# DoHoonKim8/halo2-lasso

Hardware: AMD Instinct MI355X
Metric: lasso_prove_time_ms (lower is better)
Workload: dtype u256 (BN254 Fr/Fq, 8x u32 Montgomery); 1 GPU; 2^24 AND Lasso lookup (32-bit operands, 4 chunks of 8+8 bits); lookups_per_proof=16777216, pcs=multilinear KZG (BN254), proof_bytes=64256, parallelism=1 GPU

## Files before the change

bindings/rust/src/sys.rs:

```rust
#![allow(non_camel_case_types, dead_code)]
use halo2_curves::bn256::{Fr, G1Affine, G2Affine};
use std::os::raw::{c_char, c_int, c_void};

pub type lh_status = c_int;
pub const LH_OK: lh_status = 0;
pub const LH_ERR_INVALID_SUMCHECK: lh_status = -1;
pub const LH_ERR_INVALID_PCS_PARAM: lh_status = -2;
pub const LH_ERR_INVALID_PCS_OPEN: lh_status = -3;
pub const LH_ERR_INVALID_SNARK: lh_status = -4;
pub const LH_ERR_SERIALIZATION: lh_status = -5;
pub const LH_ERR_TRANSCRIPT: lh_status = -6;
pub const LH_ERR_DEVICE: lh_status = -7;
pub const LH_ERR_ARG: lh_status = -8;

pub const LH_SC_MAX_TERMS: usize = 48;
pub const LH_SC_MAX_FACTORS: usize = 4;
pub const LH_SC_EVALUATIONS: c_int = 0;
pub const LH_SC_COEFFICIENTS: c_int = 1;
pub const LH_LASSO_MAX_CHUNKS: usize = 8;
pub const LH_LASSO_MAX_MEMORIES: usize = 16;
pub const LH_LASSO_MAX_TERMS: usize = 16;
pub const LH_RCCL_UNIQUE_ID_BYTES: usize = 128;

#[repr(C)] pub struct lh_ctx { _p: [u8; 0] }
// ... 95 lines not shown
    pub g_factor: [[u8; LH_SC_MAX_FACTORS]; LH_LASSO_MAX_TERMS],
}

#[repr(C)]
pub struct lh_comm {
    pub rank: c_int,
    pub size: c_int,
    pub user: *mut c_void,
    pub all_gather: Option<unsafe extern "C" fn(*mut c_void, *const c_void, *mut c_void, usize) -> c_int>,
    pub all_gather_device: Option<unsafe extern "C" fn(*mut c_void, *const c_void, *mut c_void, usize, *mut c_void) -> c_int>,
}

#[repr(C)]
pub struct lh_hp_lookup { pub inputs: *const lh_expr, pub tables: *const lh_expr, pub width: usize }
#[repr(C)] #[derive(Clone, Copy)]
pub struct lh_hp_lasso_lookup {
    pub table: lh_lasso_table,
    pub output_poly: usize,
    pub chunk_polys: [usize; LH_LASSO_MAX_CHUNKS],
}
#[repr(C)]
pub struct lh_hp_param {
    pub num_vars: usize,
    pub num_instance_polys: usize,
    pub num_instances: *const usize,
    pub num_preprocess_polys: usize,
    pub d_preprocess_polys: *const *const c_void,
    pub num_witness_polys: usize,
    pub num_challenges: usize,
    pub num_lookups: usize,
    pub lookups: *const lh_hp_lookup,
    pub num_permutation_polys: usize,
    pub permutation_poly_index: *const usize,
    pub d_permutation_polys: *const *const c_void,
    pub num_permutation_z_polys: usize,
    pub expression: lh_expr,
    pub num_lasso_lookups: usize,
    pub lasso_lookups: *const lh_hp_lasso_lookup,
}
#[repr(C)]
pub struct lh_hp_vparam {
    pub num_vars: usize,
    pub num_instance_polys: usize,
    pub num_instances: *const usize,
    pub num_witness_polys: usize,
    pub num_challenges: usize,
    pub num_lookups: usize,
    pub num_permutation_z_polys: usize,
    pub expression: lh_expr,
    pub num_preprocess_polys: usize,
    pub preprocess_comms: *const G1Affine,
    pub num_permutation_polys: usize,
    pub permutation_comms: *const G1Affine,
    pub num_lasso_lookups: usize,
    pub lasso_lookups: *const lh_hp_lasso_lookup,
}
#[repr(C)]
pub struct lh_hp_circuit {
    pub user: *mut c_void,
    pub synthesize: Option<unsafe extern "C" fn(*mut c_void, usize, *const Fr, usize, *mut *const c_void, usize) -> c_int>,
}

#[repr(C)]
#[derive(Clone, Copy, Debug, Default)]
pub struct lh_lasso_route {
    pub open_small_depth: u32,
    pub open_small_passes: u32,
    pub eq_factored_rounds: u32,
    pub standard_rounds: u32,
    pub rw_leaf_rounds: u32,
    pub resident_tails: u32,
    pub resident_rounds: u32,
    pub packed_ts_pairs: u32,
    pub derived_commitments: u32,
    pub sorted_dim_reuse: u32,
    pub sharded_rounds: u32,
    pub shard_exchanges: u32,
    pub window_table_jobs: u32,
    pub open_precommit: u32,
    pub resident_layers: u32,
    pub pp_folds: u32,
    pub msm_half_batches: u32,
    pub open_shared_sums: u32,
    pub reserved: [u32; 6],
}

extern "C" {
    pub fn lh_last_error() -> *const c_char;
    pub fn lh_version() -> *const c_char;
    pub fn lh_ctx_create(device_id: c_int, out: *mut *mut lh_ctx) -> lh_status;
    pub fn lh_ctx_destroy(ctx: *mut lh_ctx);
    pub fn lh_ctx_sync(ctx: *mut lh_ctx) -> lh_status;
    pub fn lh_ctx_stream(ctx: *mut lh_ctx) -> *mut c_void;
    pub fn lh_alloc(ctx: *mut lh_ctx, bytes: usize, d_out: *mut *mut c_void) -> lh_status;
    pub fn lh_free(ctx: *mut lh_ctx, d_ptr: *mut c_void) -> lh_status;
    pub fn lh_upload(ctx: *mut lh_ctx, d_dst: *mut c_void, src: *const c_void, bytes: usize) -> lh_status;
    pub fn lh_download(ctx: *mut lh_ctx, dst: *mut c_void, d_src: *const c_void, bytes: usize) -> lh_status;
    pub fn lh_fr_from_u64(ctx: *mut lh_ctx, d_in: *const u64, n: usize, d_out: *mut Fr) -> lh_status;
    pub fn lh_fr_from_u32(ctx: *mut lh_ctx, d_in: *const u32, n: usize, d_out: *mut Fr) -> lh_status;
    pub fn lh_fr_batch_invert(ctx: *mut lh_ctx, d_in: *const Fr, n: usize, d_out: *mut Fr) -> lh_status;
    pub fn lh_fix_var(ctx: *mut lh_ctx, d_in: *const Fr, n_in: usize, x: *const Fr, d_out: *mut Fr) -> lh_status;
    pub fn lh_eq_xy(ctx: *mut lh_ctx, y: *const Fr, num_vars: usize, d_out: *mut Fr) -> lh_status;
    pub fn lh_evaluate(ctx: *mut lh_ctx, d_polys: *const *const Fr, num_polys: usize, num_vars: usize,
                       point: *const Fr, out_evals: *mut Fr) -> lh_status;
    pub fn lh_lincomb(ctx: *mut lh_ctx, d_polys: *const *const Fr, w: *const Fr, num_polys: usize, n: usize,
                      d_out: *mut Fr) -> lh_status;
    pub fn lh_sumcheck_prove(ctx: *mut lh_ctx, prover_kind: c_int, num_vars: usize, expr: *const lh_sop,
                             d_polys: *const *const Fr, num_polys: usize, ys: *const Fr, num_ys: usize,
                             sum: *const Fr, t: *mut lh_transcript, out_challenges: *mut Fr, out_evals: *mut Fr) -> lh_status;
    pub fn lh_sumcheck_prove_expr(ctx: *mut lh_ctx, num_vars: usize, expr: *const lh_expr, d_polys: *const *const Fr,
                                  num_polys: usize, challenges: *const Fr, num_challenges: usize, ys: *const Fr,
                                  num_ys: usize, sum: *const Fr, t: *mut lh_transcript, out_challenges: *mut Fr,
                                  out_evals: *mut Fr) -> lh_status;
    pub fn lh_sumcheck_verify(prover_kind: c_int, num_vars: usize, degree: usize, sum: *const Fr,
                              t: *mut lh_transcript, out_eval: *mut Fr, out_x: *mut Fr) -> lh_status;
    pub fn lh_gkr_fractional_prove(ctx: *mut lh_ctx, num_batching: usize, num_vars: usize,
                                   claimed_p_0s: *const *const Fr, claimed_q_0s: *const *const Fr,
                                   d_ps: *const *const Fr, d_qs: *const *const Fr, t: *mut lh_transcript,
                                   out_p_xs: *mut Fr, out_q_xs: *mut Fr, out_x: *mut Fr) -> lh_status;
    pub fn lh_msm(ctx: *mut lh_ctx, d_scalars: *const Fr, d_bases: *const G1Affine, n: usize, out: *mut G1Affine) -> lh_status;
    pub fn lh_msm_u32(ctx: *mut lh_ctx, d_scalars: *const u32, d_bases: *const G1Affine, n: usize, out: *mut G1Affine) -> lh_status;
    pub fn lh_srs_upload(ctx: *mut lh_ctx, eqs_flat: *const G1Affine, num_vars: usize, out: *mut *mut lh_srs) -> lh_status;
    pub fn lh_srs_num_vars(srs: *const lh_srs) -> usize;
    pub fn lh_srs_free(ctx: *mut lh_ctx, srs: *mut lh_srs);
    pub fn lh_mkzg_batch_commit(ctx: *mut lh_ctx, srs: *const lh_srs, d_polys: *const *const Fr, num_polys: usize,
                                num_vars: usize, out_comms: *mut G1Affine) -> lh_status;
    pub fn lh_mkzg_open(ctx: *mut lh_ctx, srs: *const lh_srs, d_poly: *const Fr, num_vars: usize, point: *const Fr,
                        t: *mut lh_transcript, out_eval: *mut Fr) -> lh_status;
    pub fn lh_mkzg_batch_open(ctx: *mut lh_ctx, srs: *const lh_srs, num_vars: usize, d_polys: *const *const Fr,
                              num_polys: usize, points: *const Fr, num_points: usize, evals: *const lh_evaluation,
                              num_evals: usize, t: *mut lh_transcript) -> lh_status;
    pub fn lh_mkzg_vp_new(g1: *const G1Affine, g2: *const G2Affine, ss: *const G2Affine, num_vars: usize,
                          out: *mut *mut lh_mkzg_vp) -> lh_status;
    pub fn lh_mkzg_vp_free(vp: *mut lh_mkzg_vp);
    pub fn lh_mkzg_verify(vp: *const lh_mkzg_vp, comm: *const G1Affine, point: *const Fr, num_vars: usize,
                          eval: *const Fr, t: *mut lh_transcript) -> lh_status;
    pub fn lh_mkzg_batch_verify(vp: *const lh_mkzg_vp, num_vars: usize, comms: *const G1Affine, num_comms: usize,
                                points: *const Fr, num_points: usize, evals: *const lh_evaluation, num_evals: usize,
                                t: *mut lh_transcript) -> lh_status;
    pub fn lh_lasso_prove(ctx: *mut lh_ctx, srs: *const lh_srs, table: *const lh_lasso_table, num_vars: usize,
                          d_dims: *const *const u32, t: *mut lh_transcript) -> lh_status;
    pub fn lh_lasso_verify(vp: *const lh_mkzg_vp, table: *const lh_lasso_table, num_vars: usize,
                           t: *mut lh_transcript) -> lh_status;
    pub fn lh_ctx_set_comm(ctx: *mut lh_ctx, comm: *const lh_comm, shard_bit: usize) -> lh_status;
    pub fn lh_rccl_unique_id(out: *mut u8) -> lh_status;
    pub fn lh_ctx_set_comm_rccl(ctx: *mut lh_ctx, rank: c_int, size: c_int, unique_id: *const u8, shard_bit: usize) -> lh_status;
    pub fn lh_ctx_set_comm_loopback(ctx: *mut lh_ctx, rank: c_int, size: c_int, shard_bit: usize) -> lh_status;
    pub fn lh_ctx_comm_stats(ctx: *mut lh_ctx, out: *mut u64) -> lh_status;
    pub fn lh_ctx_comm_phase_stats(ctx: *mut lh_ctx, out: *mut u64, reset: c_int) -> lh_status;
    pub fn lh_ctx_memory_stats(ctx: *mut lh_ctx, out: *mut u64) -> lh_status;
    pub fn lh_ctx_compute_units(ctx: *mut lh_ctx, out: *mut usize) -> lh_status;
    pub fn lh_ctx_host_cpus(ctx: *mut lh_ctx, bus_id: *mut c_char, bus_id_cap: usize, cpulist: *mut c_char, cpulist_cap: usize) -> lh_status;
    pub fn lh_shard_extract(ctx: *mut lh_ctx, d_global: *const c_void, n_local: usize, shard_bit: usize, rho: usize,
                            rank: usize, elem_bytes: usize, d_local: *mut c_void) -> lh_status;
    pub fn lh_ctx_set_option(ctx: *mut lh_ctx, name: *const c_char, value: i64) -> lh_status;
    pub fn lh_ctx_get_option(ctx: *mut lh_ctx, name: *const c_char, out: *mut i64) -> lh_status;
    pub fn lh_lasso_last_route(ctx: *mut lh_ctx, out: *mut lh_lasso_route) -> lh_status;
    pub fn lh_lasso_prove_sharded(ctx: *mut lh_ctx, srs: *const lh_srs, table: *const lh_lasso_table, num_vars: usize,
                                  d_dims_local: *const *const u32, t: *mut lh_transcript) -> lh_status;
    pub fn lh_hyperplonk_prove(ctx: *mut lh_ctx, srs: *const lh_srs, pp: *const lh_hp_param,
                               instances: *const *const Fr, d_witness_polys: *const *const Fr,
                               t: *mut lh_transcript) -> lh_status;
    pub fn lh_hyperplonk_prove_sharded(ctx: *mut lh_ctx, srs: *const lh_srs, pp: *const lh_hp_param,
                                       instances: *const *const Fr, d_witness_polys_local: *const *const Fr,
                                       t: *mut lh_transcript) -> lh_status;
    pub fn lh_hyperplonk_prove_phases(ctx: *mut lh_ctx, srs: *const lh_srs, pp: *const lh_hp_param, num_phases: usize,
                                      num_witness_polys: *const usize, num_challenges: *const usize,
// ... 183 lines not shown
```

halo2-lasso_amd/__init__.py:

```python
import ctypes as C

from . import _ffi
from ._ffi import (lh_fr, lh_g1, lh_sop, lh_evaluation, lh_lasso_table, lh_transcript,
                   LH_SC_EVALUATIONS, LH_SC_COEFFICIENTS)

R_MOD = 0x30644E72E131A029B85045B68181585D2833E84879B9709143E1F593F0000001
Q_MOD = 0x30644E72E131A029B85045B68181585D97816A916871CA8D3C208C16D87CFD47
_MONT = 1 << 256
_MONT_INV_R = pow(_MONT, -1, R_MOD)
_MONT_INV_Q = pow(_MONT, -1, Q_MOD)

SUBTABLE_IDENTITY, SUBTABLE_AND, SUBTABLE_XOR = 0, 1, 2


class Error(Exception):
    code = None


class InvalidSumcheck(Error):
    code = _ffi.LH_ERR_INVALID_SUMCHECK


class InvalidPcsParam(Error):
    code = _ffi.LH_ERR_INVALID_PCS_PARAM
# ... 1395 lines not shown
            C.memmove(recv, out, len(out))
            return 0
        except Exception:
            return _ffi.LH_ERR_DEVICE
    comm = _ffi.lh_comm()
    comm.rank, comm.size, comm.user = rank, size, None
    comm.all_gather = _ffi._AG_CB(cb)
    ctx._comm_keepalive = (comm, cb)
    _check(ctx.lib.lh_ctx_set_comm(ctx.h, C.byref(comm), shard_bit))


def rccl_unique_id():
    buf = C.create_string_buffer(_ffi.LH_RCCL_UNIQUE_ID_BYTES)
    _check(_ffi.load().lh_rccl_unique_id(buf))
    return buf.raw


def attach_comm_rccl(ctx, rank, size, unique_id, shard_bit):
    if len(unique_id) != _ffi.LH_RCCL_UNIQUE_ID_BYTES:
        raise ArgumentError("unique id must be %d bytes" % _ffi.LH_RCCL_UNIQUE_ID_BYTES)
    _check(ctx.lib.lh_ctx_set_comm_rccl(ctx.h, rank, size, unique_id, shard_bit))


def comm_stats(ctx):
    out = (C.c_uint64 * 2)()
    _check(ctx.lib.lh_ctx_comm_stats(ctx.h, out))
    return {"device": int(out[0]), "host": int(out[1])}


def comm_phase_stats(ctx, reset=False):
    out = (C.c_uint64 * 16)()
    _check(ctx.lib.lh_ctx_comm_phase_stats(ctx.h, out, 1 if reset else 0))
    names = ["witness", "commit", "surge", "leaves", "gkr", "evals", "open", "outside"]
    return {nm: {"collectives": int(out[2 * i]), "bytes": int(out[2 * i + 1])} for i, nm in enumerate(names) if out[2 * i]}


def memory_stats(ctx):
    out = (C.c_uint64 * 4)()
    _check(ctx.lib.lh_ctx_memory_stats(ctx.h, out))
    return {"arena_high_water_bytes": int(out[0]), "arena_reserved_bytes": int(out[1]), "device_free_bytes": int(out[2]),
            "device_total_bytes": int(out[3])}


def attach_comm_loopback(ctx, rank, size, shard_bit):
    _check(ctx.lib.lh_ctx_set_comm_loopback(ctx.h, rank, size, shard_bit))


def detach_comm(ctx):
    _check(ctx.lib.lh_ctx_set_comm(ctx.h, None, 0))
    ctx._comm_keepalive = None


def shard_of(column, rank, size, shard_bit):
    rho = size.bit_length() - 1
    n = len(column)
    return column.reshape(n >> (shard_bit + rho), size, 1 << shard_bit)[:, rank, :].reshape(-1).copy()


def shard_poly(poly, rank, size, shard_bit):
    rho = size.bit_length() - 1
    n_local = (1 << poly.num_vars) >> rho
    out = poly.ctx.alloc(32 * n_local)
    _check(poly.ctx.lib.lh_shard_extract(poly.ctx.h, poly.ptr, n_local, shard_bit, rho, rank, 32, out.ptr))
    return MultilinearPolynomial(poly.ctx, out, poly.num_vars - rho)


def lasso_prove_sharded(pp, table, num_vars, dims_local, transcript):
    if len(dims_local) != table.c:
        raise ArgumentError("expected %d dim columns" % table.c)
    t = table.to_c()
    _check(pp.ctx.lib.lh_lasso_prove_sharded(pp.ctx.h, pp.h, C.byref(t), num_vars, _ptr_array(dims_local), transcript.p))


def lasso_last_timing(ctx):
    out = (C.c_double * _ffi.LH_LASSO_NUM_PHASES)()
    _check(ctx.lib.lh_lasso_last_timing(ctx.h, out))
    names = ["witness", "commit", "surge", "leaves", "gkr", "evals", "open_n", "open_l", "total"]
    return dict(zip(names, list(out)))


ROUTE_FIELDS = ["open_small_depth", "open_small_passes", "eq_factored_rounds", "standard_rounds", "rw_leaf_rounds",
                "resident_tails", "resident_rounds", "packed_ts_pairs", "derived_commitments", "sorted_dim_reuse",
                "sharded_rounds", "shard_exchanges", "window_table_jobs", "open_precommit", "resident_layers", "pp_folds", "msm_half_batches",
                "open_shared_sums"]


def lasso_last_route(ctx):
    out = (C.c_uint32 * 24)()
    _check(ctx.lib.lh_lasso_last_route(ctx.h, out))
    return dict(zip(ROUTE_FIELDS, [int(v) for v in out]))


def set_option(ctx, name, value):
    _check(ctx.lib.lh_ctx_set_option(ctx.h, name.encode(), int(value)))


def get_option(ctx, name):
    out = C.c_int64(0)
    _check(ctx.lib.lh_ctx_get_option(ctx.h, name.encode(), C.byref(out)))
    return int(out.value)


def profile_enable(ctx, on=True):
    _check(ctx.lib.lh_profile_enable(ctx.h, int(on)))


def profile_read(ctx):
    n = C.c_size_t()
    _check(ctx.lib.lh_profile_read(ctx.h, None, 0, C.byref(n)))
    arr = (_ffi.lh_prof_rec * max(n.value, 1))()
    _check(ctx.lib.lh_profile_read(ctx.h, arr, n.value, C.byref(n)))
    return [dict(name=r.name.decode(), ms=r.ms, bytes=r.bytes, muls=r.muls, items=r.items) for r in arr[:n.value]]


from . import expression
```

halo2-lasso_amd/csrc/dev.cpp:

```cpp
#include <string.h>
#include <stdlib.h>
#include <ctype.h>
#include <errno.h>
#include <sched.h>
#include <atomic>
#include <condition_variable>
#include <mutex>
#include <thread>
#include <functional>
#include <memory>
#include <emmintrin.h>
#include <hip/hip_ext.h>
#include <vector>
#include <chrono>
#include "dev.hpp"

namespace lh {

static thread_local std::string g_last_error;
void set_last_error(const char* msg) { g_last_error = msg ? msg : ""; }
const char* get_last_error() { return g_last_error.c_str(); }

Arena::~Arena() {
  for (auto& b : blocks_) (void)hipFree(b.p);
}

void* Arena::alloc(size_t bytes) {
  bytes = (bytes + 255) & ~(size_t)255;
  if (bytes == 0) bytes = 256;
  return alloc_raw(bytes);
}
void* Arena::alloc_raw(size_t bytes) {
  while (true) {
    if (!blocks_.empty()) {
      Block& b = blocks_[cur_];
      if (b.used + bytes <= b.size) {
        void* p = b.p + b.used;
        b.used += bytes;
        size_t tot = 0;
        for (size_t i = 0; i <= cur_; i++) tot += blocks_[i].used;
        if (tot > high_) high_ = tot;
        return p;
      }
      if (cur_ + 1 < blocks_.size()) {
        cur_++;
        blocks_[cur_].used = 0;
        continue;
      }
    }
    size_t want = blocks_.empty() ? ((size_t)64 << 20) : blocks_.back().size * 2;
    if (want < bytes) want = bytes;
    void* p = nullptr;
    LH_HIP(hipMalloc(&p, want));
    blocks_.push_back(Block{(char*)p, want, 0});
    cur_ = blocks_.size() - 1;
  }
}

void Arena::release(Mark m) {
  if (blocks_.empty()) return;
  for (size_t i = m.block + 1; i < blocks_.size(); i++) blocks_[i].used = 0;
  cur_ = m.block;
  blocks_[cur_].used = m.used;
}

void Ctx::opt_in_lds(const void* fn, int bytes) {
  for (const void* f : lds_opted)
    if (f == fn) return;
  LH_HIP(hipFuncSetAttribute(fn, hipFuncAttributeMaxDynamicSharedMemorySize, bytes));
  lds_opted.push_back(fn);
}

static const struct {
  const char* name;
  int64_t Options::*field;
  int64_t lo, hi;
} OPTION_TABLE[] = {
    {"open_small_min_vars", &Options::open_small_min_vars, 0, 64}, {"open_small_depth", &Options::open_small_depth, 0, 2},
    {"sc_eq_factoring", &Options::sc_eq_factoring, 0, 1},          {"lasso_pack_ts", &Options::lasso_pack_ts, 0, 1},
    {"sc_tail", &Options::sc_tail, 0, 1},                          {"sc_tail_max_len", &Options::sc_tail_max_len, 0, (int64_t)1 << 20},
    {"shard_exchange_log", &Options::shard_exchange_log, 0, 40},   {"msm_window_tables", &Options::msm_window_tables, 0, 40},
    {"open_precommit", &Options::open_precommit, 0, 64},           {"gkr_resident", &Options::gkr_resident, 0, 1},
    {"sc_pp_fold", &Options::sc_pp_fold, 0, 2},                    {"msm_half_batches", &Options::msm_half_batches, 0, 1},
    {"comm_round", &Options::comm_round, 0, 2},                    {"hyrax_rows", &Options::hyrax_rows, 0, 1},
    {"brakedown_batch_commit", &Options::brakedown_batch_commit, 0, 1}, {"brakedown_staged_open", &Options::brakedown_staged_open, 0, 1},
};

int64_t* Options::find(const char* name) {
  if (!name) return nullptr;
  for (const auto& o : OPTION_TABLE)
    if (strcmp(o.name, name) == 0) return &(this->*o.field);
  return nullptr;
}
bool Options::in_range(const char* name, int64_t value) {
  if (!name) return false;
  for (const auto& o : OPTION_TABLE)
    if (strcmp(o.name, name) == 0) return value >= o.lo && value <= o.hi;
  return false;
}

static bool env_number(const char* name, bool real, double lo, double hi, double& out, std::atomic<bool>* said = nullptr) {
  const char* e = getenv(name);
  if (!e || !*e) return false;
  char* end = nullptr;
  errno = 0;
  const double v = real ? strtod(e, &end) : (double)strtoll(e, &end, 10);
  if (end != e && *end == 0 && errno == 0 && v >= lo && v <= hi) {
    out = v;
    return true;
  }
  if (!said || !said->exchange(true))
    fprintf(stderr, "[lasso-hip] %s=%s is outside [%lld, %lld]: ignored\n", name, e, (long long)lo, (long long)hi);
  return false;
}

Options::Options() {
  for (const auto& o : OPTION_TABLE) {
    std::string env = "LH_";
    for (const char* p = o.name; *p; p++) env.push_back((char)toupper((unsigned char)*p));
    double v;
    if (!env_number(env.c_str(), false, (double)o.lo, (double)o.hi, v)) continue;
    this->*o.field = (int64_t)v;
    if (o.field == &Options::open_small_min_vars) open_small_min_vars_forced = true;
  }
}

enum KnobKind { INT, REAL, WORD, PATH };
static constexpr struct KnobRow {
  const char* env;
  KnobKind kind;
  double dflt, lo, hi;
  bool live;
  const char* word;
} KNOB_TABLE[] = {
    {"LH_SC_TAIL_G", INT, 0, 0, 1024},
    {"LH_MSM_C_OFF", INT, 4, -32, 32},
    {"LH_MSM_C_MAX", INT, 17, 1, 31},
    {"LH_MSM_K2", INT, 4, 2, 64},
    {"LH_MSM_SEG", INT, 0, 0, 256},
    {"LH_MSM_SLAB_LOG", INT, 16, 0, 31},
    {"LH_MSM_TREE_MAX", INT, 262144, 0, 1 << 30},
    {"LH_MSM_QUAD_MAX", INT, 262144, 0, 1 << 30},
    {"LH_MSM_TWO_LEVEL", INT, 1, 0, 1},
    {"LH_MSM_HALF_MIN_LOG", INT, 24, 0, 63},
    {"LH_MSM_HALF_COVER", INT, 12, 0, 1 << 20},
    {"LH_EXPR_MONOMIALS", INT, 0, 0, 1},
    {"LH_EXPR_JIT_MIN_VARS", INT, 16, 0, 64},
    {"LH_EXPR_EF_MIN_VARS", INT, 14, 2, 64},
    {"LH_FIN_LANES_MIN_BYTES", REAL, 0, -1, 1e18},
    {"LH_SC_U32", INT, 1, 0, 1}, {"LH_OPEN_U32_ROUNDS", INT, 1, 0, 1}, {"LH_OPEN_FOLD_COLS", INT, 1, 0, 1},
    {"LH_OPEN_SHARE_SUMS", INT, 1, 0, 1, true},
    {"LH_HOST_THREADS", INT, 48, 0, 4096},
    {"LH_JIT_CACHE", INT, 1, 0, 1}, {"LH_JIT_CACHE_DIR", PATH, 0, 0, 0},
    {"LH_EXPR_JIT", INT, 1, 0, 1},
    {"LH_SC_TAIL_TIMEOUT_MS", REAL, 2000, 0, 1e7, true}, {"LH_GKR_START_TIMEOUT_MS", REAL, 25, 0, 1e7, true},
    {"LH_COMM_WAIT_TIMEOUT_MS", INT, 30000, 1, 1e9}, {"LH_COMM_A2A", WORD, 0, 0, 1, false, "allgather"},
    {"LH_COMM_PROBE", INT, 1, 0, 1},
    {"LH_HOST_TRACE", INT, 0, 0, 1, true}, {"LH_SC_TAIL_TRACE", INT, 0, 0, 1}, {"LH_GKR_TRACE", INT, 0, 0, 1},
    {"LH_SC_DEBUG", INT, 0, 0, 1}, {"LH_MSM_DEBUG", INT, 0, 0, 1}, {"LH_HP_DEBUG", INT, 0, 0, 1}, {"LH_COMM_DEBUG", INT, 0, 0, 1},
    {"LH_OPEN_SMALL_CHECK", INT, 0, 0, 1},
    {"LH_COMM_A2A_SELF", INT, 0, 0, 1}, {"LH_COMM_PROBE_FAIL", INT, 0, 0, 1}, {"LH_SHARDED_COUNTERS_MIN_R", INT, 2, 1, 1 << 20},
};
static_assert(sizeof(KNOB_TABLE) / sizeof(KNOB_TABLE[0]) == (size_t)Knob::COUNT, "KNOB_TABLE: one row per Knob");

static double knob_read(const KnobRow& r, std::atomic<bool>* said) {
  double v = r.dflt;
  if (r.kind != WORD) {
    env_number(r.env, r.kind == REAL, r.lo, r.hi, v, said);
// ... 418 lines not shown
```

halo2-lasso_amd/csrc/dev.hpp:

```cpp
#pragma once
#include <hip/hip_runtime_api.h>
#include <stdint.h>
#include <stdarg.h>
#include <stdio.h>
#include <functional>
#include <string>
#include <vector>
#include <utility>
#include <stdexcept>

#include "../../include/lasso_hip.h"
#include "ec.cuh"

namespace lh {

struct Error : std::exception {
  int code;
  std::string msg;
  Error(int c, std::string m) : code(c), msg(std::move(m)) {}
  const char* what() const noexcept override { return msg.c_str(); }
};

void set_last_error(const char* msg);

#define LH_HIP(expr)                                                                       \
  do {                                                                                     \
    hipError_t e_ = (expr);                                                                \
    if (e_ != hipSuccess)                                                                  \
      throw ::lh::Error(LH_ERR_DEVICE, std::string(#expr) + ": " + hipGetErrorString(e_)); \
  } while (0)

#define LH_REQUIRE(cond, code, text) \
  do {                               \
    if (!(cond)) throw ::lh::Error((code), (text)); \
  } while (0)

class Arena {
 public:
  struct Mark {
    size_t block, used;
  };
  ~Arena();
  void* alloc(size_t bytes);
  void* alloc_raw(size_t bytes);
  template <class T>
  T* alloc_n(size_t n) {
    return (T*)alloc(n * sizeof(T));
  }
  Mark mark() const { return {cur_, blocks_.empty() ? 0 : blocks_[cur_].used}; }
  void release(Mark m);
  size_t high_water() const { return high_; }
  size_t reserved() const {
    size_t t = 0;
    for (const Block& b : blocks_) t += b.size;
    return t;
  }

 private:
  struct Block {
    char* p;
    size_t size, used;
  };
  std::vector<Block> blocks_;
  size_t cur_ = 0, high_ = 0;
};

struct ArenaScope {
  Arena& a;
  Arena::Mark m;
  explicit ArenaScope(Arena& a_) : a(a_), m(a_.mark()) {}
  ~ArenaScope() { a.release(m); }
};

struct ProfRec {
  char name[40];
  double ms;
  double bytes;
  double muls;
  double items;
};

struct ScFinishArgs {
  uint32_t* ticket;
  uint32_t last_ticket;
  Fr* out_host;
  uint32_t* flag;
  uint32_t seq;
  uint64_t* wide;
  uint32_t tag;
  uint64_t* lanes;
};
constexpr uint32_t FIN_LANE_SUMS = 65536;
constexpr unsigned SC_LANE_TAG_SHIFT = 40;

struct Options {
  int64_t open_small_min_vars = 21;
  bool open_small_min_vars_forced = false;
  int64_t open_small_depth = 0;
  int64_t sc_eq_factoring = 1;
  int64_t lasso_pack_ts = 1;
  int64_t sc_tail = 1;
  int64_t sc_tail_max_len = 8192;
  int64_t shard_exchange_log = 19;
  int64_t open_precommit = 1;
  int64_t msm_window_tables = 0;
  int64_t sc_pp_fold = 1;
  int64_t msm_half_batches = 1;
  int64_t gkr_resident = 1;
  int64_t comm_round = 0;
  int64_t hyrax_rows = 1;
  int64_t brakedown_batch_commit = 1;
  int64_t brakedown_staged_open = 0;
  Options();
  int64_t* find(const char* name);
  static bool in_range(const char* name, int64_t value);
};

enum class Knob {
  SC_TAIL_G, MSM_C_OFF, MSM_C_MAX, MSM_K2, MSM_SEG, MSM_SLAB_LOG, MSM_TREE_MAX, MSM_QUAD_MAX, MSM_TWO_LEVEL, MSM_HALF_MIN_LOG,
  MSM_HALF_COVER, EXPR_MONOMIALS, EXPR_JIT_MIN_VARS, EXPR_EF_MIN_VARS,
  FIN_LANES_MIN_BYTES, SC_U32, OPEN_U32_ROUNDS, OPEN_FOLD_COLS, OPEN_SHARE_SUMS,
  HOST_THREADS, JIT_CACHE, JIT_CACHE_DIR, EXPR_JIT, SC_TAIL_TIMEOUT_MS, GKR_START_TIMEOUT_MS, COMM_WAIT_TIMEOUT_MS, COMM_A2A,
  COMM_PROBE,
  HOST_TRACE, SC_TAIL_TRACE, GKR_TRACE, SC_DEBUG, MSM_DEBUG, HP_DEBUG, COMM_DEBUG, OPEN_SMALL_CHECK,
  COMM_A2A_SELF, COMM_PROBE_FAIL, SHARDED_COUNTERS_MIN_R,
  COUNT
};
double knob(Knob k);
const char* knob_text(Knob k);
struct RouteStats {
  uint32_t v[LH_LASSO_ROUTE_WORDS] = {0};
  enum { OPEN_DEPTH, OPEN_PASSES, EF_ROUNDS, STD_ROUNDS, RW_ROUNDS, TAILS, TAIL_ROUNDS, PACKED_TS, DERIVED, SORTED_REUSE,
         SHARDED_ROUNDS, SHARD_EXCHANGES, WIN_TABLE_JOBS, OPEN_PRECOMMIT, RESIDENT_LAYERS, PP_FOLDS, MSM_HALF_BATCHES,
         OPEN_SHARED_SUMS };
};

class HostWorker {
 public:
  HostWorker();
  ~HostWorker();
  void submit(std::function<void()> fn);
  void wait();
 private:
  struct Impl;
  Impl* impl_;
};

struct OpenPrecommit;
struct Ctx {
  Options opt;
  RouteStats route;
  int device = 0;
  hipStream_t stream = nullptr;
  Arena arena;
  void* pinned = nullptr;
  size_t pinned_bytes = 0;
  int num_cus = 256;
  int wall_clock_khz = 100000;
  double lasso_ms[LH_LASSO_NUM_PHASES] = {0};
  lh_comm comm = {0, 1, nullptr, nullptr, nullptr};
  bool has_comm = false;
  bool comm_loopback = false;
  size_t shard_bit = 0;
  bool shard_active = false;
  void* rccl_comm = nullptr;
  void* comm_stage = nullptr;
  size_t comm_stage_bytes = 0;
  uint64_t comm_stats[2] = {0, 0};
  uint64_t comm_phase_stats[8][2] = {};
  int comm_phase = 7;
  Fr* sc_redirect = nullptr;
  uint64_t* sc_wide = nullptr;
  uint32_t sc_tag = 0;
  uint32_t sc_tag_seq = 0;
  uint64_t* lanes_host = nullptr;
  bool comm_host_recv_ok = true;
  Fr* round_out(Fr* out_host) const { return sc_redirect ? sc_redirect : out_host; }
  void wait_round(uint32_t seq) {
    if (!sc_redirect) wait_flag(seq);
  }
  uint64_t* tail_trace = nullptr;
  std::vector<std::pair<const char*, double>> host_stamps;
  bool host_trace_on = false;
  void host_stamp(const char* tag);
  void host_stamps_print();
  struct EqHalfEntry {
    std::vector<uint8_t> key;
    const Fr* table;
    bool sharded = false;
  };
  std::vector<EqHalfEntry> eq_half_cache;
  struct QuadSumEntry {
    const uint32_t* col;
    size_t len;
    std::vector<uint8_t> point;
    Fr s[4];
  };
  std::vector<QuadSumEntry> quad_sums;
  bool prof = false;
  std::vector<ProfRec> prof_recs;
  bool live = false;
  struct LiveRec {
    ProfRec rec;
    hipEvent_t e0, e1;
    uint32_t batch;
  };
  std::vector<LiveRec> live_recs;
  std::vector<hipEvent_t> live_pool;
  uint32_t live_batch = 0;
  hipEvent_t live_event();
  void live_resolve(std::vector<ProfRec>& out);
  bool is_helper = false;
  Ctx* helper = nullptr;
  lh_ctx* helper_handle = nullptr;
  OpenPrecommit* precommit = nullptr;
  HostWorker* worker = nullptr;
  hipEvent_t handoff_ev = nullptr;
// ... 35 lines not shown
  void gkr_send_layer(const Fr* vals, size_t count, uint32_t seq);
  void gkr_abort();
  void gkr_resync();
  void wait_flag(uint32_t seq);
  std::vector<const void*> lds_opted;
  void opt_in_lds(const void* fn, int bytes);
  void wait_chunks(const struct TailChunk* chunks, size_t count, uint32_t seq, Fr* out);
  bool wait_chunks_or(const struct TailChunk* chunks, size_t count, uint32_t seq, uint32_t alt, Fr* out);
};

struct ShardActive {
  Ctx& c;
  explicit ShardActive(Ctx& c_) : c(c_) { c.shard_active = true; }
  ~ShardActive() { c.shard_active = false; }
};

struct Shard {
  bool on = false;
  bool loopback = false;
  size_t rho = 0, j = 0, rank = 0, R = 1;
  explicit Shard(const Ctx& c) {
    if (!c.shard_active) return;
    on = true, j = c.shard_bit, rank = (size_t)c.comm.rank, R = (size_t)c.comm.size, loopback = c.comm_loopback;
    while (((size_t)1 << rho) < R) rho++;
  }
  bool sharded(size_t num_vars) const { return on && num_vars >= j + (rho ? rho : 1) + 1; }
  size_t local_vars(size_t num_vars) const { return sharded(num_vars) ? num_vars - rho : num_vars; }
  size_t local_len(size_t num_vars) const { return (size_t)1 << local_vars(num_vars); }
};

struct ReplicatedRange {
  size_t first = 0, count = 0;
  ReplicatedRange(const Shard& sh, size_t len) {
    if (!sh.on || sh.R <= 1) {
      count = len;
    } else if (len < sh.R) {
      count = sh.rank == 0 || sh.loopback ? len : 0;
    } else {
      const size_t per = len / sh.R;
      first = sh.rank * per;
      count = sh.rank + 1 == sh.R ? len - first : per;
    }
  }
};

void host_parallel_for(size_t n, const std::function<void(size_t)>& fn);
void host_parallel_prewake(size_t n, unsigned us);

struct ProfScope {
  Ctx& c;
  ProfRec rec;
  bool on;
  ProfScope(Ctx& c_, const char* name, double bytes, double muls, double items) : c(c_), on(c_.prof) {
    if (!on) return;
    snprintf(rec.name, sizeof rec.name, "%s", name);
    rec.bytes = bytes, rec.muls = muls, rec.items = items, rec.ms = 0;
    if (!c.prof_ev[0]) {
      LH_HIP(hipEventCreate(&c.prof_ev[0]));
      LH_HIP(hipEventCreate(&c.prof_ev[1]));
    }
    LH_HIP(hipEventRecord(c.prof_ev[0], c.stream));
  }
  ~ProfScope() {
    if (!on) return;
    (void)hipEventRecord(c.prof_ev[1], c.stream);
    (void)hipEventSynchronize(c.prof_ev[1]);
    float ms = 0;
    (void)hipEventElapsedTime(&ms, c.prof_ev[0], c.prof_ev[1]);
    rec.ms = ms;
    c.prof_recs.push_back(rec);
  }
};

void k_fr_from_u64(Ctx&, const uint64_t* in, size_t n, Fr* out);
void k_fr_from_u32(Ctx&, const uint32_t* in, size_t n, Fr* out);
void k_fr_to_repr(Ctx&, const Fr* in, size_t n, Fr* out);
void k_fr_from_repr(Ctx&, const Fr* in, size_t n, Fr* out);
void k_fr_binop(Ctx&, int op, const Fr* a, const Fr* b, size_t n, Fr* out);
void k_fr_mul_chain(Ctx&, const Fr* a, const Fr* b, size_t n, int iters, Fr* out);
void k_fr_batch_invert(Ctx&, const Fr* in, size_t n, Fr* out);
void k_fix_var(Ctx&, const Fr* in, size_t n_in, const Fr& x, Fr* out);
void k_fix_var_multi(Ctx&, const Fr* const* in, Fr* const* out, size_t count, size_t n_in, const Fr& x);
void k_eq_xy(Ctx&, const Fr* y, size_t num_vars, Fr* out);
void k_bind_first(Ctx&, const Fr* const* in, size_t count, const Fr& x, Fr* out_host);
void k_gather_heads(Ctx&, const Fr* const* in, size_t count, int k, Fr* out_host);
void k_lincomb(Ctx&, const Fr* const* polys, const Fr* w, size_t count, size_t n, Fr* out);
void k_lincomb_fold(Ctx&, const Fr* const* polys, const Fr* w, size_t count, size_t half, const Fr& x, Fr* out);
bool k_lincomb_fold_small(Ctx&, const uint32_t* const* cols, const size_t* lens, const Fr* coef, size_t count, size_t half,
                          const Fr& x, Fr* out);
void k_inner_products(Ctx&, const Fr* const* polys, size_t count, const Fr* weights, size_t n, Fr* out_host);
constexpr int LCM_MAX_FR = 8, LCM_MAX_SMALL = 24;
constexpr int LCF_MAX = 24;
constexpr int LCB_MAX = 24;
void k_inner_products_small(Ctx&, const uint32_t* const* polys, size_t count, const Fr* weights, size_t n, Fr* out_host);
void k_inner_products_small_half(Ctx&, const uint32_t* const* polys, size_t count, const Fr* eq_half, size_t half,
                                 const Fr& y0, Fr* out_host);
void k_inner_products_small_quads(Ctx&, const uint32_t* col, const Fr* e0, size_t quads, Fr* out_host);
void k_inner_products_quads(Ctx&, const uint32_t* const* cols, const size_t* lens, size_t count, const Fr* e1, size_t quads,
                            Fr* d_out);
constexpr int QS_MAX_COLS = 24;
void k_quad_sums(Ctx&, const uint32_t* const* cols, const size_t* lens, size_t count, const Fr* e0, size_t quads, Fr* d_out);
void k_lincomb_bind2(Ctx&, const uint32_t* const* cols, const size_t* lens, const Fr* w, size_t count, const Fr& r0, const Fr& r1,
                     const Fr* eq_level, size_t size, Fr* out, Fr* out_host);
void k_sc_round_u32_bind2(Ctx&, const uint32_t* col, const Fr* eq_level, const Fr& r0, const Fr& r1, size_t size, Fr* out,
                          Fr* out_host);
void k_lincomb_mixed(Ctx&, const Fr* const* fr, const Fr* wfr, size_t num_fr, const uint32_t* const* sm,
                     const size_t* sm_len, const Fr* wsm, size_t num_sm, size_t n, Fr* out);
void k_tree_up(Ctx&, const Fr* in, size_t half, Fr* out);
void k_tree_up_multi(Ctx&, const Fr* const* in, Fr* const* out, size_t count, size_t half);
void k_tree_tops(Ctx&, const Fr* const* in, Fr* const* out, const int* H, size_t count);
void k_frac_up(Ctx&, const Fr* p, const Fr* q, size_t half, Fr* vp, Fr* vq);
void k_quotient_step(Ctx&, const Fr* rem, size_t half, const Fr& x, Fr* q, Fr* rem_out);
void k_lasso_rw_leaves(Ctx&, const uint32_t* dim, const uint32_t* e, const uint32_t* ts, size_t n,
                       const Fr& gamma, const Fr& gamma2, const Fr& tau, Fr* rs, Fr* ws);
void k_lasso_rw_leaves_up(Ctx&, const uint32_t* dim, const uint32_t* e, const uint32_t* ts, size_t n, const Fr& gamma,
                          const Fr& gamma2, const Fr& tau, Fr* rs, Fr* ws, Fr* rs_up, Fr* ws_up);
void k_lasso_if_leaves(Ctx&, int subtable, uint32_t chunk_bits, const uint32_t* final_cts, size_t m,
                       const Fr& gamma, const Fr& gamma2, const Fr& tau, Fr* init, Fr* fin);
void k_or_u32(Ctx&, const uint32_t* const* cols, size_t count, size_t n, uint32_t* out_host);
void k_fill_u32(Ctx&, uint32_t* out, uint32_t value, size_t n);
void k_pack_u32(Ctx&, const uint32_t* a, const uint32_t* b, uint32_t shift, size_t n, uint32_t* out);
void k_delta_u32(Ctx&, const uint32_t* col, size_t len, size_t half, uint64_t offset, uint32_t* out_lo, uint32_t* out_hi);
void k_lasso_counters(Ctx&, const uint32_t* const* dims, size_t cc, size_t n, size_t m, uint32_t* const* read_ts,
                      uint32_t* const* final_cts, uint32_t* const* keep_sorted = nullptr, uint32_t* const* keep_index = nullptr);
void k_cs_partition(Ctx&, const uint32_t* const* dims, size_t cc, size_t n, size_t m, unsigned rho, unsigned j, unsigned hi_bits,
                    uint32_t* const* sidx, uint32_t* const* send, uint32_t* start_host, bool* bad_out);
void k_cs_rank(Ctx&, const uint32_t* const* recv, const size_t* n_recv, size_t cc, unsigned hi_bits, unsigned a_bits, size_t m_loc,
               uint32_t* const* ret, uint32_t* counts);
void k_cs_scatter(Ctx&, const uint32_t* const* back, const uint32_t* const* sidx, size_t cc, size_t n, uint32_t* const* read_ts);
void k_cs_final(Ctx&, const uint32_t* all_counts, size_t cc, size_t m, unsigned rho, size_t m_loc, uint32_t* const* final_cts);
void k_lasso_subtable_read(Ctx&, int subtable, uint32_t chunk_bits, const uint32_t* dim, size_t n, uint32_t* e);
struct LassoG {
  uint32_t num_terms;
  Fr coeff[LH_LASSO_MAX_TERMS];
  uint8_t nfac[LH_LASSO_MAX_TERMS];
  uint8_t fac[LH_LASSO_MAX_TERMS][LH_SC_MAX_FACTORS];
  const uint32_t* e[LH_LASSO_MAX_MEMORIES];
};
void k_lasso_output(Ctx&, const LassoG& g, size_t n, Fr* a);
struct LassoGSmall {
  uint32_t num_terms;
  uint32_t coeff[LH_LASSO_MAX_TERMS];
  uint8_t fac[LH_LASSO_MAX_TERMS];
  const uint32_t* e[LH_LASSO_MAX_MEMORIES];
};
void k_lasso_output_small(Ctx&, const LassoGSmall& g, size_t n, uint32_t* a);
bool k_fr_to_index(Ctx&, const Fr* in, size_t n, uint32_t bits, uint32_t* out);
bool k_fr_tables_equal(Ctx&, const Fr* a, const Fr* b, size_t n);

void rccl_unique_id(uint8_t out[LH_RCCL_UNIQUE_ID_BYTES]);
void comm_attach_rccl(Ctx&, int rank, int size, const uint8_t id[LH_RCCL_UNIQUE_ID_BYTES], size_t shard_bit);
void comm_probe_host_recv(Ctx&);
void comm_attach_loopback(Ctx&, int rank, int size, size_t shard_bit);
void comm_detach(Ctx&);
void comm_all_gather_dev(Ctx&, const void* d_send, void* d_recv, size_t bytes);
void comm_all_gather_host(Ctx&, const void* send, void* recv, size_t bytes);
void comm_all_to_all_multi(Ctx&, size_t nbuf, const void* const* d_send, const size_t* send_off, const size_t* send_cnt,
                           void* const* d_recv, const size_t* recv_off, const size_t* recv_cnt, const size_t* peer_off,
                           const void* send_base, size_t send_stride, size_t elem);
void comm_sum_publish(Ctx&, const Fr* d_part, Fr* d_scratch, size_t count, Fr* out_host, uint32_t seq);
void comm_sum_lanes(Ctx&, uint64_t* d_lanes, uint64_t* d_scratch, size_t count, Fr* out_host);
uint32_t comm_next_tag(Ctx&);
void k_loopback_allreduce_lanes(Ctx&, const uint64_t* d_in, size_t n, size_t R, uint64_t* out);

void k_shard_merge(Ctx&, const void* gathered, size_t n_local, size_t j, size_t rho, size_t elem, void* global);
void k_gather_interleave(Ctx&, const Fr* gathered, size_t count, size_t n_local, size_t R, size_t block, Fr* const* out);
void k_sum_publish(Ctx&, const Fr* all, size_t R, size_t D, Fr* out_host, uint32_t seq);
void k_shard_extract(Ctx&, const void* global, size_t n_local, size_t j, size_t rho, size_t s, size_t elem, void* local);
void k_loopback_gather(Ctx&, const void* d_send, void* d_recv, size_t bytes, size_t R);
void k_scale(Ctx&, const Fr* in, const Fr& w, size_t n, Fr* out);

constexpr int SC_MAX_TABLES = 72;
struct ScRound {
  const Fr* in[SC_MAX_TABLES];
  Fr* out[SC_MAX_TABLES];
  uint32_t num_tables;
  uint32_t num_terms;
  int32_t global_eq;
  Fr coeff[LH_SC_MAX_TERMS];
  uint8_t coeff_is_one[LH_SC_MAX_TERMS];
  uint8_t nfac[LH_SC_MAX_TERMS];
  uint8_t fac[LH_SC_MAX_TERMS][LH_SC_MAX_FACTORS];
  Fr r;
  const Fr* eq_level;
  uint8_t pp;
};
bool k_sc_round(Ctx&, const ScRound& rd, int degree, bool bind, size_t size, Fr* evals_host);
bool k_sc_round_streams(const ScRound& rd, int degree, size_t size);
void k_eq_levels(Ctx&, const Fr* in, size_t n_in, Fr* const* levels, size_t nlev);
constexpr int SC_OPEN_MAX_TERMS = 6;
struct ScOpenRound {
  const Fr* in[SC_OPEN_MAX_TERMS];
  Fr* out[SC_OPEN_MAX_TERMS];
  const Fr* eq_level[SC_OPEN_MAX_TERMS];
  uint32_t num_terms;
  Fr r;
};
void k_sc_round_open(Ctx&, const ScOpenRound& rd, bool bind, size_t size, Fr* out_host);

constexpr int SC_RW_MAX_PAIRS = 8;
struct ScRwRound {
  const Fr* l[SC_RW_MAX_PAIRS];
  const Fr* r[SC_RW_MAX_PAIRS];
  Fr* lo[SC_RW_MAX_PAIRS];
  Fr* ro[SC_RW_MAX_PAIRS];
  Fr cs[SC_RW_MAX_PAIRS], k[SC_RW_MAX_PAIRS];
  const Fr* eq_level;
  Fr rchal;
  uint32_t num_pairs;
};
void k_sc_round_rw(Ctx&, const ScRwRound& rd, bool bind, size_t size, Fr* out_host, bool fold = false);

struct TailChunk {
  uint32_t w[4];
};
struct TailMbox {
  TailChunk c[3];
  uint32_t pad[4];
};
constexpr uint32_t SC_TAIL_ABORT = 0xffffffffu;
constexpr int SC_TAIL_MAX_DEGREE = 6;
size_t k_sc_tail_capacity(const Ctx&, const ScRound& rd, int degree);
void k_sc_tail_launch(Ctx&, const ScRound& rd, int degree, size_t n0, bool first_bind, size_t num_out, uint32_t seq0,
                      TailChunk* msg_host, Fr* out_host);
void k_sc_tail_resync(Ctx&);

constexpr int GKR_MAX_TREES = 16;
constexpr int GKR_MAX_VARS = 16;
constexpr uint32_t GKR_CAP = 128;
constexpr uint32_t GKR_THREADS = 256;
constexpr uint32_t GKR_MSG_CHUNKS = 3 * (GKR_MAX_TREES + GKR_MAX_VARS);
constexpr uint32_t GKR_START_FAILED = 0xfffffffeu;
enum { GKR_F_SPLIT = 1, GKR_F_BIND = 2, GKR_F_EQ = 4, GKR_F_NOMSG = 8, GKR_F_KOFF = 16 };
struct GkrLayerDev {
  const Fr* lv[GKR_MAX_TREES];
  const Fr* rv[GKR_MAX_TREES];
  uint32_t h, B;
  uint32_t g, s_log;
  uint32_t seq;
  uint32_t flags;
  const Fr* eq_level;
  Fr r_prev;
  Fr coef[GKR_MAX_TREES];
  Fr koff[GKR_MAX_TREES];
};
bool k_gkr_resident_geometry(uint32_t h, uint32_t* g, uint32_t* s_log);
void k_gkr_resident_launch(Ctx&, const GkrLayerDev* layers, size_t num_layers, TailChunk* msg_host, Fr* out_host);

struct ExtRound {
  const Fr* in[SC_MAX_TABLES];
  Fr* out[SC_MAX_TABLES];
  uint32_t num_tables, num_terms;
  const Fr* coeff;
  const uint8_t* is_one;
  const uint32_t* off;
  const uint8_t* fac;
  const uint8_t* store;
  Fr r;
};
void k_sc_round_ext(Ctx&, const ExtRound& rd, int degree, bool bind, size_t size, Fr* evals_host);
void k_rotate_gather(Ctx&, const Fr* poly, size_t num_vars, int rot, uint32_t primitive, uint32_t x_inv, Fr* out);
void k_identity_table(Ctx&, size_t n, Fr* out);
void k_identity_table_shard(Ctx&, size_t n_local, size_t j, size_t rho, size_t rank, Fr* out);
void k_bh_order(Ctx&, size_t num_vars, uint32_t primitive, uint32_t* order, uint32_t* nth);
void k_one_hot_table(Ctx&, size_t n, size_t hot, Fr* out);
enum { PROG_ADD = 0, PROG_SUB = 1, PROG_MUL = 2, PROG_NEG = 3, PROG_MOV = 4 };
enum { PROG_REG = 0, PROG_ATOM = 1, PROG_CONST = 2, PROG_PAIR = 3 };
constexpr int PROG_MAX_REGS = 8;
struct ProgRound {
  const Fr* in[SC_MAX_TABLES];
  uint32_t num_tables, num_instrs, num_regs, result_reg;
  const uint32_t* code;
  const Fr* consts;
};
struct JitKernel;
bool jit_enabled(size_t num_vars);
std::string jit_debug_source(const uint32_t* code, size_t num_instrs, uint32_t num_regs, uint32_t result_reg, int degree);
const JitKernel* jit_sc_round(const Ctx&, const uint32_t* host_code, size_t num_instrs, uint32_t num_regs, uint32_t result_reg, int degree);
unsigned jit_blocks_per_cu(const JitKernel*);
void jit_launch(Ctx&, const JitKernel*, const ProgRound& pr, unsigned points, unsigned grid, size_t size, Fr* partials, const ScFinishArgs& fin);
void k_sc_round_prog(Ctx&, const ProgRound& pr, int points, size_t size, Fr* evals_host, const JitKernel* jit = nullptr);
constexpr int LIN_MAX_TABLES = 8;
struct LinSums {
  const Fr* t[LIN_MAX_TABLES];
  Fr coeff[LIN_MAX_TABLES];
  uint32_t count;
};
void k_lin_sums(Ctx&, const LinSums& ls, size_t size, Fr* out_host);
enum { ROWS_ATOM_POLY = 0, ROWS_ATOM_IDENTITY = 1, ROWS_ATOM_LAGRANGE = 2 };
struct RowsAtom {
// ... 123 lines not shown
```

halo2-lasso_amd/csrc/host.hpp:

```cpp
#pragma once
#include <string.h>
#include <functional>
#include <map>
#include <mutex>
#include <vector>
#include "dev.hpp"
#include "ff_host.hpp"

namespace lh {

const char* get_last_error();

typedef host::Fr HFr;
typedef host::G1Affine HG1;

static inline Fr dev(const HFr& f) {
  Fr r;
  memcpy(&r, &f, 32);
  return r;
}
static inline HFr hst(const Fr& f) {
  HFr r;
  memcpy(&r, &f, 32);
  return r;
// ... 56 lines not shown
  std::vector<HFr> read_field_elements(size_t n) {
    std::vector<HFr> v(n);
    for (auto& f : v) f = read_field_element();
    return v;
  }
  HG1 read_commitment() {
    LH_REQUIRE(t->read_commitment, LH_ERR_ARG, "transcript cannot read (write-only callback table)");
    HG1 p;
    check(t->read_commitment(t->user, (lh_g1*)&p));
    return p;
  }
  std::vector<HG1> read_commitments(size_t n) {
    std::vector<HG1> v(n);
    for (auto& p : v) p = read_commitment();
    return v;
  }
};

typedef std::function<void(size_t num_vars, const HG1* comms, size_t num_comms, const HFr* points, size_t num_points,
                           const lh_evaluation* evals, size_t num_evals, Transcript& tr)>
    PcsBatchVerify;
typedef std::function<std::vector<HG1>(Transcript& tr, size_t n)> PcsReadCommitments;

std::vector<HFr> host_eq_xy(const std::vector<HFr>& y);
HFr host_eq_xy_eval(const HFr* x, const HFr* y, size_t n);
std::vector<HFr> evaluate_polys(Ctx&, const Fr* const* d_polys, size_t count, size_t num_vars, const HFr* point);

struct SumCheckResult {
  std::vector<HFr> challenges;
  std::vector<HFr> evals;
  bool u32_terms_built = false;
};
struct ScRwPairs {
  uint32_t num_pairs;
  HFr cs[SC_RW_MAX_PAIRS], k[SC_RW_MAX_PAIRS];
  HFr const_total;
};
struct ScU32 {
  const uint32_t* col = nullptr;
  bool have_sums = false;
  Fr odd, s2, s3;
};
struct ScU32Terms {
  struct Poly {
    std::vector<const uint32_t*> col;
    std::vector<size_t> len;
    std::vector<Fr> w;
  };
  std::vector<Poly> polys;
};
struct ScOptions {
  bool sum_is_exact = false;
  bool sharded = false;
  const ScRwPairs* rw = nullptr;
  const ScU32* u32 = nullptr;
  const ScU32Terms* u32_terms = nullptr;
};
SumCheckResult sum_check_prove(Ctx&, int prover_kind, size_t num_vars, const lh_sop& expr, const Fr* const* d_polys,
                               size_t num_polys, const HFr* ys, size_t num_ys, const HFr& sum, Transcript& tr,
                               const ScOptions& opt = ScOptions());

const Fr* eq_half_lookup(Ctx&, const HFr* y, size_t num_vars, bool sharded = false);
const Fr* eq_half_get(Ctx&, const HFr* y, size_t num_vars, bool sharded = false);
struct EqHalfScope {
  Ctx& c;
  size_t mark, mark_sums;
  explicit EqHalfScope(Ctx& c_) : c(c_), mark(c_.eq_half_cache.size()), mark_sums(c_.quad_sums.size()) {}
  ~EqHalfScope() {
    c.eq_half_cache.resize(mark);
    c.quad_sums.resize(mark_sums);
  }
};
bool sc_open_column_rounds(const Ctx&, size_t num_vars, bool sharded);
const Fr* quad_sums_lookup(const Ctx&, const uint32_t* col, size_t len, const HFr* y, size_t num_vars);
void quad_sums_put(Ctx&, const uint32_t* col, size_t len, const HFr* y, size_t num_vars, const HFr s[4]);
void quad_sums_evaluate(Ctx&, const uint32_t* const* cols, size_t count, const HFr* y, size_t num_vars, const Fr* eq_half, HFr* evals);

typedef std::function<void(const Fr* const*, Fr* const*, const Fr&, bool, size_t, Fr*)> RoundFn;
struct EqFactoring {
  struct One {
    size_t table;
    const HFr* y;
    std::vector<const Fr*> level;
    HFr S, S_prev;
    std::vector<HFr> q;
  };
  std::vector<One> eqs;
  bool per_term = false;
  bool trusted_claim = false;
  bool untrusted = false;
  std::vector<HFr> inv_1my;
  HFr c;
  HFr add_const;
  HFr kappa = HFr::one(), lin0 = HFr::zero(), lin1 = HFr::zero();
  std::function<bool(bool bind, size_t size)> streams;
  std::function<void(const Fr* const* in, Fr* const* out, const Fr& r, bool bind, size_t size, size_t round, int points,
                     Fr* out_host)>
      round;
  std::function<bool(const std::vector<const Fr*>& cur, bool bind, const HFr& r_prev, size_t n0, size_t round, const HFr& claim,
                     Transcript& tr, SumCheckResult& res)>
      resident_tail;
};
SumCheckResult sum_check_loop(Ctx&, int prover_kind, size_t num_vars, int degree, std::vector<const Fr*> cur,
                              const std::vector<char>& used, size_t num_polys, const HFr& sum, Transcript& tr,
                              bool sharded, const RoundFn& round_fn, const ScRound* tail_rd = nullptr,
                              EqFactoring* ef = nullptr);
SumCheckResult sum_check_prove_expr(Ctx&, size_t num_vars, const lh_expr& expr, const Fr* const* d_polys,
                                    size_t num_polys, const HFr* challenges, size_t num_challenges, const HFr* ys,
                                    size_t num_ys, const HFr& sum, Transcript& tr, bool sharded = false);

std::vector<HFr> evaluate_polys(Ctx&, const Fr* const* d_polys, size_t count, size_t num_vars, const HFr* point, bool sharded);
void comm_sum_fr(Ctx&, HFr* v, size_t n);
void comm_sum_points(Ctx&, HG1* pts, size_t n);
void comm_gather_tables(Ctx&, const Fr* local_block, size_t count, size_t n_local, size_t block, Fr* const* out);
void comm_gather_concat(Ctx&, const Fr* local, size_t n_local, Fr* out);
void eq_xy_shard(Ctx&, const Shard&, const HFr* y, size_t num_vars, size_t first, Fr* out_local);

struct FracSumCheckResult {
  std::vector<HFr> p_xs, q_xs, x;
};
FracSumCheckResult prove_fractional_sum_check(Ctx&, size_t num_batching, size_t num_vars,
                                              const HFr* const* claimed_p_0s, const HFr* const* claimed_q_0s,
                                              const Fr* const* d_ps, const Fr* const* d_qs, Transcript& tr);
struct GrandProductResult {
  std::vector<HFr> roots, claims;
  std::vector<std::vector<HFr>> points;
};
GrandProductResult prove_grand_product(Ctx&, size_t num_trees, const Fr* const* d_leaves, const size_t* num_vars,
                                       Transcript& tr, const Fr* const* d_level_up = nullptr,
                                       const uint8_t* plus_one = nullptr,
                                       const std::function<void()>& trees_built = nullptr);

struct Srs {
  G1Affine* d_eqs = nullptr;
  size_t num_vars = 0;
  const G1Affine* eq(size_t k) const { return d_eqs + (((size_t)1 << k) - 1); }
  mutable std::vector<G1Affine*> shard_levels;
  mutable int shard_rank = -1;
  mutable size_t shard_R = 0, shard_j = 0;
  mutable std::map<size_t, HG1> level_sums;
  mutable std::map<size_t, HG1> shard_level_sums;
  struct WinTable {
    G1Affine* d = nullptr;
    uint32_t c = 0, W = 0;
  };
  mutable std::map<size_t, WinTable> win_tables;
};
const Srs::WinTable* srs_window_table(Ctx&, const Srs&, size_t level);
const G1Affine* srs_shard_level(Ctx&, const Srs&, size_t level);
Srs* mkzg_setup(Ctx&, const HFr* ss, size_t num_vars);
std::vector<HG1> mkzg_batch_commit(Ctx&, const Srs&, const Fr* const* d_polys, size_t num_polys, size_t num_vars);
std::vector<HG1> mkzg_batch_commit_u32(Ctx&, const Srs&, const uint32_t* const* d_polys, size_t num_polys,
                                       size_t num_vars);
struct SmallOpen;
HFr mkzg_open(Ctx&, const Srs&, const Fr* d_poly, size_t num_vars, const HFr* point, Transcript& tr,
              const SmallOpen* small = nullptr);
struct SmallLinear {
  std::vector<size_t> poly;
  std::vector<HFr> coeff;
};
struct SmallPoly {
  const uint32_t* ptr = nullptr;
  size_t len = 0;
  uint32_t bits = 0;
  const SmallLinear* linear = nullptr;
};
void mkzg_batch_open(Ctx&, const Srs&, size_t num_vars, const Fr* const* d_polys, size_t num_polys,
                     const HFr* points, size_t num_points, const lh_evaluation* evals, size_t num_evals,
                     Transcript& tr, const SmallPoly* small = nullptr);

struct SmallOpen {
  std::vector<SmallPoly> cols;
  std::vector<HFr> coef;
  std::vector<const Fr*> merged;
  std::vector<Fr> merged_w;
  std::function<void()> ensure_merged;
};
// ... 232 lines not shown
```

halo2-lasso_amd/csrc/kernels_poly.hip:

```cpp
#include <hip/hip_runtime.h>
#include <string.h>
#include <algorithm>
#include "dev.hpp"
#include "ff_host.hpp"
#include "reduce.cuh"
#include "resident.cuh"
#include "wide.cuh"

namespace lh {

static inline dim3 grid_for(size_t n, int block = 256, size_t cap = 4096) {
  size_t g = (n + block - 1) / block;
  if (g < 1) g = 1;
  if (g > cap) g = cap;
  return dim3((unsigned)g);
}
#define GSTRIDE(i, n) \
  for (size_t i = (size_t)blockIdx.x * blockDim.x + threadIdx.x; i < (n); i += (size_t)gridDim.x * blockDim.x)

__global__ void fr_from_u64_kernel(const uint64_t* __restrict__ in, size_t n, Fr* __restrict__ out) {
  GSTRIDE(i, n) out[i] = from_u64<FrParams>(in[i]);
}
__global__ void fr_from_u32_kernel(const uint32_t* __restrict__ in, size_t n, Fr* __restrict__ out) {
  GSTRIDE(i, n) out[i] = from_u64<FrParams>(in[i]);
// ... 129 lines not shown
  int i = threadIdx.x;
  if (i < count) {
    Fr e0 = p.in[i][0], e1 = p.in[i][1];
    out[i] = add(mul(sub(e1, e0), x), e0);
  }
  __builtin_amdgcn_fence(__ATOMIC_RELEASE, "");
  __builtin_amdgcn_s_barrier();
  if (i == 0) __hip_atomic_store(flag, seq, __ATOMIC_RELEASE, __HIP_MEMORY_SCOPE_SYSTEM);
}
void k_bind_first(Ctx& c, const Fr* const* in, size_t count, const Fr& x, Fr* out_host) {
  LH_REQUIRE(count <= (size_t)SC_MAX_TABLES, LH_ERR_ARG, "bind_first: too many tables");
  if (!count) return;
  FirstPack p;
  for (size_t i = 0; i < count; i++) p.in[i] = in[i];
  const uint32_t seq = c.next_seq();
  hipLaunchKernelGGL(bind_first_kernel, dim3(1), dim3(64), 0, c.stream, p, (int)count, x, out_host, c.flag, seq);
  c.wait_flag(seq);
}
__global__ void gather_heads_kernel(FirstPack p, int count, int k, Fr* __restrict__ out) {
  int i = blockIdx.x * blockDim.x + threadIdx.x;
  if (i < count * k) out[i] = p.in[i / k][i % k];
}
void k_gather_heads(Ctx& c, const Fr* const* in, size_t count, int k, Fr* out_host) {
  LH_REQUIRE(count <= (size_t)SC_MAX_TABLES, LH_ERR_ARG, "gather_heads: too many tables");
  if (!count) return;
  FirstPack p;
  for (size_t i = 0; i < count; i++) p.in[i] = in[i];
  int total = (int)count * k;
  hipLaunchKernelGGL(gather_heads_kernel, dim3((total + 63) / 64), dim3(64), 0, c.stream, p, (int)count, k, out_host);
  c.sync();
}

__global__ void eq_expand_kernel(const Fr* __restrict__ cur, size_t n_cur, Fr y, Fr* __restrict__ nxt) {
  GSTRIDE(k, n_cur) {
    Fr e = cur[k];
    Fr hi = mul(e, y);
    nxt[2 * k + 1] = hi;
    nxt[2 * k] = sub(e, hi);
  }
}
__global__ void fr_set_one_kernel(Fr* p) { p[0] = Fr::one(); }

constexpr int EQ_SMALL = 9;
__global__ void eq_outer_kernel(const Fr* __restrict__ lo_tab, int lo_bits, const Fr* __restrict__ hi_tab, size_t n,
                                Fr* __restrict__ out) {
  const size_t mask = ((size_t)1 << lo_bits) - 1;
  GSTRIDE(i, n) out[i] = mul(hi_tab[i >> lo_bits], lo_tab[i & mask]);
}

constexpr int EQ_GROUPS = 4;
struct EqGroups {
  Fr y[EQ_GROUPS][EQ_SMALL];
  int levels[EQ_GROUPS];
  Fr* out[EQ_GROUPS];
};
__global__ __launch_bounds__(256) void eq_groups_kernel(EqGroups g) {
  __shared__ Fr a[1 << EQ_SMALL];
  __shared__ Fr b[1 << (EQ_SMALL - 1)];
  const int levels = g.levels[blockIdx.x];
  Fr* cur = (levels & 1) ? b : a;
  Fr* nxt = (levels & 1) ? a : b;
  if (threadIdx.x == 0) cur[0] = Fr::one();
  __syncthreads();
  int n = 1;
  for (int i = 0; i < levels; i++) {
    const Fr yi = g.y[blockIdx.x][i];
    for (int k = threadIdx.x; k < n; k += blockDim.x) {
      Fr e = cur[k];
      Fr hi = mul(e, yi);
      nxt[2 * k + 1] = hi;
      nxt[2 * k] = sub(e, hi);
    }
    __syncthreads();
    Fr* t = cur;
    cur = nxt;
    nxt = t;
    n <<= 1;
  }
  Fr* out = g.out[blockIdx.x];
  for (int k = threadIdx.x; k < n; k += blockDim.x) out[k] = cur[k];
}

void k_eq_xy(Ctx& c, const Fr* y, size_t num_vars, Fr* out) {
  ProfScope ps(c, "eq_xy", 64.0 * ((size_t)1 << num_vars), 1.0 * ((size_t)1 << num_vars), (double)((size_t)1 << num_vars));
  const size_t ngroups = std::max<size_t>(1, (num_vars + EQ_SMALL - 1) / EQ_SMALL);
  LH_REQUIRE(ngroups <= (size_t)EQ_GROUPS, LH_ERR_ARG, "eq_xy: too many variables");
  ArenaScope scope(c.arena);
  EqGroups g;
  size_t first[EQ_GROUPS], cnt[EQ_GROUPS];
  Fr* tab[EQ_GROUPS];
  for (size_t k = 0, done = 0; k < ngroups; k++) {
    cnt[k] = (num_vars - done + (ngroups - k) - 1) / (ngroups - k);
    first[k] = done;
    done += cnt[k];
    tab[k] = ngroups == 1 ? out : c.arena.alloc_n<Fr>((size_t)1 << cnt[k]);
    g.levels[k] = (int)cnt[k];
    g.out[k] = tab[k];
    for (size_t i = 0; i < cnt[k]; i++) g.y[k][i] = y[first[k] + cnt[k] - 1 - i];
  }
  hipLaunchKernelGGL(eq_groups_kernel, dim3((unsigned)ngroups), dim3(256), 0, c.stream, g);
  Fr* cur = tab[0];
  size_t done = cnt[0];
  for (size_t k = 1; k < ngroups; k++) {
    const bool last = k + 1 == ngroups;
    const size_t n = (size_t)1 << (done + cnt[k]);
    Fr* dst = last ? out : c.arena.alloc_n<Fr>(n);
    hipLaunchKernelGGL(eq_outer_kernel, grid_for(n), 256, 0, c.stream, cur, (int)done, tab[k], n, dst);
    cur = dst;
    done += cnt[k];
  }
}

template <class T>
__global__ void shard_extract_kernel(const T* __restrict__ g, size_t n_local, unsigned j, unsigned rho, size_t s,
                                     T* __restrict__ local) {
  const size_t lo_mask = ((size_t)1 << j) - 1;
  GSTRIDE(i, n_local) local[i] = g[((i >> j) << (j + rho)) | (s << j) | (i & lo_mask)];
}
struct alignas(16) Bytes64 {
  uint4 a, b, c, d;
};
void k_shard_extract(Ctx& c, const void* global, size_t n_local, size_t j, size_t rho, size_t s, size_t elem,
                     void* local) {
  if (!n_local) return;
  dim3 g = grid_for(n_local);
  if (elem == 4)
    hipLaunchKernelGGL(shard_extract_kernel<uint32_t>, g, 256, 0, c.stream, (const uint32_t*)global, n_local, (unsigned)j,
                       (unsigned)rho, s, (uint32_t*)local);
  else if (elem == 32)
    hipLaunchKernelGGL(shard_extract_kernel<Fr>, g, 256, 0, c.stream, (const Fr*)global, n_local, (unsigned)j,
                       (unsigned)rho, s, (Fr*)local);
  else if (elem == 64)
    hipLaunchKernelGGL(shard_extract_kernel<Bytes64>, g, 256, 0, c.stream, (const Bytes64*)global, n_local, (unsigned)j,
                       (unsigned)rho, s, (Bytes64*)local);
  else
    throw Error(LH_ERR_ARG, "shard_extract: unsupported element size");
}
template <class T>
__global__ void shard_merge_kernel(const T* __restrict__ gathered, size_t n_local, unsigned j, unsigned rho,
                                   T* __restrict__ global) {
  const size_t lo_mask = ((size_t)1 << j) - 1, s_mask = ((size_t)1 << rho) - 1;
  GSTRIDE(g, n_local << rho) {
    const size_t s = (g >> j) & s_mask, local = ((g >> (j + rho)) << j) | (g & lo_mask);
    global[g] = gathered[s * n_local + local];
  }
}
void k_shard_merge(Ctx& c, const void* gathered, size_t n_local, size_t j, size_t rho, size_t elem, void* global) {
  if (!n_local) return;
  dim3 g = grid_for(n_local << rho);
  if (elem == 4)
    hipLaunchKernelGGL(shard_merge_kernel<uint32_t>, g, 256, 0, c.stream, (const uint32_t*)gathered, n_local, (unsigned)j,
                       (unsigned)rho, (uint32_t*)global);
  else if (elem == 32)
    hipLaunchKernelGGL(shard_merge_kernel<Fr>, g, 256, 0, c.stream, (const Fr*)gathered, n_local, (unsigned)j,
                       (unsigned)rho, (Fr*)global);
  else
    throw Error(LH_ERR_ARG, "shard_merge: unsupported element size");
}

struct InterleaveOut {
  Fr* out[SC_MAX_TABLES];
};
__global__ void gather_interleave_kernel(const Fr* __restrict__ gathered, unsigned count, size_t n_local, unsigned R,
                                         size_t block, InterleaveOut o) {
  const size_t full = n_local * R;
  GSTRIDE(e, full * count) {
    const size_t t = e / full, k = e % full, lo = k % block, q = k / block, hi = q / R, s = q % R;
    o.out[t][k] = gathered[((size_t)s * count + t) * n_local + hi * block + lo];
  }
}
void k_gather_interleave(Ctx& c, const Fr* gathered, size_t count, size_t n_local, size_t R, size_t block, Fr* const* out) {
  LH_REQUIRE(count <= (size_t)SC_MAX_TABLES, LH_ERR_ARG, "gather_interleave: too many tables");
  LH_REQUIRE(block >= 1 && n_local % block == 0, LH_ERR_ARG, "gather_interleave: bad block size");
  if (!count || !n_local) return;
  InterleaveOut o;
  for (size_t t = 0; t < count; t++) o.out[t] = out[t];
  hipLaunchKernelGGL(gather_interleave_kernel, grid_for(n_local * R * count), 256, 0, c.stream, gathered, (unsigned)count,
                     n_local, (unsigned)R, block, o);
}

__global__ void sum_publish_kernel(const Fr* __restrict__ all, unsigned R, unsigned D, Fr* __restrict__ out_host,
                                   uint32_t* flag, uint32_t seq) {
  if (threadIdx.x == 0) {
    for (unsigned x = 0; x < D; x++) {
      Fr acc = all[x];
      for (unsigned s = 1; s < R; s++) acc = add(acc, all[(size_t)s * D + x]);
      out_host[x] = acc;
    }
    __hip_atomic_store(flag, seq, __ATOMIC_RELEASE, __HIP_MEMORY_SCOPE_SYSTEM);
  }
}
void k_sum_publish(Ctx& c, const Fr* all, size_t R, size_t D, Fr* out_host, uint32_t seq) {
  hipLaunchKernelGGL(sum_publish_kernel, dim3(1), dim3(64), 0, c.stream, all, (unsigned)R, (unsigned)D, out_host, c.flag, seq);
// ... 418 lines not shown
    const size_t q = base + (size_t)i * 256;
    const Fr h = q < quads ? add(e0[2 * q], e0[2 * q + 1]) : Fr::zero();
    hs[0][256 * i + threadIdx.x] = make_uint4(h.l[0], h.l[1], h.l[2], h.l[3]);
    hs[1][256 * i + threadIdx.x] = make_uint4(h.l[4], h.l[5], h.l[6], h.l[7]);
  }
  const int lane = threadIdx.x & 63;
  const size_t rows = (size_t)gridDim.x * 4, row = (size_t)blockIdx.x * 4 + (threadIdx.x >> 6);
#pragma nounroll
  for (int k = 0; k < pk.count; k++) {
    const uint4* __restrict__ col = (const uint4*)pk.p[k];
    const size_t cq = pk.quads[k];
    Wide acc[4];
#pragma unroll
    for (int t = 0; t < 4; t++) acc[t] = Wide::zero();
    uint4 a[QPL];
#pragma unroll
    for (int i = 0; i < QPL; i++) {
      const size_t q = base + (size_t)i * 256;
      a[i] = q < cq ? col[q] : make_uint4(0u, 0u, 0u, 0u);
    }
#pragma unroll
    for (int i = 0; i < QPL; i++) {
      const uint4 lo = hs[0][256 * i + threadIdx.x], hi = hs[1][256 * i + threadIdx.x];
      Fr h;
      h.l[0] = lo.x, h.l[1] = lo.y, h.l[2] = lo.z, h.l[3] = lo.w, h.l[4] = hi.x, h.l[5] = hi.y, h.l[6] = hi.z, h.l[7] = hi.w;
      wide_mac(acc[0], h, a[i].x), wide_mac(acc[1], h, a[i].y), wide_mac(acc[2], h, a[i].z), wide_mac(acc[3], h, a[i].w);
      __builtin_amdgcn_sched_barrier(0);
    }
    const bool up32 = (lane & 32) != 0, up16 = (lane & 16) != 0;
    const Wide b0 = wide_exchange_add(acc[0], acc[2], up32, 32), b1 = wide_exchange_add(acc[1], acc[3], up32, 32);
    Wide s = wide_exchange_add(b0, b1, up16, 16);
#pragma unroll
    for (int mask = 8; mask >= 1; mask >>= 1) {
      Wide o;
#pragma unroll
      for (int j = 0; j < 10; j++) o.l[j] = (uint32_t)__shfl_xor((int)s.l[j], mask, 64);
      wide_add(s, o);
    }
    if ((lane & 15) == 0) {
      uint32_t* dst = partials + ((size_t)(4 * k + (lane >> 4)) * rows + row) * 10;
#pragma unroll
      for (int j = 0; j < 10; j++) dst[j] = s.l[j];
    }
  }
}
__global__ __launch_bounds__(256) void quad_sums_reduce_kernel(const uint32_t* __restrict__ partials, size_t per_row,
                                                               Fr* __restrict__ out) {
  __shared__ Fr lds[4];
  const uint32_t* row = partials + (size_t)blockIdx.x * per_row * 10;
  Wide acc = Wide::zero();
  for (size_t i = threadIdx.x; i < per_row; i += blockDim.x) {
    Wide w;
#pragma unroll
    for (int j = 0; j < 10; j++) w.l[j] = row[i * 10 + j];
    wide_add(acc, w);
  }
  const Fr v = block_reduce_sum(wide_reduce(acc), lds);
  if (threadIdx.x == 0) out[blockIdx.x] = v;
}
void k_quad_sums(Ctx& c, const uint32_t* const* cols, const size_t* lens, size_t count, const Fr* e0, size_t quads, Fr* d_out) {
  ProfScope ps(c, "quad_sums", 4.0 * 4 * quads * count + 64.0 * quads, 0.25 * quads * count, (double)quads);
  if (!count) return;
  LH_REQUIRE(quads >= 1, LH_ERR_ARG, "quad_sums: empty table");
  const size_t per_block = (size_t)256 * QS_QPL, blocks = (quads + per_block - 1) / per_block, rows = blocks * 4;
  LH_REQUIRE(blocks < ((size_t)1 << 31), LH_ERR_ARG, "quad_sums: table too large");
  uint32_t* partials = c.arena.alloc_n<uint32_t>(rows * 10 * 4 * std::min<size_t>(count, QS_MAX_COLS));
  for (size_t base = 0; base < count; base += QS_MAX_COLS) {
    QuadSumsPack pk;
    memset(&pk, 0, sizeof(pk));
    pk.count = (int)std::min<size_t>(QS_MAX_COLS, count - base);
    for (int i = 0; i < pk.count; i++) pk.p[i] = cols[base + i], pk.quads[i] = std::min(lens[base + i] / 4, quads);
    hipLaunchKernelGGL(quad_sums_kernel<QS_QPL>, dim3((unsigned)blocks), 256, 0, c.stream, pk, e0, quads, partials);
    hipLaunchKernelGGL(quad_sums_reduce_kernel, 4 * pk.count, 256, 0, c.stream, partials, rows, d_out + 4 * base);
  }
}

struct LcBind2 {
  const uint32_t* p[LCB_MAX];
  uint64_t quads[LCB_MAX];
  Fr w[LCB_MAX][4];
  int count;
};
__global__ __launch_bounds__(256) void lincomb_bind2_kernel(const LcBind2* __restrict__ pkp, const Fr* __restrict__ eq_level,
                                                            size_t entries, Fr* __restrict__ out, Fr* __restrict__ partials,
                                                            ScFinishArgs fin) {
  __shared__ Fr lds[4];
  __shared__ int is_last;
  const LcBind2& pk = *pkp;
  const bool odd = threadIdx.x & 1;
  Fr acc = Fr::zero();
  GSTRIDE(i, entries) {
    Wide t = Wide::zero();
    for (int k = 0; k < pk.count; k++)
      if (i < pk.quads[k]) {
        const uint4 a = ((const uint4*)pk.p[k])[i];
        wide_mac(t, pk.w[k][0], a.x), wide_mac(t, pk.w[k][1], a.y), wide_mac(t, pk.w[k][2], a.z), wide_mac(t, pk.w[k][3], a.w);
      }
    const Fr v = wide_redc(t);
    out[i] = v;
    acc = add(acc, mul(v, eq_level[i >> 1]));
  }
  const Fr q0 = block_reduce_sum(odd ? Fr::zero() : acc, lds);
  const Fr q1 = block_reduce_sum(odd ? acc : Fr::zero(), lds);
  if (gridDim.x == 1) {
    if (threadIdx.x == 0) {
      fin.out_host[0] = q0, fin.out_host[1] = q1;
      publish_round(fin, 2);
    }
    return;
  }
  if (threadIdx.x == 0) fin_put(fin, partials, (size_t)blockIdx.x * 2, q0), fin_put(fin, partials, (size_t)blockIdx.x * 2 + 1, q1);
  if (!fin_ticket(fin, &is_last)) return;
  for (int x = 0; x < 2; x++) {
    Fr a2 = Fr::zero();
    for (uint32_t i = threadIdx.x; i < gridDim.x; i += blockDim.x) a2 = add(a2, fin_get(fin, partials, (size_t)i * 2 + x));
    a2 = block_reduce_sum(a2, lds);
    if (threadIdx.x == 0) fin.out_host[x] = a2;
  }
  if (threadIdx.x == 0) publish_round(fin, 2);
}
void k_lincomb_bind2(Ctx& c, const uint32_t* const* cols, const size_t* lens, const Fr* w, size_t count, const Fr& r0, const Fr& r1,
                     const Fr* eq_level, size_t size, Fr* out, Fr* out_host) {
  LH_REQUIRE(count >= 1 && count <= (size_t)LCB_MAX && size >= 1 && !c.sc_redirect, LH_ERR_ARG, "lincomb_bind2: bad shape");
  const uint32_t seq = c.next_seq();
  ArenaScope scope(c.arena);
  const size_t entries = 2 * size;
  host::Fr h0, h1;
  const host::Fr one = host::Fr::one();
  memcpy(&h0, &r0, sizeof(h0));
  memcpy(&h1, &r1, sizeof(h1));
  const host::Fr b4[4] = {(one - h1) * (one - h0), (one - h1) * h0, h1 * (one - h0), h1 * h0};
  LcBind2* h_pk = (LcBind2*)((char*)c.pin(65536) + 8192);
  memset(h_pk, 0, sizeof(LcBind2));
  h_pk->count = (int)count;
  for (size_t k = 0; k < count; k++) {
    host::Fr wk;
    memcpy(&wk, &w[k], sizeof(wk));
    h_pk->p[k] = cols[k], h_pk->quads[k] = std::min(lens[k] / 4, entries);
    for (int t = 0; t < 4; t++) {
      const host::Fr x = wk * b4[t];
      Fr d;
      memcpy(&d, &x, sizeof(d));
      h_pk->w[k][t] = prescale_r(d);
    }
  }
  LcBind2* d_pk = (LcBind2*)c.arena.alloc(sizeof(LcBind2));
  LH_HIP(hipMemcpyAsync(d_pk, h_pk, sizeof(LcBind2), hipMemcpyHostToDevice, c.stream));
  const size_t g = std::min<size_t>((entries + 255) / 256, (size_t)c.num_cus * 8);
  Fr* partials = c.arena.alloc_n<Fr>(g * 2);
  const ScFinishArgs fin = c.finish_for((uint32_t)g, out_host, seq, 32.0 * (double)entries);
  {
    ProfScope ps(c, "lincomb<bind2,u32>", (16.0 * count + 32.0 + 16.0) * (double)entries, (0.25 * count + 1.6) * (double)entries, (double)size);
    hipLaunchKernelGGL(lincomb_bind2_kernel, dim3((unsigned)g), dim3(256), 0, c.stream, d_pk, eq_level, entries, out, partials, fin);
  }
  c.wait_round(seq);
}

struct U32Bind2 {
  Fr w[4];
};
__global__ __launch_bounds__(256) void sc_round_u32_bind2_kernel(const uint32_t* __restrict__ col, const Fr* __restrict__ eq_level,
                                                                 U32Bind2 k, size_t entries, Fr* __restrict__ out,
                                                                 Fr* __restrict__ partials, ScFinishArgs fin) {
  __shared__ Fr lds[4];
  __shared__ int is_last;
  Fr acc = Fr::zero();
  GSTRIDE(i, entries) {
    const uint4 a = ((const uint4*)col)[i];
    Wide t = Wide::zero();
    wide_mac(t, k.w[0], a.x), wide_mac(t, k.w[1], a.y), wide_mac(t, k.w[2], a.z), wide_mac(t, k.w[3], a.w);
    const Fr v = wide_redc(t);
    out[i] = v;
    if (i & 1) acc = add(acc, mul(v, eq_level[i >> 1]));
  }
  acc = block_reduce_sum(acc, lds);
  if (gridDim.x == 1) {
    if (threadIdx.x == 0) {
      fin.out_host[0] = acc;
      publish_round(fin, 1);
    }
    return;
  }
  if (threadIdx.x == 0) fin_put(fin, partials, blockIdx.x, acc);
  if (!fin_ticket(fin, &is_last)) return;
  Fr a2 = Fr::zero();
  for (uint32_t i = threadIdx.x; i < gridDim.x; i += blockDim.x) a2 = add(a2, fin_get(fin, partials, i));
  a2 = block_reduce_sum(a2, lds);
  if (threadIdx.x == 0) {
    fin.out_host[0] = a2;
    publish_round(fin, 1);
  }
}
void k_sc_round_u32_bind2(Ctx& c, const uint32_t* col, const Fr* eq_level, const Fr& r0, const Fr& r1, size_t size, Fr* out,
                          Fr* out_host) {
  LH_REQUIRE(size >= 1 && !c.sc_redirect, LH_ERR_ARG, "sc_round_u32_bind2: bad shape");
  const uint32_t seq = c.next_seq();
  ArenaScope scope(c.arena);
  const size_t entries = 2 * size;
  const size_t g = std::min<size_t>((entries + 255) / 256, (size_t)c.num_cus * 8);
  Fr* partials = c.arena.alloc_n<Fr>(g);
  const ScFinishArgs fin = c.finish_for((uint32_t)g, out_host, seq, 32.0 * (double)entries);
  host::Fr h0, h1;
  const host::Fr one = host::Fr::one();
  memcpy(&h0, &r0, sizeof(h0));
  memcpy(&h1, &r1, sizeof(h1));
  const host::Fr w[4] = {(one - h1) * (one - h0), (one - h1) * h0, h1 * (one - h0), h1 * h0};
  U32Bind2 k;
  for (int i = 0; i < 4; i++) {
    Fr d;
    memcpy(&d, &w[i], sizeof(d));
    k.w[i] = prescale_r(d);
  }
  {
    ProfScope ps(c, "sc_round_u32<bind2>", 64.0 * (double)entries, 1.2 * (double)entries, (double)size);
    hipLaunchKernelGGL(sc_round_u32_bind2_kernel, dim3((unsigned)g), dim3(256), 0, c.stream, col, eq_level, k, entries, out, partials, fin);
  }
  c.wait_round(seq);
}

__global__ void tree_up_kernel(const Fr* __restrict__ in, size_t half, Fr* __restrict__ out) {
  GSTRIDE(i, half) out[i] = mul(in[i], in[half + i]);
}
__global__ void tree_up_multi_kernel(PtrPack p, size_t half) {
  const Fr* __restrict__ in = p.in[blockIdx.y];
  Fr* __restrict__ out = p.out[blockIdx.y];
  GSTRIDE(i, half) out[i] = mul(in[i], in[half + i]);
}
void k_tree_up_multi(Ctx& c, const Fr* const* in, Fr* const* out, size_t count, size_t half) {
  ProfScope ps(c, "tree_up", 96.0 * half * count, 1.0 * half * count, (double)half * count);
  if (!half) return;
  for (size_t base = 0; base < count; base += SC_MAX_TABLES) {
    size_t k = count - base < (size_t)SC_MAX_TABLES ? count - base : (size_t)SC_MAX_TABLES;
    PtrPack p;
    for (size_t i = 0; i < k; i++) {
      p.in[i] = in[base + i];
      p.out[i] = out[base + i];
    }
    dim3 g = grid_for(half);
    g.y = (unsigned)k;
    hipLaunchKernelGGL(tree_up_multi_kernel, g, 256, 0, c.stream, p, half);
  }
}
void k_tree_up(Ctx& c, const Fr* in, size_t half, Fr* out) {
  ProfScope ps(c, "tree_up", 96.0 * half, 1.0 * half, (double)half);
  if (half) hipLaunchKernelGGL(tree_up_kernel, grid_for(half), 256, 0, c.stream, in, half, out);
}
constexpr int TREE_SMALL = 9;
struct TreeTops {
  const Fr* in[SC_MAX_TABLES];
  Fr* out[SC_MAX_TABLES];
  int H[SC_MAX_TABLES];
};
__global__ __launch_bounds__(256) void tree_top_kernel(TreeTops t) {
  __shared__ Fr a[1 << TREE_SMALL];
  __shared__ Fr b[1 << (TREE_SMALL - 1)];
  const Fr* __restrict__ in = t.in[blockIdx.x];
  Fr* __restrict__ out = t.out[blockIdx.x];
  const int H = t.H[blockIdx.x];
  if (H <= 0) return;
  int half = 1 << H;
  for (int i = threadIdx.x; i < half; i += blockDim.x) {
    Fr v = mul(in[i], in[half + i]);
    a[i] = v;
    out[(half - 2) + i] = v;
  }
  __syncthreads();
  Fr* cur = a;
  Fr* nxt = b;
  for (int h = H - 2; h >= 0; h--) {
    half = 1 << (h + 1);
    for (int i = threadIdx.x; i < half; i += blockDim.x) {
      Fr v = mul(cur[i], cur[half + i]);
      nxt[i] = v;
      out[(half - 2) + i] = v;
    }
    __syncthreads();
    Fr* tmp = cur;
    cur = nxt;
    nxt = tmp;
  }
}
void k_tree_tops(Ctx& c, const Fr* const* in, Fr* const* out, const int* H, size_t count) {
  LH_REQUIRE(count <= (size_t)SC_MAX_TABLES, LH_ERR_ARG, "tree_tops: too many trees");
  if (!count) return;
  TreeTops t;
  for (size_t i = 0; i < count; i++) {
    LH_REQUIRE(H[i] <= TREE_SMALL, LH_ERR_ARG, "tree_tops: level too large");
    t.in[i] = in[i];
    t.out[i] = out[i];
    t.H[i] = H[i];
  }
  ProfScope ps(c, "tree_tops", 0, 0, (double)count);
  hipLaunchKernelGGL(tree_top_kernel, dim3((unsigned)count), dim3(256), 0, c.stream, t);
}

__global__ void frac_up_kernel(const Fr* __restrict__ p, const Fr* __restrict__ q, size_t half, Fr* __restrict__ vp,
                               Fr* __restrict__ vq) {
  GSTRIDE(i, half) {
// ... 512 lines not shown
```

halo2-lasso_amd/csrc/kernels_sumcheck.hip:

```cpp
#include <hip/hip_runtime.h>
#include <stdlib.h>
#include <algorithm>
#include "dev.hpp"
#include "reduce.cuh"
#include "resident.cuh"

namespace lh {

struct ScArgs {
  ScRound rd;
  uint8_t store[LH_SC_MAX_TERMS][LH_SC_MAX_FACTORS];
};

template <bool BIND>
__device__ __forceinline__ void load_pair(const Fr* __restrict__ in, Fr* __restrict__ out, size_t b, const Fr& r,
                                          bool store, Fr& v0, Fr& v1) {
  if (BIND) {
    const Fr* p = in + 4 * b;
    Fr e0 = p[0], e1 = p[1], e2 = p[2], e3 = p[3];
    v0 = add(mul(sub(e1, e0), r), e0);
    v1 = add(mul(sub(e3, e2), r), e2);
    if (store) {
      out[2 * b] = v0;
      out[2 * b + 1] = v1;
    }
  } else {
    v0 = in[2 * b];
    v1 = in[2 * b + 1];
  }
}


typedef ScFinishArgs ScFinish;

template <int D>
__device__ __forceinline__ void finish_round(const ScFinish& f, const Fr* __restrict__ partials, Fr* lds) {
  __shared__ int is_last;
  if (!fin_ticket(f, &is_last)) return;
  const uint32_t blocks = gridDim.x;
#pragma unroll
  for (int x = 0; x < D; x++) {
    Fr acc = Fr::zero();
    for (uint32_t i = threadIdx.x; i < blocks; i += blockDim.x) acc = add(acc, fin_get(f, partials, (size_t)i * D + x));
    acc = block_reduce_sum(acc, lds);
    if (threadIdx.x == 0) f.out_host[x] = acc;
  }
  if (threadIdx.x == 0) publish_round(f, D);
}

template <int D, bool BIND>
__global__ __launch_bounds__(256) __attribute__((amdgpu_waves_per_eu(D <= 2 ? 4 : 1, D <= 2 ? 4 : 8))) void sc_round_kernel(ScArgs a, size_t size, uint32_t tp,
                                                       Fr* __restrict__ partials, ScFinish fin) {
  __shared__ Fr lds[4];
  const ScRound& rd = a.rd;
  Fr acc[D];
#pragma unroll
  for (int x = 0; x < D; x++) acc[x] = Fr::zero();

  const size_t items = size * tp;
  for (size_t w = (size_t)blockIdx.x * blockDim.x + threadIdx.x; w < items; w += (size_t)gridDim.x * blockDim.x) {
    const size_t b = tp == 1 ? w : w / tp;
    const uint32_t m_lo = tp == 1 ? 0u : (uint32_t)(w % tp);
    const uint32_t m_hi = tp == 1 ? rd.num_terms : m_lo + 1u;
    Fr s[D];
#pragma unroll
    for (int x = 0; x < D; x++) s[x] = Fr::zero();
    for (uint32_t m = m_lo; m < m_hi; m++) {
      Fr pm[D];
      const int nf = rd.nfac[m];
      if (nf == 0) {
#pragma unroll
        for (int x = 0; x < D; x++) pm[x] = rd.coeff_is_one[m] ? Fr::one() : rd.coeff[m];
      }
      for (int k = 0; k < nf; k++) {
        const int t = rd.fac[m][k];
        Fr v0, v1;
        load_pair<BIND>(rd.in[t], rd.out[t], b, rd.r, a.store[m][k] != 0, v0, v1);
        if (k == 0) {
          if (!rd.coeff_is_one[m]) {
            v0 = mul(v0, rd.coeff[m]);
            v1 = mul(v1, rd.coeff[m]);
          }
          Fr step = sub(v1, v0);
          pm[0] = v1;
#pragma unroll
          for (int x = 1; x < D; x++) pm[x] = add(pm[x - 1], step);
        } else {
          Fr step = sub(v1, v0);
          Fr val = v1;
          pm[0] = mul(pm[0], val);
#pragma unroll
          for (int x = 1; x < D; x++) {
            val = add(val, step);
            pm[x] = mul(pm[x], val);
          }
        }
      }
#pragma unroll
      for (int x = 0; x < D; x++) s[x] = add(s[x], pm[x]);
    }
    if (rd.eq_level) {
      const Fr e = rd.eq_level[b];
#pragma unroll
      for (int x = 0; x < D; x++) s[x] = mul(s[x], e);
    } else if (rd.global_eq >= 0) {
      Fr v0, v1;
      load_pair<BIND>(rd.in[rd.global_eq], rd.out[rd.global_eq], b, rd.r, m_lo == 0, v0, v1);
      Fr step = sub(v1, v0);
      Fr val = v1;
      s[0] = mul(s[0], val);
#pragma unroll
      for (int x = 1; x < D; x++) {
        val = add(val, step);
        s[x] = mul(s[x], val);
      }
    }
#pragma unroll
    for (int x = 0; x < D; x++) acc[x] = add(acc[x], s[x]);
  }
#pragma unroll
  for (int x = 0; x < D; x++) {
    Fr v = block_reduce_sum(acc[x], lds);
    if (threadIdx.x == 0) fin_put(fin, partials, (size_t)blockIdx.x * D + x, v);
  }
  if (gridDim.x == 1) {
    if (threadIdx.x == 0) publish_round(fin, D);
    return;
  }
  finish_round<D>(fin, partials, lds);
}

__device__ __forceinline__ Fr dpp_xor1(const Fr& v) {
  Fr o;
#pragma unroll
  for (int i = 0; i < 8; i++) o.l[i] = (uint32_t)__builtin_amdgcn_mov_dpp((int)v.l[i], 0xB1, 0xF, 0xF, true);
  return o;
}
template <bool BIND>
__device__ __forceinline__ Fr load_entry(const Fr* __restrict__ in, Fr* __restrict__ out, size_t i, const Fr& r, bool store) {
  if (BIND) {
    const Fr e0 = in[2 * i], e1 = in[2 * i + 1];
    const Fr v = add(mul(sub(e1, e0), r), e0);
    if (store) out[i] = v;
    return v;
  }
  return in[i];
}
__device__ __forceinline__ Fr at_lane_point(const Fr& v, bool odd) {
  const Fr o = dpp_xor1(v);
  return odd ? v : sub(dbl(o), v);
}
__device__ __forceinline__ void reduce_by_parity(const Fr& acc, bool odd, Fr* lds, Fr& even_sum, Fr& odd_sum) {
  even_sum = block_reduce_sum(odd ? Fr::zero() : acc, lds);
  odd_sum = block_reduce_sum(odd ? acc : Fr::zero(), lds);
}

template <bool BIND>
__global__ __launch_bounds__(256) void sc_round_e2_kernel(ScArgs a, size_t size, Fr* __restrict__ partials, ScFinish fin) {
  __shared__ Fr lds[4];
  const ScRound& rd = a.rd;
  Fr acc = Fr::zero();
  const size_t items = 2 * size;
  const bool odd = threadIdx.x & 1;
  for (size_t i = (size_t)blockIdx.x * blockDim.x + threadIdx.x; i < items; i += (size_t)gridDim.x * blockDim.x) {
    Fr s = Fr::zero();
    for (uint32_t m = 0; m < rd.num_terms; m++) {
      const int nf = rd.nfac[m];
      Fr pm = rd.coeff_is_one[m] ? Fr::one() : rd.coeff[m];
      for (int k = 0; k < nf; k++) {
        const int t = rd.fac[m][k];
        const Fr val = at_lane_point(load_entry<BIND>(rd.in[t], rd.out[t], i, rd.r, a.store[m][k] != 0), odd);
        pm = k == 0 ? (rd.coeff_is_one[m] ? val : mul(val, rd.coeff[m])) : mul(pm, val);
      }
      s = add(s, pm);
    }
    acc = add(acc, mul(s, rd.eq_level[i >> 1]));
  }
  Fr q2, q1;
  reduce_by_parity(acc, odd, lds, q2, q1);
  if (threadIdx.x == 0) {
    fin_put(fin, partials, (size_t)blockIdx.x * 2, q1);
    fin_put(fin, partials, (size_t)blockIdx.x * 2 + 1, q2);
  }
  if (gridDim.x == 1) {
    if (threadIdx.x == 0) publish_round(fin, 2);
    return;
  }
  finish_round<2>(fin, partials, lds);
}

template <bool BIND>
__global__ __launch_bounds__(256) __attribute__((amdgpu_waves_per_eu(3, 8))) void sc_round_pp_kernel(ScArgs a, size_t size, Fr* __restrict__ partials, ScFinish fin) {
  __shared__ Fr lds[4];
  const ScRound& rd = a.rd;
  Fr acc = Fr::zero();
  const size_t items = 2 * size;
  const bool odd = threadIdx.x & 1;
  const bool fold = BIND && rd.pp == 2;
  const uint32_t K = rd.num_terms;
  const Fr rch = rd.r;
  for (size_t i = (size_t)blockIdx.x * blockDim.x + threadIdx.x; i < items; i += (size_t)gridDim.x * blockDim.x) {
    Fr s = Fr::zero();
    for (uint32_t m0 = 0; m0 < K; m0 += 4) {
      Fr av[4], bv[4];
#pragma unroll
      for (int h2 = 0; h2 < 2; h2++) {
        const uint32_t ma = m0 + 2 * h2, mb = ma + 1;
        const bool va = ma < K, vb = mb < K;
        const int t0 = rd.fac[va ? ma : 0][0], t1 = rd.fac[va ? ma : 0][1], t2 = rd.fac[vb ? mb : 0][0], t3 = rd.fac[vb ? mb : 0][1];
        const Fr* __restrict__ p0 = rd.in[t0];
        const Fr* __restrict__ p1 = rd.in[t1];
        const Fr* __restrict__ p2 = rd.in[t2];
        const Fr* __restrict__ p3 = rd.in[t3];
        Fr x0, x1, x2, x3;
        if (BIND) {
          const Fr e00 = p0[2 * i], e01 = p0[2 * i + 1], e10 = p1[2 * i], e11 = p1[2 * i + 1];
          const Fr e20 = p2[2 * i], e21 = p2[2 * i + 1], e30 = p3[2 * i], e31 = p3[2 * i + 1];
          x0 = add(mul(sub(e01, e00), rch), e00);
          x1 = add(mul(sub(e11, e10), rch), e10);
          x2 = add(mul(sub(e21, e20), rch), e20);
          x3 = add(mul(sub(e31, e30), rch), e30);
        } else {
          x0 = p0[i], x1 = p1[i], x2 = p2[i], x3 = p3[i];
        }
        if (BIND && !fold) {
          if (va) rd.out[t0][i] = x0, rd.out[t1][i] = x1;
          if (vb) rd.out[t2][i] = x2, rd.out[t3][i] = x3;
        }
        if (va && !rd.coeff_is_one[ma]) x0 = mul(x0, rd.coeff[ma]);
        if (vb && !rd.coeff_is_one[mb]) x2 = mul(x2, rd.coeff[mb]);
        if (BIND && fold) {
          if (va) rd.out[t0][i] = x0, rd.out[t1][i] = x1;
          if (vb) rd.out[t2][i] = x2, rd.out[t3][i] = x3;
        }
        av[2 * h2] = va ? at_lane_point(x0, odd) : Fr::zero();
        bv[2 * h2] = va ? at_lane_point(x1, odd) : Fr::zero();
        av[2 * h2 + 1] = vb ? at_lane_point(x2, odd) : Fr::zero();
        bv[2 * h2 + 1] = vb ? at_lane_point(x3, odd) : Fr::zero();
      }
      s = add(s, dot<FrParams, 4>(av, bv));
    }
    acc = add(acc, mul(s, rd.eq_level[i >> 1]));
  }
  Fr q2, q1;
  reduce_by_parity(acc, odd, lds, q2, q1);
  if (threadIdx.x == 0) {
    fin_put(fin, partials, (size_t)blockIdx.x * 2, q1);
    fin_put(fin, partials, (size_t)blockIdx.x * 2 + 1, q2);
  }
  if (gridDim.x == 1) {
    if (threadIdx.x == 0) publish_round(fin, 2);
    return;
  }
  finish_round<2>(fin, partials, lds);
}

constexpr int LDS_VALS = 1280;
constexpr int LDS_ITEMS = 512;
struct ScLdsArgs {
  ScArgs a;
  uint8_t used[SC_MAX_TABLES];
  uint8_t slot_of[SC_MAX_TABLES];
  uint32_t num_used;
  uint32_t P;
  uint32_t vals_entries;
};

template <int D, bool BIND>
__global__ __launch_bounds__(256) void sc_round_lds_kernel(ScLdsArgs g, size_t size, Fr* __restrict__ partials,
                                                           ScFinish fin) {
  extern __shared__ __align__(16) unsigned char lds_raw[];
  const ScRound& rd = g.a.rd;
  const uint32_t P = g.P, U = g.num_used;
  Fr* vals = (Fr*)lds_raw;
  Fr* red = vals + g.vals_entries;
  const size_t b0 = (size_t)blockIdx.x * P;
  for (uint32_t e = threadIdx.x; e < U * P * 2; e += blockDim.x) {
    const uint32_t which = e & 1u, pl = (e >> 1) % P, u = (e >> 1) / P;
    const size_t b = b0 + pl;
    Fr v = Fr::zero();
    if (b < size) {
      const int t = g.used[u];
      if (BIND) {
        const Fr* p = rd.in[t] + 4 * b + 2 * which;
        Fr e0 = p[0], e1 = p[1];
        v = add(mul(sub(e1, e0), rd.r), e0);
        rd.out[t][2 * b + which] = v;
      } else {
        v = rd.in[t][2 * b + which];
      }
    }
    vals[e] = v;
  }
  __syncthreads();
  const uint32_t items = rd.num_terms * D * P;
  for (uint32_t it = threadIdx.x; it < items; it += blockDim.x) {
    const uint32_t pl = it % P, mx = it / P, x = mx % D, m = mx / D;
    Fr acc = Fr::zero();
    if (b0 + pl < size) {
      const int nf = rd.nfac[m];
      for (int k = 0; k <= nf; k++) {
        int t;
        if (k < nf) t = rd.fac[m][k];
        else if (rd.global_eq >= 0) t = rd.global_eq;
        else break;
        const Fr* pv = vals + ((uint32_t)g.slot_of[t] * P + pl) * 2;
        Fr v0 = pv[0], v1 = pv[1];
        Fr val = v1;
        if (x > 0) {
          Fr step = sub(v1, v0);
          for (uint32_t j = 0; j < x; j++) val = add(val, step);
        }
        acc = k == 0 ? val : mul(acc, val);
      }
    }
    red[it] = acc;
  }
  __syncthreads();
  const uint32_t groups = rd.num_terms * D;
  Fr gsum = Fr::zero();
  if (threadIdx.x < groups) {
    for (uint32_t pl = 0; pl < P; pl++) gsum = add(gsum, red[threadIdx.x * P + pl]);
    const uint32_t m = threadIdx.x / D;
    if (!rd.coeff_is_one[m]) gsum = mul(gsum, rd.coeff[m]);
  }
  __syncthreads();
  if (threadIdx.x < groups) red[threadIdx.x] = gsum;
  __syncthreads();
  if (threadIdx.x < D) {
// ... 276 lines not shown
  a.cap = (uint32_t)std::max<size_t>(n0 / G, G);
  a.red_off = (uint32_t)((size_t)rd.num_tables * (a.cap + a.cap / 2));
  a.ticket = c.ticket;
  a.ticket_base = c.ticket_base;
  a.part = nullptr;
  a.bcast = nullptr;
  if (G > 1) {
    uint32_t rounds_a = 0;
    while (((size_t)G << (rounds_a + 1)) <= n0) rounds_a++;
    c.ticket_base += (rounds_a + 1) * G;
    a.part = c.arena.alloc_n<Fr>((size_t)2 * G * 8 + (size_t)rd.num_tables * G);
    a.bcast = (TailChunk*)(c.ticket + 32);
  }
  a.flag = c.flag;
  a.msg_host = msg_host;
  a.out_host = out_host;
  a.mbox = c.mbox();
  a.poll_ticks = (uint64_t)(knob(Knob::SC_TAIL_TIMEOUT_MS) * (double)c.wall_clock_khz);
  a.trace = nullptr;
  if (knob(Knob::SC_TAIL_TRACE) != 0) {
    a.trace = (uint64_t*)c.arena.alloc(32 * 8 * sizeof(uint64_t));
    LH_HIP(hipMemsetAsync(a.trace, 0, 32 * 8 * sizeof(uint64_t), c.stream));
    c.tail_trace = a.trace;
  }
  c.mbox_send(Fr::zero(), 0u);
  const size_t lds = ((size_t)a.red_off + tail_red_entries(rd, degree, a.cap)) * sizeof(Fr);
  c.opt_in_lds((const void*)sc_tail_kernel, (int)TAIL_LDS_BYTES + 2048);
  hipLaunchKernelGGL(sc_tail_kernel, dim3(G), dim3(G > 1 ? TAIL_THREADS_MULTI : TAIL_THREADS), lds, c.stream, a);
  LH_HIP(hipGetLastError());
}

void k_sc_tail_resync(Ctx& c) {
  LH_HIP(hipMemsetAsync(c.ticket + 32, 0, 4 * sizeof(TailChunk), c.stream));
  uint32_t v = 0;
  c.d2h(&v, c.ticket, sizeof(v));
  c.ticket_base = v;
}

bool k_sc_round_streams(const ScRound& rd, int degree, size_t size) {
  return !(rd.num_terms * (uint32_t)degree <= 256 && size * rd.num_terms <= ((size_t)1 << 16));
}

struct EqLevelsPack {
  const Fr* in;
  Fr* out[9];
};
__global__ __launch_bounds__(256) void eq_levels_kernel(EqLevelsPack pk, size_t n_in, int nlev) {
  const int lane = threadIdx.x & 63;
  const size_t waves = ((size_t)gridDim.x * blockDim.x) >> 6, tiles = (n_in + 511) / 512;
  for (size_t tile = ((size_t)blockIdx.x * blockDim.x + threadIdx.x) >> 6; tile < tiles; tile += waves) {
    Fr v[4];
#pragma unroll
    for (int r = 0; r < 4; r++) {
      const size_t i = tile * 512 + (size_t)r * 128 + 2 * (size_t)lane;
      v[r] = i + 1 < n_in ? add(pk.in[i], pk.in[i + 1]) : Fr::zero();
      if (nlev > 0 && (i >> 1) < (n_in >> 1)) pk.out[0][i >> 1] = v[r];
    }
#pragma unroll
    for (int k = 0; k < 6; k++) {
      const int lv = 1 + k;
#pragma unroll
      for (int r = 0; r < 4; r++) {
        Fr o;
#pragma unroll
        for (int q = 0; q < 8; q++) o.l[q] = __shfl_xor(v[r].l[q], 1 << k, 64);
        v[r] = add(v[r], o);
        if (lv < nlev && (lane & ((2 << k) - 1)) == 0) {
          const size_t idx = (tile * 256 + (size_t)r * 64 + (size_t)lane) >> (k + 1);
          if (idx < (n_in >> (lv + 1))) pk.out[lv][idx] = v[r];
        }
      }
    }
    if (lane == 0) {
      const Fr w0 = add(v[0], v[1]), w1 = add(v[2], v[3]);
      if (nlev > 7) {
        if (tile * 2 < (n_in >> 8)) pk.out[7][tile * 2] = w0;
        if (tile * 2 + 1 < (n_in >> 8)) pk.out[7][tile * 2 + 1] = w1;
      }
      if (nlev > 8 && tile < (n_in >> 9)) pk.out[8][tile] = add(w0, w1);
    }
  }
}
void k_eq_levels(Ctx& c, const Fr* in, size_t n_in, Fr* const* levels, size_t nlev) {
  size_t done = 0;
  while (done < nlev && n_in >= 2) {
    const size_t k = std::min<size_t>(9, nlev - done);
    EqLevelsPack pk;
    pk.in = in;
    for (size_t i = 0; i < 9; i++) pk.out[i] = i < k ? levels[done + i] : nullptr;
    const size_t waves = (n_in + 511) / 512;
    hipLaunchKernelGGL(eq_levels_kernel, dim3((unsigned)std::min<size_t>((waves + 3) / 4, 8192)), dim3(256), 0, c.stream, pk,
                       n_in, (int)k);
    in = levels[done + k - 1];
    n_in >>= k;
    done += k;
  }
}

static size_t sc_entry_grid(const Ctx& c, size_t entries) {
  constexpr size_t per_lane = 4;
  const size_t full = (entries + 255) / 256, cap = (size_t)c.num_cus * 8;
  size_t g = (entries + 256 * per_lane - 1) / (256 * per_lane);
  g = std::max(g, std::min(full, (size_t)c.num_cus * 2));
  return std::max<size_t>(1, std::min(std::min(g, full), cap));
}

template <int M, bool BIND>
__global__ __launch_bounds__(256) void sc_round_open_kernel(ScOpenRound rd, size_t size, Fr* __restrict__ partials, ScFinish fin) {
  __shared__ Fr lds[4];
  constexpr int NQ = 2 * M;
  Fr acc[M];
#pragma unroll
  for (int m = 0; m < M; m++) acc[m] = Fr::zero();
  const size_t items = 2 * size;
  const bool odd = threadIdx.x & 1;
  for (size_t i = (size_t)blockIdx.x * blockDim.x + threadIdx.x; i < items; i += (size_t)gridDim.x * blockDim.x) {
#pragma unroll
    for (int m = 0; m < M; m++) {
      const Fr v = load_entry<BIND>(rd.in[m], rd.out[m], i, rd.r, true);
      acc[m] = add(acc[m], mul(rd.eq_level[m][i >> 1], v));
    }
  }
#pragma unroll
  for (int m = 0; m < M; m++) {
    Fr q0, q1;
    reduce_by_parity(acc[m], odd, lds, q0, q1);
    if (threadIdx.x == 0) {
      fin_put(fin, partials, (size_t)blockIdx.x * NQ + 2 * m, q0);
      fin_put(fin, partials, (size_t)blockIdx.x * NQ + 2 * m + 1, q1);
    }
  }
  if (gridDim.x == 1) {
    if (threadIdx.x == 0) publish_round(fin, NQ);
    return;
  }
  finish_round<NQ>(fin, partials, lds);
}

template <int M>
static void launch_open(Ctx& c, const ScOpenRound& rd, bool bind, size_t size, unsigned g, Fr* partials, const ScFinish& fin) {
  if (bind)
    hipLaunchKernelGGL((sc_round_open_kernel<M, true>), dim3(g), dim3(256), 0, c.stream, rd, size, partials, fin);
  else
    hipLaunchKernelGGL((sc_round_open_kernel<M, false>), dim3(g), dim3(256), 0, c.stream, rd, size, partials, fin);
}

void k_sc_round_open(Ctx& c, const ScOpenRound& rd, bool bind, size_t size, Fr* out_host) {
  LH_REQUIRE(rd.num_terms >= 1 && rd.num_terms <= (uint32_t)SC_OPEN_MAX_TERMS && size >= 1, LH_ERR_ARG, "sc_round_open: bad shape");
  const uint32_t seq = c.next_seq();
  ArenaScope scope(c.arena);
  out_host = c.round_out(out_host);
  size_t g = sc_entry_grid(c, 2 * size);
  const int nq = 2 * (int)rd.num_terms;
  Fr* partials = g == 1 ? out_host : c.arena.alloc_n<Fr>(g * nq);
  const ScFinish fin = c.finish_for((uint32_t)g, out_host, seq, bind ? 64.0 * (double)size * rd.num_terms : 0.0);
  {
    ProfScope ps(c, bind ? "sc_round_open<bind>" : "sc_round_open<first>", ((bind ? 192.0 : 64.0) + 32.0) * (double)size * rd.num_terms,
                 (bind ? 4.0 : 2.0) * (double)size * rd.num_terms, (double)size);
    switch (rd.num_terms) {
      case 1: launch_open<1>(c, rd, bind, size, (unsigned)g, partials, fin); break;
      case 2: launch_open<2>(c, rd, bind, size, (unsigned)g, partials, fin); break;
      case 3: launch_open<3>(c, rd, bind, size, (unsigned)g, partials, fin); break;
      case 4: launch_open<4>(c, rd, bind, size, (unsigned)g, partials, fin); break;
      case 5: launch_open<5>(c, rd, bind, size, (unsigned)g, partials, fin); break;
      default: launch_open<6>(c, rd, bind, size, (unsigned)g, partials, fin); break;
    }
  }
  c.wait_round(seq);
}

template <int P, bool BIND, bool FOLD>
__global__ __launch_bounds__(256) void sc_round_rw_kernel(ScRwRound rd, size_t size, Fr* __restrict__ partials, ScFinish fin) {
  __shared__ Fr lds[4];
  Fr acc = Fr::zero();
  const size_t items = 2 * size;
  const bool odd = threadIdx.x & 1;
  for (size_t i = (size_t)blockIdx.x * blockDim.x + threadIdx.x; i < items; i += (size_t)gridDim.x * blockDim.x) {
    Fr av[P], bv[P];
#pragma unroll
    for (int p = 0; p < P; p++) {
      if (BIND && FOLD) {
        const Fr lf = mul(add(load_entry<true>(rd.l[p], rd.lo[p], i, rd.rchal, false), rd.k[p]), rd.cs[p]);
        const Fr rf = add(load_entry<true>(rd.r[p], rd.ro[p], i, rd.rchal, false), rd.k[p]);
        rd.lo[p][i] = lf, rd.ro[p][i] = rf;
        av[p] = at_lane_point(lf, odd), bv[p] = at_lane_point(rf, odd);
      } else {
        const Fr a = add(at_lane_point(load_entry<BIND>(rd.l[p], rd.lo[p], i, rd.rchal, true), odd), rd.k[p]);
        av[p] = mul(a, rd.cs[p]);
        bv[p] = add(at_lane_point(load_entry<BIND>(rd.r[p], rd.ro[p], i, rd.rchal, true), odd), rd.k[p]);
      }
    }
    acc = add(acc, mul(dot<FrParams, P>(av, bv), rd.eq_level[i >> 1]));
  }
  Fr q2, q1;
  reduce_by_parity(acc, odd, lds, q2, q1);
  if (threadIdx.x == 0) {
    fin_put(fin, partials, (size_t)blockIdx.x * 2, q1);
    fin_put(fin, partials, (size_t)blockIdx.x * 2 + 1, q2);
  }
  if (gridDim.x == 1) {
    if (threadIdx.x == 0) publish_round(fin, 2);
    return;
  }
  finish_round<2>(fin, partials, lds);
}

template <int P>
static void launch_rw(Ctx& c, const ScRwRound& rd, bool bind, bool fold, size_t size, unsigned g, Fr* partials, const ScFinish& fin) {
  if (bind && fold)
    hipLaunchKernelGGL((sc_round_rw_kernel<P, true, true>), dim3(g), dim3(256), 0, c.stream, rd, size, partials, fin);
  else if (bind)
    hipLaunchKernelGGL((sc_round_rw_kernel<P, true, false>), dim3(g), dim3(256), 0, c.stream, rd, size, partials, fin);
  else
    hipLaunchKernelGGL((sc_round_rw_kernel<P, false, false>), dim3(g), dim3(256), 0, c.stream, rd, size, partials, fin);
}

void k_sc_round_rw(Ctx& c, const ScRwRound& rd, bool bind, size_t size, Fr* out_host, bool fold) {
  LH_REQUIRE(!fold || bind, LH_ERR_ARG, "sc_round_rw: folding is part of a binding round");
  LH_REQUIRE(rd.num_pairs >= 1 && rd.num_pairs <= (uint32_t)SC_RW_MAX_PAIRS && size >= 1 && rd.eq_level, LH_ERR_ARG,
             "sc_round_rw: bad shape");
  const uint32_t seq = c.next_seq();
  ArenaScope scope(c.arena);
  out_host = c.round_out(out_host);
  size_t g = sc_entry_grid(c, 2 * size);
  Fr* partials = g == 1 ? out_host : c.arena.alloc_n<Fr>(g * 2);
  const ScFinish fin = c.finish_for((uint32_t)g, out_host, seq, bind ? 64.0 * (double)size * 2.0 * rd.num_pairs : 0.0);
  {
    const double P = (double)rd.num_pairs;
    ProfScope ps(c, bind ? "sc_round_rw<bind>" : "sc_round_rw<first>", ((bind ? 192.0 : 64.0) * 2.0 * P + 32.0) * (double)size,
                 ((bind ? 8.0 : 4.0) * P + 2.0) * (double)size, (double)size);
    switch (rd.num_pairs) {
      case 1: launch_rw<1>(c, rd, bind, fold, size, (unsigned)g, partials, fin); break;
      case 2: launch_rw<2>(c, rd, bind, fold, size, (unsigned)g, partials, fin); break;
      case 3: launch_rw<3>(c, rd, bind, fold, size, (unsigned)g, partials, fin); break;
      case 4: launch_rw<4>(c, rd, bind, fold, size, (unsigned)g, partials, fin); break;
      case 5: launch_rw<5>(c, rd, bind, fold, size, (unsigned)g, partials, fin); break;
      case 6: launch_rw<6>(c, rd, bind, fold, size, (unsigned)g, partials, fin); break;
      case 7: launch_rw<7>(c, rd, bind, fold, size, (unsigned)g, partials, fin); break;
      default: launch_rw<8>(c, rd, bind, fold, size, (unsigned)g, partials, fin); break;
    }
  }
  c.wait_round(seq);
}

bool k_sc_round(Ctx& c, const ScRound& rd, int degree, bool bind, size_t size, Fr* evals_host) {
  LH_REQUIRE(degree >= 1 && degree <= 6, LH_ERR_ARG, "sum-check degree must be in 1..6");
  LH_REQUIRE(size >= 1, LH_ERR_ARG, "sum-check round over an empty table");
  ScArgs a;
  a.rd = rd;
  bool seen[SC_MAX_TABLES] = {false};
  if (rd.global_eq >= 0) seen[rd.global_eq] = true;
  for (uint32_t m = 0; m < rd.num_terms; m++)
    for (int k = 0; k < rd.nfac[m]; k++) {
      int t = rd.fac[m][k];
      a.store[m][k] = seen[t] ? 0 : 1;
      seen[t] = true;
    }
  size_t tabs = 0;
  for (int t = 0; t < SC_MAX_TABLES; t++) tabs += seen[t] ? 1 : 0;
  double nfac = 0, ncoef = 0;
  for (uint32_t m = 0; m < rd.num_terms; m++) nfac += rd.nfac[m], ncoef += rd.coeff_is_one[m] ? 0 : 2;
  const double muls_pair = std::max(0.0, nfac - rd.num_terms) * degree + ncoef + (rd.global_eq >= 0 || rd.eq_level ? degree : 0) +
                           (bind ? 2.0 * (nfac + (rd.global_eq >= 0 ? 1 : 0)) : 0.0);
  const double bytes = (bind ? 192.0 : 64.0) * (double)size * (double)tabs + (rd.eq_level ? 32.0 * (double)size : 0.0);
  const uint32_t seq = c.next_seq();
  ArenaScope scope(c.arena);
  evals_host = c.round_out(evals_host);
  auto finish = [&](size_t grid, bool streams = false) {
    return c.finish_for((uint32_t)grid, evals_host, seq, streams && bind ? bytes / 3.0 : 0.0);
  };

  uint32_t P = (uint32_t)std::min<size_t>(size, 64);
  P = std::min<uint32_t>(P, LDS_VALS / (2 * (uint32_t)tabs));
  P = std::min<uint32_t>(P, LDS_ITEMS / (rd.num_terms * degree));
  const bool use_lds = P >= 1 && !rd.eq_level && !k_sc_round_streams(rd, degree, size);
  if (use_lds) {
    uint32_t want = (256 + rd.num_terms * degree - 1) / (rd.num_terms * degree);
    want = std::min<uint32_t>(want, std::max<uint32_t>(1, 256 / (2 * (uint32_t)tabs)));
    if (P > want && want >= 1) P = std::max<uint32_t>(want, 1);
    ScLdsArgs g;
    g.a = a;
    g.num_used = 0;
    for (int t = 0; t < SC_MAX_TABLES; t++)
      if (seen[t]) {
        g.slot_of[t] = (uint8_t)g.num_used;
        g.used[g.num_used++] = (uint8_t)t;
      }
    g.P = P;
    g.vals_entries = std::max<uint32_t>(g.num_used * P * 2, 8);
    size_t grid = (size + P - 1) / P;
    Fr* partials = grid == 1 ? evals_host : c.arena.alloc_n<Fr>(grid * degree);
    const ScFinish kflag = finish(grid);
    {
      char name[40];
      snprintf(name, sizeof name, "sc_round<%d,%s>/lds", degree, bind ? "bind" : "first");
      ProfScope ps(c, name, bytes, muls_pair * (double)size, (double)size);
      switch (degree) {
        case 1: launch_lds<1>(c, g, bind, size, (unsigned)grid, partials, kflag); break;
        case 2: launch_lds<2>(c, g, bind, size, (unsigned)grid, partials, kflag); break;
        case 3: launch_lds<3>(c, g, bind, size, (unsigned)grid, partials, kflag); break;
        case 4: launch_lds<4>(c, g, bind, size, (unsigned)grid, partials, kflag); break;
        case 5: launch_lds<5>(c, g, bind, size, (unsigned)grid, partials, kflag); break;
        default: launch_lds<6>(c, g, bind, size, (unsigned)grid, partials, kflag); break;
      }
    }
    c.wait_round(seq);
    return false;
  }

  const uint32_t tp = (rd.num_terms > 1 && size * rd.num_terms <= ((size_t)1 << 17)) ? rd.num_terms : 1u;
  if (degree == 2 && rd.eq_level && tp == 1) {
    size_t g2 = sc_entry_grid(c, 2 * size);
    Fr* partials = g2 == 1 ? evals_host : c.arena.alloc_n<Fr>(g2 * 2);
    const ScFinish kflag = finish(g2, true);
    if (rd.pp) {
      const double mp = (bind ? 2.0 * nfac : 0.0) + ncoef + 2.0 * 0.62 * rd.num_terms + 2.0;
      ProfScope ps(c, bind ? "sc_round_pp<bind>" : "sc_round_pp<first>", bytes, mp * (double)size, (double)size);
      if (bind) hipLaunchKernelGGL((sc_round_pp_kernel<true>), dim3((unsigned)g2), dim3(256), 0, c.stream, a, size, partials, kflag);
      else hipLaunchKernelGGL((sc_round_pp_kernel<false>), dim3((unsigned)g2), dim3(256), 0, c.stream, a, size, partials, kflag);
    } else {
      ProfScope ps(c, bind ? "sc_round<2,bind>" : "sc_round<2,first>", bytes, muls_pair * (double)size, (double)size);
      if (bind) hipLaunchKernelGGL((sc_round_e2_kernel<true>), dim3((unsigned)g2), dim3(256), 0, c.stream, a, size, partials, kflag);
      else hipLaunchKernelGGL((sc_round_e2_kernel<false>), dim3((unsigned)g2), dim3(256), 0, c.stream, a, size, partials, kflag);
    }
    c.wait_round(seq);
    return rd.pp == 2 && bind;
  }
  size_t g = (size * tp + 255) / 256;
  size_t cap = (size_t)c.num_cus * 4;
  if (g > cap) g = cap;
  Fr* partials = g == 1 ? evals_host : c.arena.alloc_n<Fr>(g * degree);
  const ScFinish kflag = finish(g, true);
  {
    char name[40];
    snprintf(name, sizeof name, "sc_round<%d,%s>%s", degree, bind ? "bind" : "first", tp > 1 ? "/tp" : "");
    ProfScope ps(c, name, bytes, muls_pair * (double)size, (double)size);
    switch (degree) {
      case 1: launch_round<1>(c, a, bind, size, tp, (unsigned)g, partials, kflag); break;
      case 2: launch_round<2>(c, a, bind, size, tp, (unsigned)g, partials, kflag); break;
      case 3: launch_round<3>(c, a, bind, size, tp, (unsigned)g, partials, kflag); break;
      case 4: launch_round<4>(c, a, bind, size, tp, (unsigned)g, partials, kflag); break;
      case 5: launch_round<5>(c, a, bind, size, tp, (unsigned)g, partials, kflag); break;
      default: launch_round<6>(c, a, bind, size, tp, (unsigned)g, partials, kflag); break;
    }
  }
  c.wait_round(seq);
  return false;
}

}
```

halo2-lasso_amd/csrc/reduce.cuh:

```cuda
#pragma once
#if !defined(__HIPCC_RTC__)
#include <hip/hip_runtime.h>
#endif
#include "ff.cuh"

namespace lh {

template <class P>
__device__ __forceinline__ Fp<P> wave_reduce_sum(Fp<P> v) {
#pragma unroll
  for (int off = 32; off > 0; off >>= 1) {
    Fp<P> o;
#pragma unroll
    for (int i = 0; i < 8; i++) o.l[i] = __shfl_down(v.l[i], off, 64);
    v = add(v, o);
  }
  return v;
}

template <class P>
__device__ __forceinline__ Fp<P> block_reduce_sum(Fp<P> v, Fp<P>* lds) {
  v = wave_reduce_sum(v);
  const int lane = threadIdx.x & 63, wave = threadIdx.x >> 6;
  const int nw = (blockDim.x + 63) >> 6;
  __syncthreads();
  if (lane == 0) lds[wave] = v;
  __syncthreads();
  if (threadIdx.x == 0) {
    for (int w = 1; w < nw; w++) v = add(v, lds[w]);
  }
  return v;
}

}
```

halo2-lasso_amd/csrc/sumcheck.cpp:

```cpp
#include <algorithm>
#include <functional>
#include <chrono>
#include <memory>
#include <thread>
#include "host.hpp"
#include "resident_host.hpp"

namespace lh {

std::vector<HFr> host_eq_xy(const std::vector<HFr>& y) {
  if (y.empty()) return {};
  std::vector<HFr> evals{HFr::one()};
  for (size_t i = y.size(); i-- > 0;) {
    std::vector<HFr> nxt(evals.size() * 2);
    for (size_t k = 0; k < evals.size(); k++) {
      nxt[2 * k + 1] = evals[k] * y[i];
      nxt[2 * k] = evals[k] - nxt[2 * k + 1];
    }
    evals.swap(nxt);
  }
  return evals;
}

HFr host_eq_xy_eval(const HFr* x, const HFr* y, size_t n) {
// ... 230 lines not shown
    for (int x = 1; x <= degree; x++) ev[x] = hst(sums[x - 1]);
    ev[0] = claim - ev[1];
    HFr r;
    if (prover_kind == LH_SC_COEFFICIENTS) {
      std::vector<HFr> co(3);
      co[0] = ev[0];
      co[2] = (ev[2] - ev[1].dbl() + ev[0]) * inv2;
      co[1] = claim - (co[0].dbl() + co[2]);
      tr.write_field_elements(co);
      r = tr.squeeze_challenge();
      pending = std::move(co), pending_coeffs = true;
    } else {
      tr.write_field_elements(ev);
      r = tr.squeeze_challenge();
      pending = std::move(ev), pending_coeffs = false;
    }
    pending_r = r;
    res.challenges.push_back(r);
    return r;
  };
  bool factored_round = false;
  Fr *d_part = nullptr, *d_all = nullptr;
  bool tail_ok = true;
  bool resident_ok = true;
  for (size_t round = 0; round < num_vars; round++) {
    bool bind = round > 0;
    if (sh && round == x_round) {
      len >>= 1;
      std::vector<size_t> live;
      for (size_t i = 0; i < T; i++) {
        bool factored = false;
        if (ef_on)
          for (const EqFactoring::One& one : ef->eqs) factored = factored || one.table == i;
        if (!factored) live.push_back(i);
      }
      const size_t L = live.size();
      Fr* block = c.arena.alloc_n<Fr>(L * len);
      std::vector<const Fr*> src(L);
      std::vector<Fr*> dst(L), rep(L);
      for (size_t k = 0; k < L; k++) src[k] = cur[live[k]], dst[k] = block + k * len;
      k_fix_var_multi(c, src.data(), dst.data(), L, len << 1, dev(r_prev));
      const size_t full = len << rho;
      for (size_t k = 0; k < L; k++) rep[k] = c.arena.alloc_n<Fr>(full);
      comm_gather_tables(c, block, L, len, (size_t)1 << (j - round), rep.data());
      c.route.v[RouteStats::SHARD_EXCHANGES]++;
      for (size_t k = 0; k < L; k++) cur[live[k]] = rep[k];
      if (ef_on && tail_ok && ef->resident_tail && !ef->per_term && !ef->untrusted && full >= 4 && full <= ((size_t)GKR_CAP * GKR_CAP)) {
        EqFactoring::One& one = ef->eqs[0];
        Fr* lvl = c.arena.alloc_n<Fr>(full >> 1);
        k_eq_xy(c, (const Fr*)(one.y + round + 1), num_vars - round - 1, lvl);
        one.level[round] = lvl;
        resolve_claim();
        if (ef->resident_tail(cur, false, r_prev, full, round, claim, tr, res)) return res;
      }
      if (ef_on) {
        for (EqFactoring::One& one : ef->eqs) {
          Fr* tab = c.arena.alloc_n<Fr>(full);
          k_eq_xy(c, (const Fr*)(one.y + round), num_vars - round, tab);
          k_scale(c, tab, dev(one.S), full, tab);
          cur[one.table] = tab;
        }
        ef_on = false;
      }
      len = full;
      alloc_bufs(len);
      flip = 0;
      sh = false;
      bind = false;
    }
    if (ef_on && !sh && tail_ok && resident_ok && ef->resident_tail) {
      const size_t n0 = bind ? len >> 1 : len;
      if (n0 >= 2 && n0 <= ((size_t)GKR_CAP * GKR_CAP) && (round > 0 || ef->trusted_claim) && !ef->untrusted) {
        resolve_claim();
        if (ef->resident_tail(cur, bind, r_prev, n0, round, claim, tr, res)) return res;
        resident_ok = false;
      }
    }
    const bool tail_now = !sh && tail_ok && tail_cap && (bind ? len >> 1 : len) <= tail_cap;
    const bool keep_factored = tail_ok && resident_ok && ef_on && ef->resident_tail && !ef->per_term && !ef->untrusted &&
                               (sh || (bind ? len >> 1 : len) > ((size_t)GKR_CAP * GKR_CAP));
    if (ef_on && !keep_factored && (tail_now || !ef->streams(bind, bind ? len >> 2 : len >> 1))) {
      for (EqFactoring::One& one : ef->eqs) {
        Fr* tab = c.arena.alloc_n<Fr>(len);
        if (round >= 2) {
          LH_REQUIRE(bind, LH_ERR_ARG, "sum-check: internal round mismatch");
          k_scale(c, one.level[round - 2], dev(one.S_prev), len, tab);
        } else if (sharded) {
          eq_xy_shard(c, Shard(c), one.y, num_vars, 0, tab);
        } else {
          k_eq_xy(c, (const Fr*)one.y, num_vars, tab);
        }
        cur[one.table] = tab;
      }
      ef_on = false;
    }
    if (tail_now) {
      const size_t n0 = bind ? len >> 1 : len, rounds = num_vars - round;
      LH_REQUIRE(((size_t)1 << rounds) == n0 && num_polys <= T, LH_ERR_ARG, "sum-check: internal size mismatch");
      ScRound rd = *tail_rd;
      for (size_t i = 0; i < T; i++) rd.in[i] = cur[i], rd.out[i] = nullptr;
      rd.r = dev(r_prev);
      const uint32_t seq0 = c.flag_seq + 1;
      c.flag_seq += (uint32_t)rounds + 1;
      const bool tail_debug = knob(Knob::SC_DEBUG) != 0;
      const auto t_tail = std::chrono::steady_clock::now();
      ProfScope ps(c, "sc_tail", 0, 0, (double)n0);
      struct Guard {
        Ctx& c;
        bool done = false;
        ~Guard() {
          if (done) return;
          c.mbox_abort();
          (void)hipStreamSynchronize(c.stream);
          try {
            k_sc_tail_resync(c);
          } catch (...) {
          }
        }
      } guard{c};
      TailChunk* chunks = (TailChunk*)evals_host;
      memset((void*)chunks, 0, 3 * SC_TAIL_MAX_DEGREE * sizeof(TailChunk));
      k_sc_tail_launch(c, rd, degree, n0, bind, num_polys, seq0, chunks, evals_host + 16);
      c.route.v[RouteStats::TAILS]++;
      double host_us = 0;
      size_t absorbed = 0;
      bool gave_up = false;
      Fr sums[SC_TAIL_MAX_DEGREE];
      auto wait = [&](uint32_t seq, bool msg) {
        try {
          if (msg) c.wait_chunks(chunks, 3 * (size_t)degree, seq, sums);
          else c.wait_flag(seq);
          return true;
        } catch (const Error& e) {
          if (e.code != LH_ERR_DEVICE || hipStreamQuery(c.stream) != hipSuccess) throw;
          return false;
        }
      };
      for (size_t i = 0; i < rounds && !gave_up; i++) {
        if (!wait(seq0 + (uint32_t)i, true)) {
          gave_up = true;
          break;
        }
        const auto t_h = std::chrono::steady_clock::now();
        const HFr r = message(sums);
        c.mbox_send(dev(r), seq0 + (uint32_t)i);
        absorbed = i + 1;
        c.route.v[RouteStats::TAIL_ROUNDS]++;
        if (tail_debug) host_us += std::chrono::duration<double, std::micro>(std::chrono::steady_clock::now() - t_h).count();
      }
      if (!gave_up && !wait(seq0 + (uint32_t)rounds, false)) gave_up = true;
      guard.done = true;
      if (!gave_up && c.tail_trace) {
        std::vector<uint64_t> st(rounds * 8);
        c.d2h(st.data(), c.tail_trace, st.size() * sizeof(uint64_t));
        c.tail_trace = nullptr;
        const double tick_us = 1e3 / (double)c.wall_clock_khz;
        fprintf(stderr, "[sc_tail trace] T %zu degree %d n0 %zu\n", T, degree, n0);
        for (size_t i = 0; i < rounds; i++) {
          const uint64_t* s8 = &st[i * 8];
          auto rel = [&](int k) { return s8[k] ? (double)(int64_t)(s8[k] - s8[0]) * tick_us : -1.0; };
          fprintf(stderr, "  round %2zu: eval %.2f ticket %.2f last-sees %.2f sent %.2f challenge %.2f | next round starts %.2f\n", i,
                  rel(1), rel(2), rel(3), rel(4), rel(5),
                  i + 1 < rounds && st[(i + 1) * 8] ? (double)(int64_t)(st[(i + 1) * 8] - s8[0]) * tick_us : -1.0);
        }
      }
      if (!gave_up) {
        if (tail_debug)
// ... 241 lines not shown
                        k_sc_round_streams(rd, degree, (size_t)1 << (nvl - 2));
  if (ef_enabled && nvl >= 3 && (!sharded || j >= 2) && (streams2 || tail_shape)) {
    if (rd.global_eq >= 0 && prover_kind == LH_SC_EVALUATIONS && degree >= 2 && (!sharded || sum_is_exact)) {
      bool ok = true;
      for (uint32_t m = 0; m < rd.num_terms && ok; m++)
        for (int k = 0; k < rd.nfac[m]; k++) ok = ok && rd.fac[m][k] != rd.global_eq;
      const HFr* y = ys + (size_t)expr.global_eq * num_vars;
      std::vector<HFr> d(num_vars);
      for (size_t i = 0; i < num_vars && ok; i++) {
        d[i] = HFr::one() - y[i];
        ok = !d[i].is_zero();
      }
      if (ok) {
        std::vector<HFr> pre(num_vars + 1);
        pre[0] = HFr::one();
        for (size_t i = 0; i < num_vars; i++) pre[i + 1] = pre[i] * d[i];
        HFr inv = pre[num_vars].inv();
        ef.inv_1my.resize(num_vars);
        for (size_t i = num_vars; i-- > 0;) {
          ef.inv_1my[i] = inv * pre[i];
          inv = inv * d[i];
        }
        ef.per_term = false;
        ef.trusted_claim = sum_is_exact;
        ef.c = sum;
        EqFactoring::One one;
        one.table = (size_t)rd.global_eq, one.y = y, one.S = one.S_prev = HFr::one();
        ef.eqs.push_back(one);
        use_ef = true;
      }
    } else if (rd.global_eq < 0 && prover_kind == LH_SC_COEFFICIENTS && rd.num_terms <= (uint32_t)SC_OPEN_MAX_TERMS &&
               T == 2 * (size_t)rd.num_terms) {
      bool ok = true;
      std::vector<char> seen(T, 0);
      for (uint32_t m = 0; m < rd.num_terms && ok; m++) {
        ok = rd.nfac[m] == 2 && rd.coeff_is_one[m];
        if (!ok) break;
        size_t a = rd.fac[m][0], b = rd.fac[m][1];
        if (a < num_polys) std::swap(a, b);
        ok = a >= num_polys && b < num_polys && !seen[a] && !seen[b];
        if (!ok) break;
        seen[a] = seen[b] = 1;
        EqFactoring::One one;
        one.table = a, one.y = ys + (a - num_polys) * num_vars, one.S = one.S_prev = HFr::one();
        ef.eqs.push_back(one);
        term_poly.push_back(b);
      }
      ef.per_term = true;
      use_ef = ok;
    }
  }
  ScU32 u32s = u32;
  Fr u32_r0;
  bool u32_bound = false;
  if (u32.col) {
    const bool u32_off = knob(Knob::SC_U32) == 0;
    u32_rounds = !u32_off && use_ef && !ef.per_term && !sharded && !rw && num_polys == 1 && rd.num_terms == 1 && rd.nfac[0] == 1 &&
                 rd.fac[0][0] == 0 && rd.coeff_is_one[0] && degree == 2 && sum_is_exact && streams2 && num_vars >= 6 &&
                 k_sc_round_streams(rd, degree, len0 >> 3) &&
                 (len0 >> 2) > std::max<size_t>(k_sc_tail_capacity(c, rd, degree), (size_t)GKR_CAP * GKR_CAP);
    if (!u32_rounds) k_fr_from_u32(c, u32.col, len0, const_cast<Fr*>(d_polys[0]));
  }
  std::vector<Fr> u32t_sums;
  Fr u32t_r0;
  if (!u32t.polys.empty()) {
    LH_REQUIRE(u32t.polys.size() == num_polys, LH_ERR_ARG, "sum-check: the column hint does not match the polys");
    bool ok = sc_open_column_rounds(c, num_vars, sharded) && use_ef && ef.per_term && degree == 2 && streams2 &&
              k_sc_round_streams(rd, degree, len0 >> 3) &&
              (len0 >> 2) > std::max<size_t>(k_sc_tail_capacity(c, rd, degree), (size_t)GKR_CAP * GKR_CAP);
    for (const ScU32Terms::Poly& pl : u32t.polys) {
      ok = ok && !pl.col.empty() && pl.col.size() <= 24;
      for (size_t ln : pl.len) ok = ok && ln % 4 == 0;
    }
    u32t_rounds = ok;
    if (!ok)
      for (size_t b = 0; b < num_polys; b++) {
        const ScU32Terms::Poly& pl = u32t.polys[b];
        k_lincomb_mixed(c, nullptr, nullptr, 0, pl.col.data(), pl.len.data(), pl.w.data(), pl.col.size(), len0, const_cast<Fr*>(d_polys[b]));
      }
  }
  const bool pp_shape = use_ef && !ef.per_term && pp_terms;
  std::vector<HFr> pp_folded;
  bool rw_folded = false;
  if (use_ef) {
    const Shard shg(c);
    const size_t half = (size_t)1 << (nvl - 1);
    for (EqFactoring::One& one : ef.eqs) {
      const Fr* shared = eq_half_lookup(c, one.y, num_vars, sharded);
      Fr* buf = c.arena.alloc_n<Fr>(shared ? half : 2 * half);
      one.level.resize(num_vars);
      size_t off = 0;
      for (size_t jl = 0; jl < nvl; jl++) {
        if (jl == 0 && shared) {
          one.level[0] = const_cast<Fr*>(shared);
          continue;
        }
        one.level[jl] = buf + off;
        off += half >> jl;
      }
      if (!shared) {
        if (sharded) eq_xy_shard(c, shg, one.y, num_vars, 1, buf);
        else k_eq_xy(c, (const Fr*)(one.y + 1), num_vars - 1, buf);
      }
      std::vector<Fr*> lower;
      for (size_t jl = 1; jl < nvl; jl++) lower.push_back((Fr*)one.level[jl]);
      k_eq_levels(c, one.level[0], half, lower.data(), lower.size());
    }
    ef.streams = [&](bool, size_t size) { return k_sc_round_streams(rd, degree, size); };
    ef.round = [&](const Fr* const* in, Fr* const* out, const Fr& r, bool bind, size_t size, size_t round, int points,
                   Fr* out_host) {
      if (!ef.per_term && rw && rw_folded) {
        LH_REQUIRE(points == 2, LH_ERR_ARG, "sum-check: tree-pair rounds asked for an extra point after the fold");
        ScRound g;
        memset(&g, 0, sizeof(g));
        g.num_tables = 2 * rw->num_pairs, g.num_terms = rw->num_pairs;
        for (size_t i = 0; i < 2 * (size_t)rw->num_pairs; i++) g.in[i] = in[i], g.out[i] = out[i];
        for (uint32_t m = 0; m < rw->num_pairs; m++) {
          g.coeff[m] = dev(HFr::one()), g.coeff_is_one[m] = 1;
          g.nfac[m] = 2, g.fac[m][0] = (uint8_t)(2 * m), g.fac[m][1] = (uint8_t)(2 * m + 1);
        }
        g.r = r;
        g.global_eq = -1;
        g.eq_level = ef.eqs[0].level[round];
        g.pp = 1;
        k_sc_round(c, g, points, bind, size, out_host);
        ef.add_const = rw->const_total;
      } else if (!ef.per_term && rw && points == 2) {
        ScRwRound g;
        memset(&g, 0, sizeof(g));
        g.num_pairs = rw->num_pairs;
        for (uint32_t i = 0; i < rw->num_pairs; i++) {
          g.l[i] = in[2 * i], g.r[i] = in[2 * i + 1];
          g.lo[i] = out[2 * i], g.ro[i] = out[2 * i + 1];
          g.cs[i] = dev(rw->cs[i]), g.k[i] = dev(rw->k[i]);
        }
        g.eq_level = ef.eqs[0].level[round];
        g.rchal = r;
        const bool fold = bind && c.opt.sc_pp_fold == 1;
        k_sc_round_rw(c, g, bind, size, out_host, fold);
        if (fold) {
          rw_folded = true;
          c.route.v[RouteStats::PP_FOLDS]++;
          const uint32_t P = rw->num_pairs;
          rd.num_terms = P + 1;
          for (uint32_t m = 0; m < P; m++) {
            rd.coeff[m] = dev(HFr::one()), rd.coeff_is_one[m] = 1;
            rd.nfac[m] = 2, rd.fac[m][0] = (uint8_t)(2 * m), rd.fac[m][1] = (uint8_t)(2 * m + 1);
          }
          rd.coeff[P] = dev(rw->const_total), rd.coeff_is_one[P] = 0, rd.nfac[P] = 0;
        }
        c.route.v[RouteStats::RW_ROUNDS]++;
        ef.add_const = rw->const_total;
      } else if (!ef.per_term && u32_rounds && round <= 2) {
        LH_REQUIRE(points == 1 && bind == (round >= 1), LH_ERR_ARG, "sum-check: the 32-bit rounds met another shape");
        if (round == 0) {
          if (!u32s.have_sums) {
            Fr s4[4];
            k_inner_products_small_quads(c, u32.col, ef.eqs[0].level[0], size >> 1, s4);
            u32s.odd = s4[1], u32s.s2 = s4[2], u32s.s3 = s4[3], u32s.have_sums = true;
          }
          out_host[0] = u32s.odd;
        } else if (round == 1) {
          u32_r0 = r;
          const HFr r0 = hst(r);
          out_host[0] = dev((HFr::one() - r0) * hst(u32s.s2) + r0 * hst(u32s.s3));
        } else {
          k_sc_round_u32_bind2(c, u32.col, ef.eqs[0].level[2], u32_r0, r, size, out[0], out_host);
          u32_bound = true;
        }
      } else if (!ef.per_term) {
        ScRound g = rd;
        for (size_t i = 0; i < T; i++) g.in[i] = in[i], g.out[i] = out[i];
        g.r = r;
        g.global_eq = -1;
        g.eq_level = ef.eqs[0].level[round];
        g.pp = pp_shape && points == 2 ? 1 : 0;
        if (g.pp && bind && pp_folded.empty() && c.opt.sc_pp_fold == 1) g.pp = 2;
        if (k_sc_round(c, g, points, bind, size, out_host)) {
          pp_folded.resize(rd.num_terms);
          for (uint32_t m = 0; m < rd.num_terms; m++) {
            memcpy(&pp_folded[m], &rd.coeff[m], 32);
            rd.coeff[m] = dev(HFr::one());
            rd.coeff_is_one[m] = 1;
          }
          c.route.v[RouteStats::PP_FOLDS]++;
        }
      } else if (u32t_rounds && round <= 2) {
        LH_REQUIRE(bind == (round >= 1), LH_ERR_ARG, "sum-check: the column rounds met another shape");
        const uint32_t M = rd.num_terms;
        if (round == 0) {
          ArenaScope scope(c.arena);
          const bool share = knob(Knob::OPEN_SHARE_SUMS) != 0;
          size_t total = 0;
          for (uint32_t m = 0; m < M; m++) total += u32t.polys[term_poly[m]].col.size();
          std::vector<Fr> hs(4 * total);
          std::vector<char> found(total, 0);
          size_t off = 0, missing = 0;
          for (uint32_t m = 0; m < M; m++) {
            const ScU32Terms::Poly& pl = u32t.polys[term_poly[m]];
            for (size_t k = 0; k < pl.col.size(); k++) {
              const Fr* s4 = share ? quad_sums_lookup(c, pl.col[k], pl.len[k], ef.eqs[m].y, num_vars) : nullptr;
              if (s4) memcpy(&hs[4 * (off + k)], s4, 4 * sizeof(Fr)), found[off + k] = 1;
              else missing++;
            }
            off += pl.col.size();
          }
          c.route.v[RouteStats::OPEN_SHARED_SUMS] += (uint32_t)(total - missing);
          if (missing) {
            Fr* d_s = c.arena.alloc_n<Fr>(4 * missing);
            size_t at = 0;
            off = 0;
            for (uint32_t m = 0; m < M; m++) {
              const ScU32Terms::Poly& pl = u32t.polys[term_poly[m]];
              std::vector<const uint32_t*> mc;
              std::vector<size_t> ml;
              for (size_t k = 0; k < pl.col.size(); k++)
                if (!found[off + k]) mc.push_back(pl.col[k]), ml.push_back(pl.len[k]);
              if (!mc.empty()) k_inner_products_quads(c, mc.data(), ml.data(), mc.size(), ef.eqs[m].level[1], size >> 1, d_s + 4 * at);
              at += mc.size();
              off += pl.col.size();
            }
            std::vector<Fr> ms(4 * missing);
            c.d2h(ms.data(), d_s, ms.size() * sizeof(Fr));
            at = 0;
            for (size_t i = 0; i < total; i++)
              if (!found[i]) memcpy(&hs[4 * i], &ms[4 * at++], 4 * sizeof(Fr));
          }
          u32t_sums.assign(4 * (size_t)M, dev(HFr::zero()));
          off = 0;
          for (uint32_t m = 0; m < M; m++) {
            const ScU32Terms::Poly& pl = u32t.polys[term_poly[m]];
            HFr t4[4] = {HFr::zero(), HFr::zero(), HFr::zero(), HFr::zero()};
            for (size_t k = 0; k < pl.col.size(); k++)
              for (int t = 0; t < 4; t++) t4[t] += hst(pl.w[k]) * hst(hs[4 * (off + k) + t]);
            off += pl.col.size();
            for (int t = 0; t < 4; t++) u32t_sums[4 * m + t] = dev(t4[t]);
            const HFr y1 = ef.eqs[m].y[1], n1 = HFr::one() - y1;
            out_host[2 * m] = dev(n1 * t4[0] + y1 * t4[2]);
            out_host[2 * m + 1] = dev(n1 * t4[1] + y1 * t4[3]);
          }
        } else if (round == 1) {
          u32t_r0 = r;
          const HFr r0 = hst(r), n0 = HFr::one() - r0;
          for (uint32_t m = 0; m < M; m++) {
            const Fr* t4 = &u32t_sums[4 * m];
            out_host[2 * m] = dev(n0 * hst(t4[0]) + r0 * hst(t4[1]));
            out_host[2 * m + 1] = dev(n0 * hst(t4[2]) + r0 * hst(t4[3]));
          }
        } else {
          Fr* two = (Fr*)c.pin(65536) + 1024;
          for (uint32_t m = 0; m < M; m++) {
            const ScU32Terms::Poly& pl = u32t.polys[term_poly[m]];
            k_lincomb_bind2(c, pl.col.data(), pl.len.data(), pl.w.data(), pl.col.size(), u32t_r0, r, ef.eqs[m].level[2], size,
                            out[term_poly[m]], two);
            out_host[2 * m] = two[0], out_host[2 * m + 1] = two[1];
          }
          u32t_bound = true;
        }
      } else {
        ScOpenRound g;
        g.num_terms = rd.num_terms;
        g.r = r;
        for (uint32_t m = 0; m < rd.num_terms; m++) {
          g.in[m] = in[term_poly[m]], g.out[m] = out[term_poly[m]];
          g.eq_level[m] = ef.eqs[m].level[round];
        }
        k_sc_round_open(c, g, bind, size, out_host);
      }
    };
  }
  if (use_ef && !ef.per_term && c.opt.gkr_resident && c.opt.sc_tail && (pp_shape || rw) && num_polys == 2 * (size_t)(rw ? rw->num_pairs : rd.num_terms) &&
      (rw ? rw->num_pairs : rd.num_terms) <= (uint32_t)GKR_MAX_TREES) {
    ef.resident_tail = [&](const std::vector<const Fr*>& cur_t, bool bind, const HFr& r_prev, size_t n0, size_t round,
                           const HFr& claim_now, Transcript& trr, SumCheckResult& res) {
      const size_t Bt = rw ? rw->num_pairs : rd.num_terms;
      GkrLayerDev L;
      memset(&L, 0, sizeof(L));
      L.B = (uint32_t)Bt;
      L.flags = GKR_F_SPLIT | GKR_F_NOMSG | GKR_F_EQ | (bind ? GKR_F_BIND : 0) | (rw && !rw_folded ? GKR_F_KOFF : 0);
      std::vector<size_t> li(Bt), ri(Bt);
      std::vector<HFr> co(Bt), ko(Bt, HFr::zero());
      for (size_t m = 0; m < Bt; m++) {
        li[m] = rw ? 2 * m : rd.fac[m][0], ri[m] = rw ? 2 * m + 1 : rd.fac[m][1];
        if (rw && rw_folded) co[m] = HFr::one();
        else if (rw) co[m] = rw->cs[m], ko[m] = rw->k[m];
        else memcpy(&co[m], &rd.coeff[m], 32);
        if (co[m].is_zero()) return false;
        L.lv[m] = cur_t[li[m]], L.rv[m] = cur_t[ri[m]];
        L.coef[m] = dev(co[m]), L.koff[m] = dev(ko[m]);
      }
      EqFactoring::One& e = ef.eqs[0];
      L.eq_level = e.level[round];
      L.r_prev = dev(r_prev);
      std::vector<HFr> x, finals;
      if (!resident_tail_run(c, L, n0, e.y + round, ef.inv_1my.data() + round, e.S, ef.c, claim_now, rw ? rw->const_total : HFr::zero(),
                             trr, x, finals))
        return false;
      res.challenges.insert(res.challenges.end(), x.begin(), x.end());
      std::vector<HFr> pre(Bt + 1);
      pre[0] = HFr::one();
      for (size_t m = 0; m < Bt; m++) pre[m + 1] = pre[m] * co[m];
      HFr inv = pre[Bt].inv();
      res.evals.assign(num_polys, HFr::zero());
      for (size_t m = Bt; m-- > 0;) {
        res.evals[li[m]] = finals[2 * m] * (inv * pre[m]) - ko[m];
        res.evals[ri[m]] = finals[2 * m + 1] - ko[m];
        inv = inv * co[m];
      }
      return true;
    };
  }
  for (size_t jy = 0; jy < num_ys; jy++) {
    bool factored = false;
    if (use_ef)
      for (const EqFactoring::One& one : ef.eqs) factored = factored || one.table == num_polys + jy;
    if (factored) continue;
    Fr* eq = c.arena.alloc_n<Fr>(len0);
    if (sharded) eq_xy_shard(c, Shard(c), ys + jy * num_vars, num_vars, 0, eq);
    else k_eq_xy(c, (const Fr*)(ys + jy * num_vars), num_vars, eq);
    cur[num_polys + jy] = eq;
  }
  SumCheckResult res = sum_check_loop(c, prover_kind, num_vars, degree, cur, used, num_polys, sum, tr, sharded, round_fn, &rd,
                                      use_ef ? &ef : nullptr);
  LH_REQUIRE(!u32_rounds || u32_bound, LH_ERR_DEVICE, "sum-check: the 32-bit column was never bound");
  LH_REQUIRE(!u32t_rounds || u32t_bound, LH_ERR_DEVICE, "sum-check: the 32-bit columns were never bound");
  res.u32_terms_built = !u32t.polys.empty() && !u32t_rounds;
  if (rw_folded) {
    const size_t K = rw->num_pairs;
    std::vector<HFr> pre(K + 1);
    pre[0] = HFr::one();
    for (size_t m = 0; m < K; m++) pre[m + 1] = pre[m] * rw->cs[m];
    HFr inv = pre[K].inv();
    for (size_t m = K; m-- > 0;) {
      res.evals[2 * m] = res.evals[2 * m] * (inv * pre[m]) - rw->k[m];
      res.evals[2 * m + 1] = res.evals[2 * m + 1] - rw->k[m];
      inv = inv * rw->cs[m];
    }
  }
  if (!pp_folded.empty()) {
    const size_t K = pp_folded.size();
    std::vector<HFr> pre(K + 1);
    pre[0] = HFr::one();
    for (size_t m = 0; m < K; m++) pre[m + 1] = pre[m] * pp_folded[m];
    HFr inv = pre[K].inv();
    for (size_t m = K; m-- > 0;) {
      res.evals[rd.fac[m][0]] = res.evals[rd.fac[m][0]] * (inv * pre[m]);
      inv = inv * pp_folded[m];
    }
  }
  return res;
}

}
```

include/lasso_hip.h:

```cpp
#ifndef LASSO_HIP_H
#define LASSO_HIP_H

#include <stddef.h>
#include <stdint.h>

#ifdef __cplusplus
extern "C" {
#endif

typedef struct { uint64_t l[4]; } lh_fr;
typedef struct { uint64_t x[4], y[4]; } lh_g1;

typedef int lh_status;
#define LH_OK 0
#define LH_ERR_INVALID_SUMCHECK (-1)
#define LH_ERR_INVALID_PCS_PARAM (-2)
#define LH_ERR_INVALID_PCS_OPEN (-3)
#define LH_ERR_INVALID_SNARK (-4)
#define LH_ERR_SERIALIZATION (-5)
#define LH_ERR_TRANSCRIPT (-6)
#define LH_ERR_DEVICE (-7)
#define LH_ERR_ARG (-8)

typedef struct lh_ctx lh_ctx;
// ... 72 lines not shown
#define LH_EX_SUM 7
#define LH_EX_PRODUCT 8
#define LH_EX_SCALED 9
typedef struct lh_expr_node { uint32_t op; int32_t a, b; uint32_t reserved; lh_fr scalar; } lh_expr_node;
typedef struct lh_expr { const lh_expr_node* nodes; size_t num_nodes; } lh_expr;
lh_status lh_sumcheck_prove_expr(lh_ctx*, size_t num_vars, const lh_expr* expr, const lh_fr* const* d_polys,
                                 size_t num_polys, const lh_fr* challenges, size_t num_challenges,
                                 const lh_fr* ys, size_t num_ys, const lh_fr* sum, lh_transcript* t,
                                 lh_fr* out_challenges, lh_fr* out_evals);

lh_status lh_gkr_fractional_prove(lh_ctx*, size_t num_batching, size_t num_vars,
                                  const lh_fr* const* claimed_p_0s, const lh_fr* const* claimed_q_0s,
                                  const lh_fr* const* d_ps, const lh_fr* const* d_qs,
                                  lh_transcript* t, lh_fr* out_p_xs, lh_fr* out_q_xs, lh_fr* out_x);
lh_status lh_grand_product_prove(lh_ctx*, size_t num_trees, const lh_fr* const* d_leaves,
                                 const size_t* num_vars, lh_transcript* t, lh_fr* out_roots,
                                 lh_fr* out_claims, lh_fr* out_points);

lh_status lh_msm(lh_ctx*, const lh_fr* d_scalars, const lh_g1* d_bases, size_t n, lh_g1* out);
lh_status lh_msm_u32(lh_ctx*, const uint32_t* d_scalars, const lh_g1* d_bases, size_t n, lh_g1* out);

typedef struct lh_srs lh_srs;
lh_status lh_mkzg_setup(lh_ctx*, const lh_fr* ss, size_t num_vars, lh_srs** out);
lh_status lh_srs_upload(lh_ctx*, const lh_g1* eqs_flat, size_t num_vars, lh_srs** out);
lh_status lh_srs_download(lh_ctx*, const lh_srs*, lh_g1* eqs_flat);
size_t lh_srs_num_vars(const lh_srs*);
void lh_srs_free(lh_ctx*, lh_srs*);
lh_status lh_mkzg_commit(lh_ctx*, const lh_srs*, const lh_fr* d_poly, size_t num_vars, lh_g1* out);
lh_status lh_mkzg_batch_commit(lh_ctx*, const lh_srs*, const lh_fr* const* d_polys, size_t num_polys,
                               size_t num_vars, lh_g1* out_comms);
lh_status lh_mkzg_open(lh_ctx*, const lh_srs*, const lh_fr* d_poly, size_t num_vars,
                       const lh_fr* point, lh_transcript* t, lh_fr* out_eval);
typedef struct lh_evaluation { uint32_t poly, point; lh_fr value; } lh_evaluation;
lh_status lh_mkzg_batch_open(lh_ctx*, const lh_srs*, size_t num_vars,
                             const lh_fr* const* d_polys, size_t num_polys,
                             const lh_fr* points, size_t num_points,
                             const lh_evaluation* evals, size_t num_evals, lh_transcript* t);

#define LH_SUBTABLE_IDENTITY 0
#define LH_SUBTABLE_AND 1
#define LH_SUBTABLE_XOR 2
#define LH_LASSO_MAX_CHUNKS 8
#define LH_LASSO_MAX_MEMORIES 16
#define LH_LASSO_MAX_TERMS 16
typedef struct lh_lasso_table {
  uint32_t num_chunks;
  uint32_t chunk_bits;
  uint32_t num_memories;
  uint32_t memory_chunk[LH_LASSO_MAX_MEMORIES];
  uint32_t memory_subtable[LH_LASSO_MAX_MEMORIES];
  uint32_t num_terms;
  lh_fr g_coeff[LH_LASSO_MAX_TERMS];
  uint8_t g_num_factors[LH_LASSO_MAX_TERMS];
  uint8_t g_factor[LH_LASSO_MAX_TERMS][LH_SC_MAX_FACTORS];
} lh_lasso_table;
lh_status lh_lasso_prove(lh_ctx*, const lh_srs*, const lh_lasso_table*, size_t num_vars,
                         const uint32_t* const* d_dims, lh_transcript* t);

#define LH_LASSO_NUM_PHASES 9
lh_status lh_lasso_last_timing(lh_ctx*, double* out_ms);

lh_status lh_ctx_set_option(lh_ctx*, const char* name, int64_t value);
lh_status lh_ctx_get_option(lh_ctx*, const char* name, int64_t* out);
#define LH_LASSO_ROUTE_WORDS 24
typedef struct lh_lasso_route {
  uint32_t open_small_depth;
  uint32_t open_small_passes;
  uint32_t eq_factored_rounds;
  uint32_t standard_rounds;
  uint32_t rw_leaf_rounds;
  uint32_t resident_tails;
  uint32_t resident_rounds;
  uint32_t packed_ts_pairs;
  uint32_t derived_commitments;
  uint32_t sorted_dim_reuse;
  uint32_t sharded_rounds;
  uint32_t shard_exchanges;
  uint32_t window_table_jobs;
  uint32_t open_precommit;
  uint32_t resident_layers;
  uint32_t pp_folds;
  uint32_t msm_half_batches;
  uint32_t open_shared_sums;
  uint32_t reserved[6];
} lh_lasso_route;
lh_status lh_lasso_last_route(lh_ctx*, lh_lasso_route* out);

typedef struct lh_comm {
  int rank, size;
  void* user;
  int (*all_gather)(void* user, const void* send, void* recv, size_t bytes_per_rank);
  int (*all_gather_device)(void* user, const void* d_send, void* d_recv, size_t bytes_per_rank, void* hip_stream);
} lh_comm;
lh_status lh_ctx_set_comm(lh_ctx*, const lh_comm* comm, size_t shard_bit);
#define LH_RCCL_UNIQUE_ID_BYTES 128
lh_status lh_rccl_unique_id(uint8_t out[LH_RCCL_UNIQUE_ID_BYTES]);
lh_status lh_ctx_set_comm_rccl(lh_ctx*, int rank, int size, const uint8_t unique_id[LH_RCCL_UNIQUE_ID_BYTES],
                               size_t shard_bit);
lh_status lh_ctx_set_comm_loopback(lh_ctx*, int rank, int size, size_t shard_bit);
lh_status lh_ctx_comm_stats(lh_ctx*, uint64_t out[2]);
lh_status lh_ctx_comm_phase_stats(lh_ctx*, uint64_t out[16], int reset);
lh_status lh_ctx_memory_stats(lh_ctx*, uint64_t out[4]);
lh_status lh_ctx_compute_units(lh_ctx*, size_t* out);
lh_status lh_ctx_host_cpus(lh_ctx*, char* bus_id, size_t bus_id_cap, char* cpulist, size_t cpulist_cap);
lh_status lh_lasso_prove_sharded(lh_ctx*, const lh_srs*, const lh_lasso_table*, size_t num_vars,
                                 const uint32_t* const* d_dims_local, lh_transcript* t);

typedef struct lh_hp_lookup {
  const lh_expr* inputs;
  const lh_expr* tables;
  size_t width;
} lh_hp_lookup;
#define LH_HP_LASSO_MAX_COMMITMENTS 63
typedef struct lh_hp_lasso_lookup {
  lh_lasso_table table;
  size_t output_poly;
  size_t chunk_polys[LH_LASSO_MAX_CHUNKS];
} lh_hp_lasso_lookup;
typedef struct lh_hp_param {
  size_t num_vars;
  size_t num_instance_polys;
  const size_t* num_instances;
  size_t num_preprocess_polys;
  const void* const* d_preprocess_polys;
  size_t num_witness_polys;
  size_t num_challenges;
  size_t num_lookups;
  const lh_hp_lookup* lookups;
  size_t num_permutation_polys;
  const size_t* permutation_poly_index;
  const void* const* d_permutation_polys;
  size_t num_permutation_z_polys;
  lh_expr expression;
  size_t num_lasso_lookups;
  const lh_hp_lasso_lookup* lasso_lookups;
} lh_hp_param;
lh_status lh_hyperplonk_prove(lh_ctx*, const lh_srs*, const lh_hp_param*, const lh_fr* const* instances,
                              const lh_fr* const* d_witness_polys, lh_transcript* t);

lh_status lh_shard_extract(lh_ctx*, const void* d_global, size_t n_local, size_t shard_bit, size_t rho, size_t rank,
                           size_t elem_bytes, void* d_local);
lh_status lh_hyperplonk_prove_sharded(lh_ctx*, const lh_srs*, const lh_hp_param*, const lh_fr* const* instances,
                                      const lh_fr* const* d_witness_polys_local, lh_transcript* t);

typedef struct lh_hp_circuit {
  void* user;
  int (*synthesize)(void* user, size_t round, const lh_fr* challenges, size_t num_challenges,
                    const void** d_out_polys, size_t num_out);
} lh_hp_circuit;
lh_status lh_hyperplonk_prove_phases(lh_ctx*, const lh_srs*, const lh_hp_param*, size_t num_phases,
                                     const size_t* num_witness_polys, const size_t* num_challenges,
                                     const lh_fr* const* instances, const lh_hp_circuit* circuit, lh_transcript* t);

typedef struct lh_g2 { uint64_t x_c0[4], x_c1[4], y_c0[4], y_c1[4]; } lh_g2;
typedef struct lh_mkzg_vp lh_mkzg_vp;
lh_status lh_mkzg_vp_setup(const lh_fr* ss, size_t num_vars, lh_mkzg_vp** out);
lh_status lh_mkzg_vp_new(const lh_g1* g1, const lh_g2* g2, const lh_g2* ss, size_t num_vars, lh_mkzg_vp** out);
lh_status lh_mkzg_vp_export(const lh_mkzg_vp*, lh_g1* g1, lh_g2* g2, lh_g2* ss);
size_t lh_mkzg_vp_num_vars(const lh_mkzg_vp*);
void lh_mkzg_vp_free(lh_mkzg_vp*);
lh_status lh_pairing_check(const lh_g1* ps, const lh_g2* qs, size_t n, int* out_is_identity);
lh_status lh_mkzg_verify(const lh_mkzg_vp*, const lh_g1* comm, const lh_fr* point, size_t num_vars,
                         const lh_fr* eval, lh_transcript* t);
lh_status lh_mkzg_batch_verify(const lh_mkzg_vp*, size_t num_vars, const lh_g1* comms, size_t num_comms,
                               const lh_fr* points, size_t num_points, const lh_evaluation* evals,
                               size_t num_evals, lh_transcript* t);
lh_status lh_sumcheck_verify(int prover_kind, size_t num_vars, size_t degree, const lh_fr* sum,
// ... 287 lines not shown
```

Baseline: 53.83 ms.

## Split eq levels into hi/lo tensor factors in factored sum-check rounds

```diff
diff --git a/bindings/rust/src/sys.rs b/bindings/rust/src/sys.rs
--- a/bindings/rust/src/sys.rs
+++ b/bindings/rust/src/sys.rs
@@ -201,7 +201,8 @@
     pub pp_folds: u32,
     pub msm_half_batches: u32,
     pub open_shared_sums: u32,
-    pub reserved: [u32; 6],
+    pub eq_split_rounds: u32,
+    pub reserved: [u32; 5],
 }
 
 extern "C" {
diff --git a/halo2-lasso_amd/__init__.py b/halo2-lasso_amd/__init__.py
--- a/halo2-lasso_amd/__init__.py
+++ b/halo2-lasso_amd/__init__.py
@@ -1501,7 +1501,7 @@
 ROUTE_FIELDS = ["open_small_depth", "open_small_passes", "eq_factored_rounds", "standard_rounds", "rw_leaf_rounds",
                 "resident_tails", "resident_rounds", "packed_ts_pairs", "derived_commitments", "sorted_dim_reuse",
                 "sharded_rounds", "shard_exchanges", "window_table_jobs", "open_precommit", "resident_layers", "pp_folds", "msm_half_batches",
-                "open_shared_sums"]
+                "open_shared_sums", "eq_split_rounds"]
 
 
 def lasso_last_route(ctx):
diff --git a/halo2-lasso_amd/csrc/dev.cpp b/halo2-lasso_amd/csrc/dev.cpp
--- a/halo2-lasso_amd/csrc/dev.cpp
+++ b/halo2-lasso_amd/csrc/dev.cpp
@@ -84,6 +84,7 @@
     {"sc_pp_fold", &Options::sc_pp_fold, 0, 2},                    {"msm_half_batches", &Options::msm_half_batches, 0, 1},
     {"comm_round", &Options::comm_round, 0, 2},                    {"hyrax_rows", &Options::hyrax_rows, 0, 1},
     {"brakedown_batch_commit", &Options::brakedown_batch_commit, 0, 1}, {"brakedown_staged_open", &Options::brakedown_staged_open, 0, 1},
+    {"sc_eq_split", &Options::sc_eq_split, 0, 40},
 };
 
 int64_t* Options::find(const char* name) {
diff --git a/halo2-lasso_amd/csrc/dev.hpp b/halo2-lasso_amd/csrc/dev.hpp
--- a/halo2-lasso_amd/csrc/dev.hpp
+++ b/halo2-lasso_amd/csrc/dev.hpp
@@ -98,6 +98,7 @@
   bool open_small_min_vars_forced = false;
   int64_t open_small_depth = 0;
   int64_t sc_eq_factoring = 1;
+  int64_t sc_eq_split = 20;
   int64_t lasso_pack_ts = 1;
   int64_t sc_tail = 1;
   int64_t sc_tail_max_len = 8192;
@@ -132,7 +133,7 @@
   uint32_t v[LH_LASSO_ROUTE_WORDS] = {0};
   enum { OPEN_DEPTH, OPEN_PASSES, EF_ROUNDS, STD_ROUNDS, RW_ROUNDS, TAILS, TAIL_ROUNDS, PACKED_TS, DERIVED, SORTED_REUSE,
          SHARDED_ROUNDS, SHARD_EXCHANGES, WIN_TABLE_JOBS, OPEN_PRECOMMIT, RESIDENT_LAYERS, PP_FOLDS, MSM_HALF_BATCHES,
-         OPEN_SHARED_SUMS };
+         OPEN_SHARED_SUMS, EQ_SPLIT_ROUNDS };
 };
 
 class HostWorker {
@@ -334,6 +335,16 @@
 void k_fix_var(Ctx&, const Fr* in, size_t n_in, const Fr& x, Fr* out);
 void k_fix_var_multi(Ctx&, const Fr* const* in, Fr* const* out, size_t count, size_t n_in, const Fr& x);
 void k_eq_xy(Ctx&, const Fr* y, size_t num_vars, Fr* out);
+void k_eq_outer(Ctx&, const Fr* lo_tab, int lo_bits, const Fr* hi_tab, size_t n, Fr* out);
+struct EqSplit {
+  const Fr* hi;
+  const Fr* lo;
+  uint32_t lo_bits;
+};
+int k_sc_split_lo_bits(const Ctx&, size_t size);
+constexpr int EQ_SPLIT_MAX_VARS = 32, EQ_SPLIT_MAX_TABLES = 64;
+void k_eq_split_tables(Ctx&, const Fr* y, size_t num_vars, const uint32_t* first, const uint32_t* bits, const uint32_t* off,
+                       size_t count, size_t total, Fr* out);
 void k_bind_first(Ctx&, const Fr* const* in, size_t count, const Fr& x, Fr* out_host);
 void k_gather_heads(Ctx&, const Fr* const* in, size_t count, int k, Fr* out_host);
 void k_lincomb(Ctx&, const Fr* const* polys, const Fr* w, size_t count, size_t n, Fr* out);
@@ -353,9 +364,9 @@
 constexpr int QS_MAX_COLS = 24;
 void k_quad_sums(Ctx&, const uint32_t* const* cols, const size_t* lens, size_t count, const Fr* e0, size_t quads, Fr* d_out);
 void k_lincomb_bind2(Ctx&, const uint32_t* const* cols, const size_t* lens, const Fr* w, size_t count, const Fr& r0, const Fr& r1,
-                     const Fr* eq_level, size_t size, Fr* out, Fr* out_host);
+                     const Fr* eq_level, size_t size, Fr* out, Fr* out_host, const EqSplit* split = nullptr);
 void k_sc_round_u32_bind2(Ctx&, const uint32_t* col, const Fr* eq_level, const Fr& r0, const Fr& r1, size_t size, Fr* out,
-                          Fr* out_host);
+                          Fr* out_host, const EqSplit* split = nullptr);
 void k_lincomb_mixed(Ctx&, const Fr* const* fr, const Fr* wfr, size_t num_fr, const uint32_t* const* sm,
                      const size_t* sm_len, const Fr* wsm, size_t num_sm, size_t n, Fr* out);
 void k_tree_up(Ctx&, const Fr* in, size_t half, Fr* out);
@@ -435,16 +446,21 @@
   uint8_t fac[LH_SC_MAX_TERMS][LH_SC_MAX_FACTORS];
   Fr r;
   const Fr* eq_level;
+  const Fr* eq_hi;
+  uint32_t eq_lo_bits;
   uint8_t pp;
 };
 bool k_sc_round(Ctx&, const ScRound& rd, int degree, bool bind, size_t size, Fr* evals_host);
 bool k_sc_round_streams(const ScRound& rd, int degree, size_t size);
+bool k_sc_round_can_split(const Ctx&, const ScRound& rd, int degree, size_t size);
 void k_eq_levels(Ctx&, const Fr* in, size_t n_in, Fr* const* levels, size_t nlev);
 constexpr int SC_OPEN_MAX_TERMS = 6;
 struct ScOpenRound {
   const Fr* in[SC_OPEN_MAX_TERMS];
   Fr* out[SC_OPEN_MAX_TERMS];
   const Fr* eq_level[SC_OPEN_MAX_TERMS];
+  const Fr* eq_hi[SC_OPEN_MAX_TERMS];
+  uint32_t eq_lo_bits;
   uint32_t num_terms;
   Fr r;
 };
@@ -458,6 +474,8 @@
   Fr* ro[SC_RW_MAX_PAIRS];
   Fr cs[SC_RW_MAX_PAIRS], k[SC_RW_MAX_PAIRS];
   const Fr* eq_level;
+  const Fr* eq_hi;
+  uint32_t eq_lo_bits;
   Fr rchal;
   uint32_t num_pairs;
 };
diff --git a/halo2-lasso_amd/csrc/host.hpp b/halo2-lasso_amd/csrc/host.hpp
--- a/halo2-lasso_amd/csrc/host.hpp
+++ b/halo2-lasso_amd/csrc/host.hpp
@@ -162,6 +162,7 @@
     size_t table;
     const HFr* y;
     std::vector<const Fr*> level;
+    std::vector<EqSplit> split;
     HFr S, S_prev;
     std::vector<HFr> q;
   };
@@ -173,6 +174,7 @@
   HFr c;
   HFr add_const;
   HFr kappa = HFr::one(), lin0 = HFr::zero(), lin1 = HFr::zero();
+  std::function<const Fr*(One& one, size_t j, bool with_lower)> level_of;
   std::function<bool(bool bind, size_t size)> streams;
   std::function<void(const Fr* const* in, Fr* const* out, const Fr& r, bool bind, size_t size, size_t round, int points,
                      Fr* out_host)>
diff --git a/halo2-lasso_amd/csrc/kernels_poly.hip b/halo2-lasso_amd/csrc/kernels_poly.hip
--- a/halo2-lasso_amd/csrc/kernels_poly.hip
+++ b/halo2-lasso_amd/csrc/kernels_poly.hip
@@ -235,7 +235,7 @@
 }
 
 void k_eq_xy(Ctx& c, const Fr* y, size_t num_vars, Fr* out) {
-  ProfScope ps(c, "eq_xy", 64.0 * ((size_t)1 << num_vars), 1.0 * ((size_t)1 << num_vars), (double)((size_t)1 << num_vars));
+  ProfScope ps(c, "eq_tables", 64.0 * ((size_t)1 << num_vars), 1.0 * ((size_t)1 << num_vars), (double)((size_t)1 << num_vars));
   const size_t ngroups = std::max<size_t>(1, (num_vars + EQ_SMALL - 1) / EQ_SMALL);
   LH_REQUIRE(ngroups <= (size_t)EQ_GROUPS, LH_ERR_ARG, "eq_xy: too many variables");
   ArenaScope scope(c.arena);
@@ -262,6 +262,52 @@
     cur = dst;
     done += cnt[k];
   }
+}
+
+void k_eq_outer(Ctx& c, const Fr* lo_tab, int lo_bits, const Fr* hi_tab, size_t n, Fr* out) {
+  ProfScope ps(c, "eq_outer", 32.0 * (double)n + 32.0 * (double)(n >> lo_bits), (double)n, (double)n);
+  hipLaunchKernelGGL(eq_outer_kernel, grid_for(n), 256, 0, c.stream, lo_tab, lo_bits, hi_tab, n, out);
+}
+
+struct EqSplitBuild {
+  Fr y[EQ_SPLIT_MAX_VARS];
+  uint32_t first[EQ_SPLIT_MAX_TABLES], off[EQ_SPLIT_MAX_TABLES + 1];
+  uint8_t bits[EQ_SPLIT_MAX_TABLES];
+  uint32_t count;
+};
+__global__ __launch_bounds__(256) void eq_split_tables_kernel(EqSplitBuild g, Fr* __restrict__ out) {
+  const uint32_t total = g.off[g.count];
+  for (uint32_t i = blockIdx.x * blockDim.x + threadIdx.x; i < total; i += gridDim.x * blockDim.x) {
+    uint32_t t = 0;
+    while (t + 1 < g.count && i >= g.off[t + 1]) t++;
+    const uint32_t e = i - g.off[t], first = g.first[t], bits = g.bits[t];
+    Fr acc = Fr::one();
+    for (uint32_t k = 0; k < bits; k++) {
+      const Fr yk = g.y[first + k];
+      acc = mul(acc, (e >> k) & 1 ? yk : sub(Fr::one(), yk));
+    }
+    out[i] = acc;
+  }
+}
+void k_eq_split_tables(Ctx& c, const Fr* y, size_t num_vars, const uint32_t* first, const uint32_t* bits, const uint32_t* off,
+                       size_t count, size_t total, Fr* out) {
+  LH_REQUIRE(num_vars <= (size_t)EQ_SPLIT_MAX_VARS && count >= 1 && count <= (size_t)EQ_SPLIT_MAX_TABLES && total >= 1 &&
+                 total < ((size_t)1 << 31),
+             LH_ERR_ARG, "eq_split_tables: bad shape");
+  EqSplitBuild g;
+  memset(&g, 0, sizeof(g));
+  for (size_t i = 0; i < num_vars; i++) g.y[i] = y[i];
+  size_t at = 0;
+  for (size_t t = 0; t < count; t++) {
+    LH_REQUIRE(off[t] == at && bits[t] <= 13 && (size_t)first[t] + bits[t] <= num_vars, LH_ERR_ARG, "eq_split_tables: bad table");
+    g.first[t] = first[t], g.bits[t] = (uint8_t)bits[t], g.off[t] = off[t];
+    at += (size_t)1 << bits[t];
+  }
+  LH_REQUIRE(at == total, LH_ERR_ARG, "eq_split_tables: the tables do not fill the buffer");
+  g.off[count] = (uint32_t)total;
+  g.count = (uint32_t)count;
+  ProfScope ps(c, "eq_split", 32.0 * (double)total, 7.0 * (double)total, (double)total);
+  hipLaunchKernelGGL(eq_split_tables_kernel, grid_for(total), 256, 0, c.stream, g, out);
 }
 
 template <class T>
@@ -846,14 +892,16 @@
   int count;
 };
 __global__ __launch_bounds__(256) void lincomb_bind2_kernel(const LcBind2* __restrict__ pkp, const Fr* __restrict__ eq_level,
-                                                            size_t entries, Fr* __restrict__ out, Fr* __restrict__ partials,
-                                                            ScFinishArgs fin) {
+                                                            EqSplit sp, size_t entries, Fr* __restrict__ out,
+                                                            Fr* __restrict__ partials, ScFinishArgs fin) {
   __shared__ Fr lds[4];
   __shared__ int is_last;
   const LcBind2& pk = *pkp;
   const bool odd = threadIdx.x & 1;
   Fr acc = Fr::zero();
-  GSTRIDE(i, entries) {
+  if (sp.hi) eq_level = sp.lo;
+  const EntryWalk wk = entry_walk(entries, sp.hi, sp.lo_bits);
+  for (size_t i = wk.first; i < wk.end; i += wk.step) {
     Wide t = Wide::zero();
     for (int k = 0; k < pk.count; k++)
       if (i < pk.quads[k]) {
@@ -862,10 +910,11 @@
       }
     const Fr v = wide_redc(t);
     out[i] = v;
-    acc = add(acc, mul(v, eq_level[i >> 1]));
-  }
-  const Fr q0 = block_reduce_sum(odd ? Fr::zero() : acc, lds);
-  const Fr q1 = block_reduce_sum(odd ? acc : Fr::zero(), lds);
+    acc = add(acc, mul(v, eq_level[(i >> 1) & wk.mask]));
+  }
+  Fr q0 = block_reduce_sum(odd ? Fr::zero() : acc, lds);
+  Fr q1 = block_reduce_sum(odd ? acc : Fr::zero(), lds);
+  if (sp.hi && threadIdx.x == 0) q0 = mul(q0, sp.hi[blockIdx.x]), q1 = mul(q1, sp.hi[blockIdx.x]);
   if (gridDim.x == 1) {
     if (threadIdx.x == 0) {
       fin.out_host[0] = q0, fin.out_host[1] = q1;
@@ -884,8 +933,13 @@
   if (threadIdx.x == 0) publish_round(fin, 2);
 }
 void k_lincomb_bind2(Ctx& c, const uint32_t* const* cols, const size_t* lens, const Fr* w, size_t count, const Fr& r0, const Fr& r1,
-                     const Fr* eq_level, size_t size, Fr* out, Fr* out_host) {
+                     const Fr* eq_level, size_t size, Fr* out, Fr* out_host, const EqSplit* split) {
   LH_REQUIRE(count >= 1 && count <= (size_t)LCB_MAX && size >= 1 && !c.sc_redirect, LH_ERR_ARG, "lincomb_bind2: bad shape");
+  EqSplit sp = {nullptr, nullptr, 0};
+  if (split && split->hi) {
+    LH_REQUIRE(k_sc_split_lo_bits(c, size) == (int)split->lo_bits, LH_ERR_ARG, "lincomb_bind2: the split eq level does not fit the launch");
+    sp = *split;
+  }
   const uint32_t seq = c.next_seq();
   ArenaScope scope(c.arena);
   const size_t entries = 2 * size;
@@ -910,12 +964,12 @@
   }
   LcBind2* d_pk = (LcBind2*)c.arena.alloc(sizeof(LcBind2));
   LH_HIP(hipMemcpyAsync(d_pk, h_pk, sizeof(LcBind2), hipMemcpyHostToDevice, c.stream));
-  const size_t g = std::min<size_t>((entries + 255) / 256, (size_t)c.num_cus * 8);
+  const size_t g = sp.hi ? size >> sp.lo_bits : std::min<size_t>((entries + 255) / 256, (size_t)c.num_cus * 8);
   Fr* partials = c.arena.alloc_n<Fr>(g * 2);
   const ScFinishArgs fin = c.finish_for((uint32_t)g, out_host, seq, 32.0 * (double)entries);
   {
-    ProfScope ps(c, "lincomb<bind2,u32>", (16.0 * count + 32.0 + 16.0) * (double)entries, (0.25 * count + 1.6) * (double)entries, (double)size);
-    hipLaunchKernelGGL(lincomb_bind2_kernel, dim3((unsigned)g), dim3(256), 0, c.stream, d_pk, eq_level, entries, out, partials, fin);
+    ProfScope ps(c, "lincomb<bind2,u32>", (16.0 * count + 32.0 + (sp.hi ? 0.0 : 16.0)) * (double)entries, (0.25 * count + 1.6) * (double)entries, (double)size);
+    hipLaunchKernelGGL(lincomb_bind2_kernel, dim3((unsigned)g), dim3(256), 0, c.stream, d_pk, eq_level, sp, entries, out, partials, fin);
   }
   c.wait_round(seq);
 }
@@ -924,20 +978,23 @@
   Fr w[4];
 };
 __global__ __launch_bounds__(256) void sc_round_u32_bind2_kernel(const uint32_t* __restrict__ col, const Fr* __restrict__ eq_level,
-                                                                 U32Bind2 k, size_t entries, Fr* __restrict__ out,
+                                                                 EqSplit sp, U32Bind2 k, size_t entries, Fr* __restrict__ out,
                                                                  Fr* __restrict__ partials, ScFinishArgs fin) {
   __shared__ Fr lds[4];
   __shared__ int is_last;
   Fr acc = Fr::zero();
-  GSTRIDE(i, entries) {
+  if (sp.hi) eq_level = sp.lo;
+  const EntryWalk wk = entry_walk(entries, sp.hi, sp.lo_bits);
+  for (size_t i = wk.first; i < wk.end; i += wk.step) {
     const uint4 a = ((const uint4*)col)[i];
     Wide t = Wide::zero();
     wide_mac(t, k.w[0], a.x), wide_mac(t, k.w[1], a.y), wide_mac(t, k.w[2], a.z), wide_mac(t, k.w[3], a.w);
     const Fr v = wide_redc(t);
     out[i] = v;
-    if (i & 1) acc = add(acc, mul(v, eq_level[i >> 1]));
+    if (i & 1) acc = add(acc, mul(v, eq_level[(i >> 1) & wk.mask]));
   }
   acc = block_reduce_sum(acc, lds);
+  if (sp.hi && threadIdx.x == 0) acc = mul(acc, sp.hi[blockIdx.x]);
   if (gridDim.x == 1) {
     if (threadIdx.x == 0) {
       fin.out_host[0] = acc;
@@ -956,12 +1013,17 @@
   }
 }
 void k_sc_round_u32_bind2(Ctx& c, const uint32_t* col, const Fr* eq_level, const Fr& r0, const Fr& r1, size_t size, Fr* out,
-                          Fr* out_host) {
+                          Fr* out_host, const EqSplit* split) {
   LH_REQUIRE(size >= 1 && !c.sc_redirect, LH_ERR_ARG, "sc_round_u32_bind2: bad shape");
+  EqSplit sp = {nullptr, nullptr, 0};
+  if (split && split->hi) {
+    LH_REQUIRE(k_sc_split_lo_bits(c, size) == (int)split->lo_bits, LH_ERR_ARG, "sc_round_u32_bind2: the split eq level does not fit the launch");
+    sp = *split;
+  }
   const uint32_t seq = c.next_seq();
   ArenaScope scope(c.arena);
   const size_t entries = 2 * size;
-  const size_t g = std::min<size_t>((entries + 255) / 256, (size_t)c.num_cus * 8);
+  const size_t g = sp.hi ? size >> sp.lo_bits : std::min<size_t>((entries + 255) / 256, (size_t)c.num_cus * 8);
   Fr* partials = c.arena.alloc_n<Fr>(g);
   const ScFinishArgs fin = c.finish_for((uint32_t)g, out_host, seq, 32.0 * (double)entries);
   host::Fr h0, h1;
@@ -976,8 +1038,8 @@
     k.w[i] = prescale_r(d);
   }
   {
-    ProfScope ps(c, "sc_round_u32<bind2>", 64.0 * (double)entries, 1.2 * (double)entries, (double)size);
-    hipLaunchKernelGGL(sc_round_u32_bind2_kernel, dim3((unsigned)g), dim3(256), 0, c.stream, col, eq_level, k, entries, out, partials, fin);
+    ProfScope ps(c, "sc_round_u32<bind2>", (sp.hi ? 48.0 : 64.0) * (double)entries, 1.2 * (double)entries, (double)size);
+    hipLaunchKernelGGL(sc_round_u32_bind2_kernel, dim3((unsigned)g), dim3(256), 0, c.stream, col, eq_level, sp, k, entries, out, partials, fin);
   }
   c.wait_round(seq);
 }
diff --git a/halo2-lasso_amd/csrc/kernels_sumcheck.hip b/halo2-lasso_amd/csrc/kernels_sumcheck.hip
--- a/halo2-lasso_amd/csrc/kernels_sumcheck.hip
+++ b/halo2-lasso_amd/csrc/kernels_sumcheck.hip
@@ -58,7 +58,8 @@
   for (int x = 0; x < D; x++) acc[x] = Fr::zero();
 
   const size_t items = size * tp;
-  for (size_t w = (size_t)blockIdx.x * blockDim.x + threadIdx.x; w < items; w += (size_t)gridDim.x * blockDim.x) {
+  const EntryWalk wk = entry_walk(items, rd.eq_hi, rd.eq_lo_bits, 0);
+  for (size_t w = wk.first; w < wk.end; w += wk.step) {
     const size_t b = tp == 1 ? w : w / tp;
     const uint32_t m_lo = tp == 1 ? 0u : (uint32_t)(w % tp);
     const uint32_t m_hi = tp == 1 ? rd.num_terms : m_lo + 1u;
@@ -100,7 +101,7 @@
       for (int x = 0; x < D; x++) s[x] = add(s[x], pm[x]);
     }
     if (rd.eq_level) {
-      const Fr e = rd.eq_level[b];
+      const Fr e = rd.eq_level[b & wk.mask];
 #pragma unroll
       for (int x = 0; x < D; x++) s[x] = mul(s[x], e);
     } else if (rd.global_eq >= 0) {
@@ -121,7 +122,10 @@
 #pragma unroll
   for (int x = 0; x < D; x++) {
     Fr v = block_reduce_sum(acc[x], lds);
-    if (threadIdx.x == 0) fin_put(fin, partials, (size_t)blockIdx.x * D + x, v);
+    if (threadIdx.x == 0) {
+      if (rd.eq_hi) v = mul(v, rd.eq_hi[blockIdx.x]);
+      fin_put(fin, partials, (size_t)blockIdx.x * D + x, v);
+    }
   }
   if (gridDim.x == 1) {
     if (threadIdx.x == 0) publish_round(fin, D);
@@ -162,7 +166,8 @@
   Fr acc = Fr::zero();
   const size_t items = 2 * size;
   const bool odd = threadIdx.x & 1;
-  for (size_t i = (size_t)blockIdx.x * blockDim.x + threadIdx.x; i < items; i += (size_t)gridDim.x * blockDim.x) {
+  const EntryWalk wk = entry_walk(items, rd.eq_hi, rd.eq_lo_bits);
+  for (size_t i = wk.first; i < wk.end; i += wk.step) {
     Fr s = Fr::zero();
     for (uint32_t m = 0; m < rd.num_terms; m++) {
       const int nf = rd.nfac[m];
@@ -174,11 +179,12 @@
       }
       s = add(s, pm);
     }
-    acc = add(acc, mul(s, rd.eq_level[i >> 1]));
+    acc = add(acc, mul(s, rd.eq_level[(i >> 1) & wk.mask]));
   }
   Fr q2, q1;
   reduce_by_parity(acc, odd, lds, q2, q1);
   if (threadIdx.x == 0) {
+    if (rd.eq_hi) q1 = mul(q1, rd.eq_hi[blockIdx.x]), q2 = mul(q2, rd.eq_hi[blockIdx.x]);
     fin_put(fin, partials, (size_t)blockIdx.x * 2, q1);
     fin_put(fin, partials, (size_t)blockIdx.x * 2 + 1, q2);
   }
@@ -199,7 +205,8 @@
   const bool fold = BIND && rd.pp == 2;
   const uint32_t K = rd.num_terms;
   const Fr rch = rd.r;
-  for (size_t i = (size_t)blockIdx.x * blockDim.x + threadIdx.x; i < items; i += (size_t)gridDim.x * blockDim.x) {
+  const EntryWalk wk = entry_walk(items, rd.eq_hi, rd.eq_lo_bits);
+  for (size_t i = wk.first; i < wk.end; i += wk.step) {
     Fr s = Fr::zero();
     for (uint32_t m0 = 0; m0 < K; m0 += 4) {
       Fr av[4], bv[4];
@@ -240,11 +247,12 @@
       }
       s = add(s, dot<FrParams, 4>(av, bv));
     }
-    acc = add(acc, mul(s, rd.eq_level[i >> 1]));
+    acc = add(acc, mul(s, rd.eq_level[(i >> 1) & wk.mask]));
   }
   Fr q2, q1;
   reduce_by_parity(acc, odd, lds, q2, q1);
   if (threadIdx.x == 0) {
+    if (rd.eq_hi) q1 = mul(q1, rd.eq_hi[blockIdx.x]), q2 = mul(q2, rd.eq_hi[blockIdx.x]);
     fin_put(fin, partials, (size_t)blockIdx.x * 2, q1);
     fin_put(fin, partials, (size_t)blockIdx.x * 2 + 1, q2);
   }
@@ -687,6 +695,7 @@
   }
 }
 void k_eq_levels(Ctx& c, const Fr* in, size_t n_in, Fr* const* levels, size_t nlev) {
+  ProfScope ps(c, "eq_tables", 32.0 * (double)n_in + 32.0 * (double)(n_in - (nlev < 64 ? n_in >> nlev : 0)), 0.0, (double)(n_in >> 1));
   size_t done = 0;
   while (done < nlev && n_in >= 2) {
     const size_t k = std::min<size_t>(9, nlev - done);
@@ -710,6 +719,21 @@
   return std::max<size_t>(1, std::min(std::min(g, full), cap));
 }
 
+int k_sc_split_lo_bits(const Ctx& c, size_t size) {
+  if (size < 128 || (size & (size - 1))) return -1;
+  int n = 0, hb = 0;
+  while (((size_t)1 << (n + 1)) <= size) n++;
+  const size_t g = sc_entry_grid(c, 2 * size);
+  while (((size_t)2 << hb) <= g) hb++;
+  hb = std::min(std::min(hb, 13), n - 7);
+  if (n - hb > 13) hb = n - 13;
+  return hb > 13 ? -1 : n - hb;
+}
+static size_t sc_split_grid(const Ctx& c, size_t size, uint32_t lo_bits) {
+  LH_REQUIRE(k_sc_split_lo_bits(c, size) == (int)lo_bits, LH_ERR_ARG, "sum-check round: the split eq level does not fit the launch");
+  return size >> lo_bits;
+}
+
 template <int M, bool BIND>
 __global__ __launch_bounds__(256) void sc_round_open_kernel(ScOpenRound rd, size_t size, Fr* __restrict__ partials, ScFinish fin) {
   __shared__ Fr lds[4];
@@ -719,11 +743,13 @@
   for (int m = 0; m < M; m++) acc[m] = Fr::zero();
   const size_t items = 2 * size;
   const bool odd = threadIdx.x & 1;
-  for (size_t i = (size_t)blockIdx.x * blockDim.x + threadIdx.x; i < items; i += (size_t)gridDim.x * blockDim.x) {
+  const bool split = rd.eq_hi[0] != nullptr;
+  const EntryWalk wk = entry_walk(items, rd.eq_hi[0], rd.eq_lo_bits);
+  for (size_t i = wk.first; i < wk.end; i += wk.step) {
 #pragma unroll
     for (int m = 0; m < M; m++) {
       const Fr v = load_entry<BIND>(rd.in[m], rd.out[m], i, rd.r, true);
-      acc[m] = add(acc[m], mul(rd.eq_level[m][i >> 1], v));
+      acc[m] = add(acc[m], mul(rd.eq_level[m][(i >> 1) & wk.mask], v));
     }
   }
 #pragma unroll
@@ -731,6 +757,7 @@
     Fr q0, q1;
     reduce_by_parity(acc[m], odd, lds, q0, q1);
     if (threadIdx.x == 0) {
+      if (split) q0 = mul(q0, rd.eq_hi[m][blockIdx.x]), q1 = mul(q1, rd.eq_hi[m][blockIdx.x]);
       fin_put(fin, partials, (size_t)blockIdx.x * NQ + 2 * m, q0);
       fin_put(fin, partials, (size_t)blockIdx.x * NQ + 2 * m + 1, q1);
     }
@@ -755,12 +782,15 @@
   const uint32_t seq = c.next_seq();
   ArenaScope scope(c.arena);
   out_host = c.round_out(out_host);
-  size_t g = sc_entry_grid(c, 2 * size);
+  bool split = rd.eq_hi[0] != nullptr;
+  for (uint32_t m = 0; m < rd.num_terms; m++)
+    LH_REQUIRE((rd.eq_hi[m] != nullptr) == split && rd.eq_level[m], LH_ERR_ARG, "sc_round_open: every term's eq level in the same form");
+  size_t g = split ? sc_split_grid(c, size, rd.eq_lo_bits) : sc_entry_grid(c, 2 * size);
   const int nq = 2 * (int)rd.num_terms;
   Fr* partials = g == 1 ? out_host : c.arena.alloc_n<Fr>(g * nq);
   const ScFinish fin = c.finish_for((uint32_t)g, out_host, seq, bind ? 64.0 * (double)size * rd.num_terms : 0.0);
   {
-    ProfScope ps(c, bind ? "sc_round_open<bind>" : "sc_round_open<first>", ((bind ? 192.0 : 64.0) + 32.0) * (double)size * rd.num_terms,
+    ProfScope ps(c, bind ? "sc_round_open<bind>" : "sc_round_open<first>", ((bind ? 192.0 : 64.0) + (split ? 0.0 : 32.0)) * (double)size * rd.num_terms,
                  (bind ? 4.0 : 2.0) * (double)size * rd.num_terms, (double)size);
     switch (rd.num_terms) {
       case 1: launch_open<1>(c, rd, bind, size, (unsigned)g, partials, fin); break;
@@ -780,7 +810,8 @@
   Fr acc = Fr::zero();
   const size_t items = 2 * size;
   const bool odd = threadIdx.x & 1;
-  for (size_t i = (size_t)blockIdx.x * blockDim.x + threadIdx.x; i < items; i += (size_t)gridDim.x * blockDim.x) {
+  const EntryWalk wk = entry_walk(items, rd.eq_hi, rd.eq_lo_bits);
+  for (size_t i = wk.first; i < wk.end; i += wk.step) {
     Fr av[P], bv[P];
 #pragma unroll
     for (int p = 0; p < P; p++) {
@@ -795,11 +826,12 @@
         bv[p] = add(at_lane_point(load_entry<BIND>(rd.r[p], rd.ro[p], i, rd.rchal, true), odd), rd.k[p]);
       }
     }
-    acc = add(acc, mul(dot<FrParams, P>(av, bv), rd.eq_level[i >> 1]));
+    acc = add(acc, mul(dot<FrParams, P>(av, bv), rd.eq_level[(i >> 1) & wk.mask]));
   }
   Fr q2, q1;
   reduce_by_parity(acc, odd, lds, q2, q1);
   if (threadIdx.x == 0) {
+    if (rd.eq_hi) q1 = mul(q1, rd.eq_hi[blockIdx.x]), q2 = mul(q2, rd.eq_hi[blockIdx.x]);
     fin_put(fin, partials, (size_t)blockIdx.x * 2, q1);
     fin_put(fin, partials, (size_t)blockIdx.x * 2 + 1, q2);
   }
@@ -827,12 +859,12 @@
   const uint32_t seq = c.next_seq();
   ArenaScope scope(c.arena);
   out_host = c.round_out(out_host);
-  size_t g = sc_entry_grid(c, 2 * size);
+  size_t g = rd.eq_hi ? sc_split_grid(c, size, rd.eq_lo_bits) : sc_entry_grid(c, 2 * size);
   Fr* partials = g == 1 ? out_host : c.arena.alloc_n<Fr>(g * 2);
   const ScFinish fin = c.finish_for((uint32_t)g, out_host, seq, bind ? 64.0 * (double)size * 2.0 * rd.num_pairs : 0.0);
   {
     const double P = (double)rd.num_pairs;
-    ProfScope ps(c, bind ? "sc_round_rw<bind>" : "sc_round_rw<first>", ((bind ? 192.0 : 64.0) * 2.0 * P + 32.0) * (double)size,
+    ProfScope ps(c, bind ? "sc_round_rw<bind>" : "sc_round_rw<first>", ((bind ? 192.0 : 64.0) * 2.0 * P + (rd.eq_hi ? 0.0 : 32.0)) * (double)size,
                  ((bind ? 8.0 : 4.0) * P + 2.0) * (double)size, (double)size);
     switch (rd.num_pairs) {
       case 1: launch_rw<1>(c, rd, bind, fold, size, (unsigned)g, partials, fin); break;
@@ -846,6 +878,13 @@
     }
   }
   c.wait_round(seq);
+}
+
+static uint32_t sc_term_lanes(const ScRound& rd, size_t size) {
+  return (rd.num_terms > 1 && size * rd.num_terms <= ((size_t)1 << 17)) ? rd.num_terms : 1u;
+}
+bool k_sc_round_can_split(const Ctx& c, const ScRound& rd, int degree, size_t size) {
+  return rd.eq_level && sc_term_lanes(rd, size) == 1 && k_sc_split_lo_bits(c, size) >= 0;
 }
 
 bool k_sc_round(Ctx& c, const ScRound& rd, int degree, bool bind, size_t size, Fr* evals_host) {
@@ -867,7 +906,7 @@
   for (uint32_t m = 0; m < rd.num_terms; m++) nfac += rd.nfac[m], ncoef += rd.coeff_is_one[m] ? 0 : 2;
   const double muls_pair = std::max(0.0, nfac - rd.num_terms) * degree + ncoef + (rd.global_eq >= 0 || rd.eq_level ? degree : 0) +
                            (bind ? 2.0 * (nfac + (rd.global_eq >= 0 ? 1 : 0)) : 0.0);
-  const double bytes = (bind ? 192.0 : 64.0) * (double)size * (double)tabs + (rd.eq_level ? 32.0 * (double)size : 0.0);
+  const double bytes = (bind ? 192.0 : 64.0) * (double)size * (double)tabs + (rd.eq_level && !rd.eq_hi ? 32.0 * (double)size : 0.0);
   const uint32_t seq = c.next_seq();
   ArenaScope scope(c.arena);
   evals_host = c.round_out(evals_host);
@@ -913,9 +952,10 @@
     return false;
   }
 
-  const uint32_t tp = (rd.num_terms > 1 && size * rd.num_terms <= ((size_t)1 << 17)) ? rd.num_terms : 1u;
+  const uint32_t tp = sc_term_lanes(rd, size);
+  LH_REQUIRE(!rd.eq_hi || k_sc_round_can_split(c, rd, degree, size), LH_ERR_ARG, "sum-check round: no kernel for a split eq level here");
   if (degree == 2 && rd.eq_level && tp == 1) {
-    size_t g2 = sc_entry_grid(c, 2 * size);
+    size_t g2 = rd.eq_hi ? sc_split_grid(c, size, rd.eq_lo_bits) : sc_entry_grid(c, 2 * size);
     Fr* partials = g2 == 1 ? evals_host : c.arena.alloc_n<Fr>(g2 * 2);
     const ScFinish kflag = finish(g2, true);
     if (rd.pp) {
@@ -934,6 +974,7 @@
   size_t g = (size * tp + 255) / 256;
   size_t cap = (size_t)c.num_cus * 4;
   if (g > cap) g = cap;
+  if (rd.eq_hi) g = sc_split_grid(c, size, rd.eq_lo_bits);
   Fr* partials = g == 1 ? evals_host : c.arena.alloc_n<Fr>(g * degree);
   const ScFinish kflag = finish(g, true);
   {
diff --git a/halo2-lasso_amd/csrc/reduce.cuh b/halo2-lasso_amd/csrc/reduce.cuh
--- a/halo2-lasso_amd/csrc/reduce.cuh
+++ b/halo2-lasso_amd/csrc/reduce.cuh
@@ -32,4 +32,20 @@
   return v;
 }
 
+struct EntryWalk {
+  size_t first, end, step, mask;
+};
+__device__ __forceinline__ EntryWalk entry_walk(size_t items, const void* eq_hi, uint32_t lo_bits, uint32_t per_pair = 1) {
+  EntryWalk w;
+  if (eq_hi) {
+    const size_t base = (size_t)blockIdx.x << (lo_bits + per_pair);
+    w.first = base + threadIdx.x, w.end = base + ((size_t)1 << (lo_bits + per_pair)), w.step = blockDim.x;
+    w.mask = ((size_t)1 << lo_bits) - 1;
+  } else {
+    w.first = (size_t)blockIdx.x * blockDim.x + threadIdx.x, w.end = items, w.step = (size_t)gridDim.x * blockDim.x;
+    w.mask = ~(size_t)0;
+  }
+  return w;
 }
+
+}
diff --git a/halo2-lasso_amd/csrc/sumcheck.cpp b/halo2-lasso_amd/csrc/sumcheck.cpp
--- a/halo2-lasso_amd/csrc/sumcheck.cpp
+++ b/halo2-lasso_amd/csrc/sumcheck.cpp
@@ -336,7 +336,13 @@
     if (ef_on && !keep_factored && (tail_now || !ef->streams(bind, bind ? len >> 2 : len >> 1))) {
       for (EqFactoring::One& one : ef->eqs) {
         Fr* tab = c.arena.alloc_n<Fr>(len);
-        if (round >= 2) {
+        if (round >= 2 && !one.level[round - 2] && ef->level_of) {
+          LH_REQUIRE(bind, LH_ERR_ARG, "sum-check: internal round mismatch");
+          Fr* t4 = c.arena.alloc_n<Fr>(4);
+          k_eq_xy(c, (const Fr*)(one.y + round - 1), 2, t4);
+          k_scale(c, t4, dev(one.S_prev), 4, t4);
+          k_eq_outer(c, t4, 2, ef->level_of(one, round, false), len, tab);
+        } else if (round >= 2) {
           LH_REQUIRE(bind, LH_ERR_ARG, "sum-check: internal round mismatch");
           k_scale(c, one.level[round - 2], dev(one.S_prev), len, tab);
         } else if (sharded) {
@@ -744,7 +750,81 @@
   const bool pp_shape = use_ef && !ef.per_term && pp_terms;
   std::vector<HFr> pp_folded;
   bool rw_folded = false;
-  if (use_ef) {
+  const bool eq_split = use_ef && c.opt.sc_eq_split > 0 && !sharded && num_vars <= (size_t)EQ_SPLIT_MAX_VARS &&
+                        (int64_t)num_vars - 1 >= c.opt.sc_eq_split && k_sc_split_lo_bits(c, (size_t)1 << (num_vars - 1)) >= 0;
+  if (eq_split) {
+    for (EqFactoring::One& one : ef.eqs) {
+      one.level.assign(num_vars, nullptr);
+      one.split.assign(num_vars, EqSplit{nullptr, nullptr, 0});
+      std::vector<uint32_t> first, bits, off;
+      std::vector<size_t> of_round;
+      size_t total = 0;
+      for (size_t jl = 0; jl + 1 < num_vars && 2 * of_round.size() + 2 <= (size_t)EQ_SPLIT_MAX_TABLES; jl++) {
+        const size_t nb = num_vars - 1 - jl;
+        const int lo = (int64_t)nb >= c.opt.sc_eq_split ? k_sc_split_lo_bits(c, (size_t)1 << nb) : -1;
+        if (lo < 0) continue;
+        first.push_back((uint32_t)(jl + 1)), bits.push_back((uint32_t)lo), off.push_back((uint32_t)total);
+        total += (size_t)1 << lo;
+        first.push_back((uint32_t)(jl + 1 + lo)), bits.push_back((uint32_t)(nb - lo)), off.push_back((uint32_t)total);
+        total += (size_t)1 << (nb - lo);
+        of_round.push_back(jl);
+      }
+      if (of_round.empty()) continue;
+      Fr* buf = c.arena.alloc_n<Fr>(total);
+      k_eq_split_tables(c, (const Fr*)one.y, num_vars, first.data(), bits.data(), off.data(), first.size(), total, buf);
+      for (size_t k = 0; k < of_round.size(); k++)
+        one.split[of_round[k]] = EqSplit{buf + off[2 * k + 1], buf + off[2 * k], bits[2 * k]};
+    }
+    ef.level_of = [&c, num_vars](EqFactoring::One& one, size_t jl, bool with_lower) -> const Fr* {
+      LH_REQUIRE(jl < num_vars, LH_ERR_ARG, "sum-check: no such eq level");
+      if (one.level[jl]) return one.level[jl];
+      const size_t n = (size_t)1 << (num_vars - 1 - jl);
+      const Fr* shared = jl == 0 ? eq_half_lookup(c, one.y, num_vars, false) : nullptr;
+      if (shared) {
+        one.level[jl] = shared;
+      } else {
+        Fr* buf = c.arena.alloc_n<Fr>(n);
+        k_eq_xy(c, (const Fr*)(one.y + jl + 1), num_vars - 1 - jl, buf);
+        one.level[jl] = buf;
+      }
+      if (with_lower && jl + 1 < num_vars && !one.level[jl + 1]) {
+        std::vector<Fr*> lower;
+        Fr* buf = c.arena.alloc_n<Fr>(n);
+        size_t off = 0;
+        for (size_t k = jl + 1; k < num_vars; k++) {
+          lower.push_back(buf + off);
+          one.level[k] = buf + off;
+          off += n >> (k - jl);
+        }
+        k_eq_levels(c, one.level[jl], n, lower.data(), lower.size());
+      }
+      return one.level[jl];
+    };
+  }
+  if (eq_split) {
+    for (EqFactoring::One& one : ef.eqs) {
+      size_t js = 0;
+      while (js < num_vars && one.split[js].hi) js++;
+      if (js < num_vars) ef.level_of(one, js, true);
+    }
+  }
+  auto level_for = [&](EqFactoring::One& one, size_t round, bool can_split, EqSplit& sp) -> const Fr* {
+    sp = EqSplit{nullptr, nullptr, 0};
+    if (!eq_split) return one.level[round];
+    if (can_split && one.split[round].hi) {
+      sp = one.split[round];
+      return sp.lo;
+    }
+    return ef.level_of(one, round, true);
+  };
+  auto set_level = [&](ScRound& g, size_t round, int points, size_t size) {
+    g.eq_level = (const Fr*)&g;
+    EqSplit sp;
+    g.eq_level = level_for(ef.eqs[0], round, k_sc_round_can_split(c, g, points, size), sp);
+    g.eq_hi = sp.hi, g.eq_lo_bits = sp.lo_bits;
+    if (sp.hi) c.route.v[RouteStats::EQ_SPLIT_ROUNDS]++;
+  };
+  if (use_ef && !eq_split) {
     const Shard shg(c);
     const size_t half = (size_t)1 << (nvl - 1);
     for (EqFactoring::One& one : ef.eqs) {
@@ -768,9 +848,12 @@
       for (size_t jl = 1; jl < nvl; jl++) lower.push_back((Fr*)one.level[jl]);
       k_eq_levels(c, one.level[0], half, lower.data(), lower.size());
     }
+  }
+  if (use_ef) {
     ef.streams = [&](bool, size_t size) { return k_sc_round_streams(rd, degree, size); };
     ef.round = [&](const Fr* const* in, Fr* const* out, const Fr& r, bool bind, size_t size, size_t round, int points,
                    Fr* out_host) {
+      LH_REQUIRE(!eq_split || size == (size_t)1 << (num_vars - 1 - round), LH_ERR_ARG, "sum-check: a factored round of another size");
       if (!ef.per_term && rw && rw_folded) {
         LH_REQUIRE(points == 2, LH_ERR_ARG, "sum-check: tree-pair rounds asked for an extra point after the fold");
         ScRound g;
@@ -783,8 +866,8 @@
         }
         g.r = r;
         g.global_eq = -1;
-        g.eq_level = ef.eqs[0].level[round];
         g.pp = 1;
+        set_level(g, round, points, size);
         k_sc_round(c, g, points, bind, size, out_host);
         ef.add_const = rw->const_total;
       } else if (!ef.per_term && rw && points == 2) {
@@ -796,7 +879,10 @@
           g.lo[i] = out[2 * i], g.ro[i] = out[2 * i + 1];
           g.cs[i] = dev(rw->cs[i]), g.k[i] = dev(rw->k[i]);
         }
-        g.eq_level = ef.eqs[0].level[round];
+        EqSplit sp;
+        g.eq_level = level_for(ef.eqs[0], round, true, sp);
+        g.eq_hi = sp.hi, g.eq_lo_bits = sp.lo_bits;
+        if (sp.hi) c.route.v[RouteStats::EQ_SPLIT_ROUNDS]++;
         g.rchal = r;
         const bool fold = bind && c.opt.sc_pp_fold == 1;
         k_sc_round_rw(c, g, bind, size, out_host, fold);
@@ -818,7 +904,8 @@
         if (round == 0) {
           if (!u32s.have_sums) {
             Fr s4[4];
-            k_inner_products_small_quads(c, u32.col, ef.eqs[0].level[0], size >> 1, s4);
+            const Fr* e0 = eq_split ? ef.level_of(ef.eqs[0], 0, false) : ef.eqs[0].level[0];
+            k_inner_products_small_quads(c, u32.col, e0, size >> 1, s4);
             u32s.odd = s4[1], u32s.s2 = s4[2], u32s.s3 = s4[3], u32s.have_sums = true;
           }
           out_host[0] = u32s.odd;
@@ -827,7 +914,10 @@
           const HFr r0 = hst(r);
           out_host[0] = dev((HFr::one() - r0) * hst(u32s.s2) + r0 * hst(u32s.s3));
         } else {
-          k_sc_round_u32_bind2(c, u32.col, ef.eqs[0].level[2], u32_r0, r, size, out[0], out_host);
+          EqSplit sp;
+          const Fr* e2 = level_for(ef.eqs[0], 2, true, sp);
+          if (sp.hi) c.route.v[RouteStats::EQ_SPLIT_ROUNDS]++;
+          k_sc_round_u32_bind2(c, u32.col, e2, u32_r0, r, size, out[0], out_host, &sp);
           u32_bound = true;
         }
       } else if (!ef.per_term) {
@@ -835,9 +925,9 @@
         for (size_t i = 0; i < T; i++) g.in[i] = in[i], g.out[i] = out[i];
         g.r = r;
         g.global_eq = -1;
-        g.eq_level = ef.eqs[0].level[round];
         g.pp = pp_shape && points == 2 ? 1 : 0;
         if (g.pp && bind && pp_folded.empty() && c.opt.sc_pp_fold == 1) g.pp = 2;
+        set_level(g, round, points, size);
         if (k_sc_round(c, g, points, bind, size, out_host)) {
           pp_folded.resize(rd.num_terms);
           for (uint32_t m = 0; m < rd.num_terms; m++) {
@@ -878,7 +968,13 @@
               std::vector<size_t> ml;
               for (size_t k = 0; k < pl.col.size(); k++)
                 if (!found[off + k]) mc.push_back(pl.col[k]), ml.push_back(pl.len[k]);
-              if (!mc.empty()) k_inner_products_quads(c, mc.data(), ml.data(), mc.size(), ef.eqs[m].level[1], size >> 1, d_s + 4 * at);
+              const Fr* e1 = ef.eqs[m].level[1];
+              if (!mc.empty() && !e1) {
+                Fr* t = c.arena.alloc_n<Fr>(size >> 1);
+                k_eq_xy(c, (const Fr*)(ef.eqs[m].y + 2), num_vars - 2, t);
+                e1 = t;
+              }
+              if (!mc.empty()) k_inner_products_quads(c, mc.data(), ml.data(), mc.size(), e1, size >> 1, d_s + 4 * at);
               at += mc.size();
               off += pl.col.size();
             }
@@ -911,22 +1007,31 @@
           }
         } else {
           Fr* two = (Fr*)c.pin(65536) + 1024;
+          bool split_round = false;
           for (uint32_t m = 0; m < M; m++) {
             const ScU32Terms::Poly& pl = u32t.polys[term_poly[m]];
-            k_lincomb_bind2(c, pl.col.data(), pl.len.data(), pl.w.data(), pl.col.size(), u32t_r0, r, ef.eqs[m].level[2], size,
-                            out[term_poly[m]], two);
+            EqSplit sp;
+            const Fr* e2 = level_for(ef.eqs[m], 2, true, sp);
+            split_round = split_round || sp.hi;
+            k_lincomb_bind2(c, pl.col.data(), pl.len.data(), pl.w.data(), pl.col.size(), u32t_r0, r, e2, size,
+                            out[term_poly[m]], two, &sp);
             out_host[2 * m] = two[0], out_host[2 * m + 1] = two[1];
           }
+          if (split_round) c.route.v[RouteStats::EQ_SPLIT_ROUNDS]++;
           u32t_bound = true;
         }
       } else {
         ScOpenRound g;
+        memset(&g, 0, sizeof(g));
         g.num_terms = rd.num_terms;
         g.r = r;
         for (uint32_t m = 0; m < rd.num_terms; m++) {
           g.in[m] = in[term_poly[m]], g.out[m] = out[term_poly[m]];
-          g.eq_level[m] = ef.eqs[m].level[round];
-        }
+          EqSplit sp;
+          g.eq_level[m] = level_for(ef.eqs[m], round, true, sp);
+          g.eq_hi[m] = sp.hi, g.eq_lo_bits = sp.lo_bits;
+        }
+        if (g.eq_hi[0]) c.route.v[RouteStats::EQ_SPLIT_ROUNDS]++;
         k_sc_round_open(c, g, bind, size, out_host);
       }
     };
@@ -952,7 +1057,7 @@
         L.coef[m] = dev(co[m]), L.koff[m] = dev(ko[m]);
       }
       EqFactoring::One& e = ef.eqs[0];
-      L.eq_level = e.level[round];
+      L.eq_level = eq_split ? ef.level_of(e, round, false) : e.level[round];
       L.r_prev = dev(r_prev);
       std::vector<HFr> x, finals;
       if (!resident_tail_run(c, L, n0, e.y + round, ef.inv_1my.data() + round, e.S, ef.c, claim_now, rw ? rw->const_total : HFr::zero(),
diff --git a/include/lasso_hip.h b/include/lasso_hip.h
--- a/include/lasso_hip.h
+++ b/include/lasso_hip.h
@@ -178,7 +178,8 @@
   uint32_t pp_folds;
   uint32_t msm_half_batches;
   uint32_t open_shared_sums;
-  uint32_t reserved[6];
+  uint32_t eq_split_rounds;
+  uint32_t reserved[5];
 } lh_lasso_route;
 lh_status lh_lasso_last_route(lh_ctx*, lh_lasso_route* out);
 
```

Result: no change. 53.31 ms, median of 6 (-1.0%).
